# qwagrox/field-coverage-path-planning

Measured on AMD Instinct MI355X. Metric: validated path points/sec (Clothoid+speed+geofence) on 500x200m field batch, higher is better.
Workload: dtype f64; 1 GPU; cfg1 x 4096: 4096 fields of 500 x 200 m per GPU, ARC turns (the reference's own model, pinned to its outputs) at the reference's sampling, 1691 points per field; a step = one fresh plan call of the ba; turn_model=arc (reference, pinned), points_per_gpu_step=6926336, fields_per_gpu=4096, setup=device

## Files before the change

### field_coverage_path_planning_amd/_lib.py

```python
import ctypes as C
import os

_HERE = os.path.dirname(os.path.abspath(__file__))
LIB_PATH = os.environ.get('FCPP_LIBRARY') or os.path.join(_HERE, 'libfcpp.so')

OK, EINVAL, EHEADLAND, EUNSUPPORTED, EHIP, ENOMEM, ESIZE = 0, -1, -2, -3, -4, -5, -6
TURN_ARC, TURN_CLOTHOID = 0, 1
KIND_SWATH, KIND_UTURN, KIND_HEAD_START, KIND_HEAD_STRAIGHT, KIND_CORNER, KIND_REVERSE, KIND_DETOUR = range(7)
OBSTACLES_FLAG, OBSTACLES_AVOID = 0, 1
RING_AS_VERTICES, RING_REVERSED = 0, 1
KIND_MASK, FLAG_HEADLAND, FLAG_ALAT, FLAG_OUTSIDE, FLAG_OBSTACLE, INDEX_SHIFT = 7, 8, 16, 32, 64, 8
OUTPUT_PITCH = 24 << 30

c_double_p = C.POINTER(C.c_double)
c_i64_p = C.POINTER(C.c_int64)


class FcppError(RuntimeError):
    def __init__(self, code, msg):
        super().__init__(f'libfcpp error {code}: {msg}')
        self.code = code


class Vehicle(C.Structure):
    _fields_ = [(n, C.c_double) for n in (
        'working_width', 'min_turn_radius', 'max_work_speed_kmh', 'max_headland_speed_kmh',
        'headland_turn_speed_kmh', 'max_lateral_accel', 'max_longitudinal_accel', 'safety_factor')]


class Options(C.Structure):
    _fields_ = [('turn_model', C.c_int32), ('clothoid_fit', C.c_int32), ('sample_spacing', C.c_double),
                ('clothoid_frac', C.c_double), ('geofence_tol', C.c_double), ('obstacle_mode', C.c_int32), ('ring_order', C.c_int32)]


class Field(C.Structure):
    _fields_ = [('vx', C.c_double * 4), ('vy', C.c_double * 4), ('from_vertices', C.c_int32),
                ('has_start', C.c_int32), ('has_end', C.c_int32),
                ('start_x', C.c_double), ('start_y', C.c_double), ('end_x', C.c_double), ('end_y', C.c_double),
                ('n_obstacles', C.c_int32), ('_pad', C.c_int32), ('obstacle_first', C.c_int64)]


class Polys(C.Structure):
    _fields_ = [('n_polys', C.c_int64), ('offsets', c_i64_p), ('x', c_double_p), ('y', c_double_p)]


class FieldInfo(C.Structure):
    _fields_ = [('point_offset', C.c_int64), ('n_main', C.c_int64), ('n_head', C.c_int64),
                ('n_swaths', C.c_int32), ('n_loops', C.c_int32), ('start_corner', C.c_int32),
                ('reverse_order', C.c_int32), ('start_from_right', C.c_int32), ('rotated', C.c_int32),
                ('start_kept', C.c_int32), ('end_kept', C.c_int32), ('shape', C.c_int32),
                ('n_reverse', C.c_int32 * 4), ('status', C.c_int32),
                ('corner_angles', C.c_double * 4), ('field_length', C.c_double), ('field_width', C.c_double),
                ('headland_width', C.c_double), ('rotation_angle', C.c_double),
                ('approach_from', C.c_double * 2), ('approach_to', C.c_double * 2),
                ('departure_from', C.c_double * 2), ('departure_to', C.c_double * 2)]


class FieldStats(C.Structure):
    _fields_ = [('main_len_m', C.c_double), ('main_time_pre_s', C.c_double), ('main_time_s', C.c_double),
                ('head_len_m', C.c_double), ('head_time_pre_s', C.c_double), ('head_time_s', C.c_double),
                ('max_kappa', C.c_double), ('max_alat', C.c_double), ('max_jump', C.c_double),
                ('n_viol', C.c_int64), ('n_outside', C.c_int64), ('n_in_obstacle', C.c_int64),
                ('n_adjusted', C.c_int64)]


class SetupTimes(C.Structure):
    _fields_ = [('host_plan_ms', C.c_double), ('templates_ms', C.c_double), ('tiler_ms', C.c_double), ('image_ms', C.c_double),
                ('h2d_ms', C.c_double), ('total_ms', C.c_double), ('image_bytes', C.c_int64), ('threads', C.c_int32), ('device_setup', C.c_int32)]


class GaConfig(C.Structure):
    _fields_ = [('population_size', C.c_int32), ('max_generations', C.c_int32), ('crossover_rate', C.c_double),
                ('mutation_rate', C.c_double), ('elite_size', C.c_int32), ('tournament_size', C.c_int32),
                ('convergence_threshold', C.c_int32), ('_pad', C.c_int32), ('seed', C.c_uint64)]


class GaResult(C.Structure):
    _fields_ = [('generations', C.c_int32), ('convergence_gen', C.c_int32), ('best_distance', C.c_double),
                ('best_fitness', C.c_double)]


class CoverJob(C.Structure):
    _fields_ = [('ox', C.c_double), ('oy', C.c_double), ('res', C.c_double), ('shift', C.c_double), ('radius', C.c_double),
                ('nx', C.c_int32), ('ny', C.c_int32), ('n_a', C.c_int32), ('n_b', C.c_int32),
                ('pts_first', C.c_int64), ('grid_first', C.c_int64), ('strict', C.c_int32), ('region', C.c_int32),
                ('outer', C.c_double * 12), ('inner', C.c_double * 12)]


SETUP_AUTO, SETUP_HOST, SETUP_DEVICE = 0, 1, 2

STATS_DOUBLES = 9
STATS_WORDS = 13

_VP = C.c_void_p
PROTOTYPES = [
    ('fcpp_last_error', C.c_char_p, []),
    ('fcpp_abi_version', C.c_int, []),
    ('fcpp_vehicle_default', None, [C.POINTER(Vehicle)]),
    ('fcpp_options_default', None, [C.POINTER(Options)]),
    ('fcpp_ctx_create', C.c_int, [C.c_int, C.POINTER(_VP)]),
    ('fcpp_ctx_destroy', C.c_int, [_VP]),
    ('fcpp_ctx_set_stream', C.c_int, [_VP, _VP]),
    ('fcpp_ctx_synchronize', C.c_int, [_VP]),
    ('fcpp_ctx_set_setup', C.c_int, [_VP, C.c_int]),
    ('fcpp_malloc', C.c_int, [_VP, C.c_int64, C.POINTER(_VP)]),
    ('fcpp_free', C.c_int, [_VP, _VP]),
    ('fcpp_ctx_reserve_outputs', C.c_int, [_VP, C.c_int64, C.c_int64]),
    ('fcpp_ctx_outputs_info', C.c_int, [_VP, c_i64_p, c_i64_p, c_i64_p]),
    ('fcpp_outputs_alloc', C.c_int, [_VP, C.c_int64, C.c_int64] + [C.POINTER(_VP)] * 5),
    ('fcpp_outputs_free', C.c_int, [_VP, _VP]),
    ('fcpp_memcpy_h2d', C.c_int, [_VP, _VP, _VP, C.c_int64]),
    ('fcpp_memcpy_d2h', C.c_int, [_VP, _VP, _VP, C.c_int64]),
    ('fcpp_plan_count', C.c_int, [C.POINTER(Vehicle), C.POINTER(Options), C.c_int64, C.POINTER(Field), C.POINTER(Polys),
                                  C.POINTER(FieldInfo)]),
    ('fcpp_plan_points', C.c_int, [_VP, C.POINTER(Vehicle), C.POINTER(Options), C.c_int64, C.POINTER(Field), C.POINTER(Polys), c_i64_p]),
    ('fcpp_batch_create', C.c_int, [_VP, C.POINTER(Vehicle), C.POINTER(Options), C.c_int64, C.POINTER(Field),
                                    C.POINTER(Polys), C.POINTER(_VP)]),
    ('fcpp_batch_plan', C.c_int, [_VP, C.POINTER(Vehicle), C.POINTER(Options), C.c_int64, C.POINTER(Field), C.POINTER(Polys), _VP,
                                  C.POINTER(_VP)] + [C.POINTER(_VP)] * 5 + [c_i64_p]),
    ('fcpp_batch_own_stats', C.c_int, [_VP, C.POINTER(_VP)]),
    ('fcpp_batch_info', C.c_int, [_VP, C.POINTER(FieldInfo), c_i64_p]),
    ('fcpp_batch_setup_times', C.c_int, [_VP, C.POINTER(SetupTimes)]),
    ('fcpp_batch_run', C.c_int, [_VP, _VP, _VP, _VP, _VP, _VP, _VP, C.c_int]),
    ('fcpp_batch_connectors', C.c_int, [_VP, _VP, _VP]),
    ('fcpp_batch_trajectory', C.c_int, [_VP] * 9),
    ('fcpp_batch_destroy', C.c_int, [_VP]),
    ('fcpp_batch_set_profiling', C.c_int, [_VP, C.c_int]),
    ('fcpp_batch_stage_times', C.c_int, [_VP, C.c_int, c_double_p, C.POINTER(C.c_int), C.POINTER(C.c_int)]),
    ('fcpp_batch_stage_name', C.c_char_p, [C.c_int, C.c_int]),
    ('fcpp_batch_stage_points', C.c_int, [_VP, C.c_int, C.c_int, c_i64_p]),
    ('fcpp_batch_point_split', C.c_int, [_VP, c_i64_p, c_i64_p]),
    ('fcpp_batch_reduce_classes', C.c_int, [_VP, c_i64_p]),
    ('fcpp_curvature', C.c_int, [_VP, C.c_int64, _VP, C.c_int64, _VP, _VP, _VP, _VP]),
    ('fcpp_speed_plan', C.c_int, [_VP, C.POINTER(Vehicle), C.c_int, C.c_int64, _VP, C.c_int64, _VP, _VP, _VP, _VP,
                                  _VP, _VP, _VP]),
    ('fcpp_verify', C.c_int, [_VP, C.POINTER(Vehicle), C.c_int64, _VP, C.c_int64, _VP, _VP, _VP, _VP, _VP]),
    ('fcpp_validate', C.c_int, [_VP, C.POINTER(Vehicle), C.POINTER(Options), C.c_int64, _VP, C.c_int64, _VP, _VP, _VP, C.POINTER(Polys),
                               C.POINTER(Polys), _VP, _VP, _VP, _VP]),
    ('fcpp_trajectory', C.c_int, [_VP, C.c_int64, _VP, C.c_int64] + [_VP] * 9),
    ('fcpp_trajectory_counts', C.c_int, [_VP, C.c_int64, _VP, C.c_double, C.c_int, _VP, _VP]),
    ('fcpp_trajectory_sample', C.c_int, [_VP, C.c_int64, _VP, C.c_int64] + [_VP] * 7 + [C.c_double, C.c_int, _VP, C.c_int64] + [_VP] * 9),
    ('fcpp_straight_segments', C.c_int, [_VP, C.c_int64, _VP, C.c_int32, _VP]),
    ('fcpp_corner_turns', C.c_int, [_VP, C.POINTER(Vehicle), C.c_int64, _VP, _VP, _VP, C.c_double, C.c_double, C.c_int32, _VP, _VP]),
    ('fcpp_fresnel', C.c_int, [_VP, C.c_int64, _VP, _VP, _VP]),
    ('fcpp_ga_fitness', C.c_int, [_VP, C.c_int32, C.c_int64, _VP, _VP, _VP, _VP, C.c_int]),
    ('fcpp_distance_matrix', C.c_int, [_VP, C.c_int32, _VP, _VP, _VP]),
    ('fcpp_best_connections', C.c_int, [_VP, C.c_int64, _VP, _VP, _VP, _VP, _VP, _VP, _VP, _VP, _VP]),
    ('fcpp_dubins_solve', C.c_int, [_VP, C.c_int64] + [_VP] * 6 + [C.c_double, _VP, _VP, _VP]),
    ('fcpp_dubins_matrix', C.c_int, [_VP, C.c_int64, _VP, _VP, _VP, C.c_int64, _VP, _VP, _VP, C.c_double, _VP, _VP]),
    ('fcpp_dubins_counts', C.c_int, [_VP, C.c_int64, _VP, C.c_double, _VP, _VP]),
    ('fcpp_dubins_sample', C.c_int, [_VP, C.c_int64, _VP, _VP, _VP, C.c_double, _VP, _VP, C.c_double, _VP, C.c_int64] + [_VP] * 5),
    ('fcpp_rs_solve', C.c_int, [_VP, C.c_int64] + [_VP] * 6 + [C.c_double, _VP, _VP, _VP]),
    ('fcpp_rs_matrix', C.c_int, [_VP, C.c_int64, _VP, _VP, _VP, C.c_int64, _VP, _VP, _VP, C.c_double, _VP, _VP]),
    ('fcpp_rs_counts', C.c_int, [_VP, C.c_int64, _VP, _VP, C.c_double, _VP, _VP]),
    ('fcpp_rs_sample', C.c_int, [_VP, C.c_int64, _VP, _VP, _VP, C.c_double, _VP, _VP, C.c_double, _VP, C.c_int64] + [_VP] * 6),
    ('fcpp_swath_scores', C.c_int, [_VP, C.c_int64, _VP, C.c_int64, _VP, C.c_int64, _VP, _VP, C.c_int64, _VP, C.c_double, C.c_double, C.c_double]
     + [_VP] * 4),
    ('fcpp_swath_counts', C.c_int, [_VP, C.c_int64, _VP, C.c_int64, _VP, C.c_int64, _VP, _VP, _VP, C.c_double, C.c_double, C.c_double] + [_VP] * 4),
    ('fcpp_swath_fill', C.c_int, [_VP, C.c_int64, _VP, C.c_int64, _VP, C.c_int64, _VP, _VP, _VP, C.c_double, C.c_double, C.c_double, _VP, C.c_int64]
     + [_VP] * 6),
    ('fcpp_ga_evolve', C.c_int, [_VP, C.c_int32, C.POINTER(GaConfig), _VP, _VP, _VP, _VP, C.POINTER(GaResult)]),
    ('fcpp_cover_grid', C.c_int, [_VP, C.c_int64, C.POINTER(CoverJob), C.c_int64, _VP, _VP, _VP, _VP]),
    ('fcpp_gather', C.c_int, [_VP, _VP, C.c_int, C.c_int, C.c_int, C.c_int, _VP, _VP, c_i64_p, _VP, C.c_int]),
    ('fcpp_debug_math', C.c_int, [C.c_int, C.c_int64, _VP, _VP, _VP, _VP]),
    ('fcpp_debug_math_dev', C.c_int, [_VP, C.c_int, C.c_int64, _VP, _VP, _VP, _VP]),
    ('fcpp_debug_dubins', C.c_int, [C.c_int64] + [_VP] * 6 + [C.c_double, _VP, _VP, _VP]),
    ('fcpp_debug_rs', C.c_int, [C.c_int64] + [_VP] * 6 + [C.c_double, _VP, _VP, _VP]),
    ('fcpp_debug_swaths', C.c_int, [C.c_int64, _VP, C.c_int64, _VP, C.c_int64, _VP, _VP, C.c_int64, _VP, C.c_int, C.c_double, C.c_double, C.c_double]
     + [_VP] * 5 + [C.c_int64] + [_VP] * 6),
    ('fcpp_batch_debug_table', C.c_int, [_VP, C.c_int, _VP, C.c_int64, c_i64_p]),
]

_lib = None


def load():
    global _lib
    if _lib is None:
        if not os.path.exists(LIB_PATH):
            raise ImportError(
                f'{LIB_PATH} is missing: build it with `python -c "import __graft_entry__ as g; g.build()"` '
                f'or `make -C {os.path.join(_HERE, "csrc")}`; there is no CPU fallback')
        try:
            import torch
        except ImportError:
            pass
        lib = C.CDLL(LIB_PATH)
        for name, res, args in PROTOTYPES:
            fn = getattr(lib, name)
            fn.restype = res
            fn.argtypes = args
        if lib.fcpp_abi_version() != 5:
            raise ImportError('libfcpp.so ABI version mismatch')
        _lib = lib
    return _lib


def check(rc):
    if rc != OK:
        raise FcppError(rc, load().fcpp_last_error().decode('utf-8', 'replace'))


def default_vehicle():
    v = Vehicle()
    load().fcpp_vehicle_default(C.byref(v))
    return v


def default_options():
    o = Options()
    load().fcpp_options_default(C.byref(o))
    return o
```

### field_coverage_path_planning_amd/csrc/fcpp_api.cpp

```cpp
#include <dlfcn.h>
#include <hip/hip_runtime_api.h>
#include <math.h>
#include <stdio.h>
#include <stdlib.h>
#include <string.h>

#include <algorithm>
#include <atomic>
#include <chrono>
#include <memory>
#include <new>
#include <string>
#include <vector>

#include "fcpp_api_internal.h"
#include "fcpp_cover.h"
#include "fcpp_ga.h"
#include "fcpp_devplan.h"
#include "fcpp_dubinsfn.h"
#include "fcpp_rsfn.h"
#include "fcpp_parallel.h"

using namespace fcpp;

namespace fcpp { thread_local LaunchProf g_launch_prof; }

namespace { thread_local std::string g_err; }

int fcpp::fail(int code, const std::string &msg) { g_err = msg; return code; }

DevConst fcpp::make_const(const fcpp_vehicle &veh, const fcpp_options &opt)
{
    DevConst c;
    c.a_lat = veh.max_lateral_accel; c.a_lon = veh.max_longitudinal_accel; c.sf = veh.safety_factor;
    c.geofence_tol = opt.geofence_tol;
    c.v_work = veh.max_work_speed_kmh; c.v_turn = veh.headland_turn_speed_kmh; c.v_head = veh.max_headland_speed_kmh;
    const double vm = std::max(std::max(veh.max_work_speed_kmh, veh.max_headland_speed_kmh),
                               std::max(veh.headland_turn_speed_kmh, 2.5)) / 3.6;
    c.u_cap = vm * vm;
    c.inv_sf36 = 1.0 / (c.sf * 3.6);
    c.ms_work = c.v_work / 3.6; c.ms_turn = c.v_turn / 3.6; c.ms_head = c.v_head / 3.6; c.ms_rev = 2.5 / 3.6;
    c.shapes = nullptr; c.tmpl_u = nullptr; c.tmpl_c = nullptr; c.tmpl_u_dk = nullptr; c.field_junc = nullptr;
    c.tmpl_n = 0; c.tmpl_nc = 1;
    c.turn_kappa_last[0] = c.turn_kappa_last[1] = c.turn_len = c.turn_time = 0.0;
    c.turn_max_kappa[0] = c.turn_max_kappa[1] = c.turn_max_jump[0] = c.turn_max_jump[1] = 0.0;
    c.turn_jump[0] = c.turn_jump[1] = 0.0;
    return c;
}

namespace fcpp {
struct TemplateSet {
    TurnTemplates tt;
    double clothoid_frac = 0.0;
    DevBuf<CacShape> shapes;
    DevBuf<double2> tmpl_u, tmpl_c, tmpl_u_dk;
    DevBuf<double2> tmpl_c_dk;
    std::vector<double2> h_tu, h_tc, h_dk, h_dkc;
    double tc_lo[2] = { 0.0, 0.0 }, tc_hi[2] = { 0.0, 0.0 };
    bool box_done = false;
    void template_box()
    {
        if (box_done) return;
        for (int d = 0; d < 2; ++d) { tc_lo[d] = 0.0; tc_hi[d] = 0.0; }
        for (size_t k = 0; k < h_tc.size(); ++k) {
            tc_lo[0] = std::min(tc_lo[0], h_tc[k].x); tc_hi[0] = std::max(tc_hi[0], h_tc[k].x);
            tc_lo[1] = std::min(tc_lo[1], h_tc[k].y); tc_hi[1] = std::max(tc_hi[1], h_tc[k].y);
        }
        box_done = true;
    }
    bool same(const TurnTemplates &o, double frac) const { return memcmp(&tt, &o, sizeof tt) == 0 && clothoid_frac == frac; }
};
}

struct fcpp_batch {
    fcpp_ctx *ctx = nullptr;
    fcpp_vehicle veh;
    fcpp_options opt;
    int64_t n_fields = 0;
    HostPlan hp;
    DevConst cst;
    void *slab = nullptr; size_t slab_bytes = 0;
    ImageLayout lay;
    SlabTables t;
    DevTiling til0;
    bool til0_built = false;
    std::shared_ptr<TemplateSet> templates;
    int profiling = 0;
    int64_t run_counter = 0;
    std::vector<hipEvent_t> events;
    std::vector<unsigned char> ev_set;
    int prof_runs = 0;
    int last_mode = 0;
    fcpp_setup_times setup = {};
    const fcpp_field_info *info_dev = nullptr;
    std::vector<hipStream_t> used_streams;
    void note_stream(hipStream_t s) { if (std::find(used_streams.begin(), used_streams.end(), s) == used_streams.end()) used_streams.push_back(s); }
    hipStream_t setup_stream = nullptr;
    bool setup_pending = false;
    hipEvent_t ev_setup = nullptr;
    std::vector<hipStream_t> setup_seen;
    hipError_t wait_setup(hipStream_t s)
    {
        if (!setup_pending || s == setup_stream || std::find(setup_seen.begin(), setup_seen.end(), s) != setup_seen.end()) return hipSuccess;
        if (!ev_setup) {
            if (!ctx->ev_pool.empty()) { ev_setup = ctx->ev_pool.back(); ctx->ev_pool.pop_back(); }
            else { const hipError_t e = hipEventCreateWithFlags(&ev_setup, hipEventDisableTiming); if (e != hipSuccess) return e; }
        }
        hipError_t e = hipEventRecord(ev_setup, setup_stream);
        if (e != hipSuccess) {
            (void)hipGetLastError();
            e = hipDeviceSynchronize();
            if (e == hipSuccess) setup_pending = false;
            return e;
        }
        e = hipStreamWaitEvent(s, ev_setup, 0);
        if (e == hipSuccess) setup_seen.push_back(s);
        return e;
    }
    ~fcpp_batch() { for (hipEvent_t e : events) (void)hipEventDestroy(e); if (ev_setup) (void)hipEventDestroy(ev_setup); }
};

namespace {
constexpr int kStages = 7;
constexpr int kProfRuns = 256;
const char *const kStageNames[2][kStages] = {
    { "k_generate", "k_curv_clamp", "k_scan_tiles", "k_scan_spine", "k_scan_apply", "k_validate", "k_reduce_stats" },
    { "k_plan_quiet_spans", "k_plan_quiet", "k_plan_sparse", "k_plan_fused", "k_reduce_stats", "k_plan_sparse_fields", "" } };
const int kStageCount[2] = { 7, 6 };
}

static bool closed_form_turns(const fcpp_vehicle &veh, const TurnTemplates &tt, const std::vector<double2> &t,
                              const std::vector<double2> &dk, DevConst &c)
{
    const int nu = tt.nu;
    const double W = veh.working_width, R = veh.min_turn_radius;
    if (nu < 3 || fabs(t[0].x - (tt.turn_model == FCPP_TURN_ARC ? R : 0.0)) > 1e-9 || fabs(t[0].y) > 1e-9) return false;
    const double q_t = c.v_turn * c.inv_sf36, q_w = c.v_work * c.inv_sf36, lim = c.a_lat * 0.999;
    double len = 0.0, maxk = 0.0, maxj = 0.0;
    for (int k = 1; k < nu; ++k) len += dk[(size_t)k].x;
    for (int k = 1; k + 1 < nu; ++k) {
        maxk = std::max(maxk, dk[(size_t)k].y);
        maxj = std::max(maxj, fabs(dk[(size_t)k].y - dk[(size_t)k - 1].y));
    }
    if (maxk * q_t * q_t >= lim) return false;
    const bool arc = tt.turn_model == FCPP_TURN_ARC;
    const double sx = arc ? -1.0 : 1.0;
    const double c1x = sx * (t[(size_t)nu - 1].x - t[(size_t)nu - 2].x), c1y = t[(size_t)nu - 1].y - t[(size_t)nu - 2].y;
    const double d1 = sqrt(c1x * c1x + c1y * c1y);
    const double u_t = c.ms_turn * c.ms_turn, u_w = c.ms_work * c.ms_work;
    for (int v = 0; v < 2; ++v) {
        const double jx = arc ? (-R + t[(size_t)nu - 1].x) : -t[(size_t)nu - 1].x;
        const double jy = (v == 0 ? W : -W) - t[(size_t)nu - 1].y;
        const double dj = sqrt(jx * jx + jy * jy);
        if (!(dj >= 1e-3) || d1 < 1e-6) return false;
        if (u_t + 2 * c.a_lon * dj < u_w * (1.0 + 1e-9)) return false;
        const double k_last = fabs(2 * atan2_fd(c1x * jy - c1y * jx, c1x * jx + c1y * jy) / (d1 + dj));
        const double k_first_max = fabs(2 * atan2_fd(jx * 0.0 - jy * -1.0, jx * -1.0 + jy * 0.0) / dj);
        if (k_last * q_t * q_t >= lim || k_first_max * q_w * q_w >= lim) return false;
        c.turn_kappa_last[v] = k_last;
        c.turn_jump[v] = dj;
        c.turn_max_kappa[v] = std::max(maxk, k_last);
        c.turn_max_jump[v] = std::max(std::max(maxj, fabs(dk[(size_t)nu - 2].y - (nu >= 3 ? dk[(size_t)nu - 3].y : 0.0))), fabs(k_last - dk[(size_t)nu - 2].y));
    }
    c.turn_len = len;
    c.turn_time = len / std::max(c.ms_turn, 0.1);
    return true;
}
static CutConsts make_cut_consts(TemplateSet &ts, bool device, const BatchTileConsts &k, const DevConst &cst)
{
    CutConsts cc;
    memset(&cc, 0, sizeof cc);
    ts.template_box();
    if (device) {
        cc.tu = reinterpret_cast<const Pt2 *>(ts.tmpl_u.p); cc.tc = reinterpret_cast<const Pt2 *>(ts.tmpl_c.p);
        cc.dk_u = reinterpret_cast<const Pt2 *>(ts.tmpl_u_dk.p); cc.dk_c = reinterpret_cast<const Pt2 *>(ts.tmpl_c_dk.p);
    } else {
        cc.tu = reinterpret_cast<const Pt2 *>(ts.h_tu.data()); cc.tc = reinterpret_cast<const Pt2 *>(ts.h_tc.data());
        cc.dk_u = reinterpret_cast<const Pt2 *>(ts.h_dk.data()); cc.dk_c = reinterpret_cast<const Pt2 *>(ts.h_dkc.data());
    }
    cc.nu = k.nu; cc.nc = k.nc; cc.turn_quiet = k.turn_quiet ? 1 : 0; cc.wave_factor = k.wave_factor;
    cc.two_a = k.two_a; cc.u_cap = k.u_cap; cc.c_line = k.c_line; cc.fence_margin = k.fence_margin;
    cc.jump[0] = cst.turn_jump[0]; cc.jump[1] = cst.turn_jump[1];
    for (int d = 0; d < 2; ++d) { cc.tc_lo[d] = ts.tc_lo[d]; cc.tc_hi[d] = ts.tc_hi[d]; }
    cc.u_step_min = cc.c_step_min = HUGE_VAL;
    for (size_t k = 1; k < ts.h_dk.size(); ++k) cc.u_step_min = std::min(cc.u_step_min, ts.h_dk[k].x);
    for (size_t k = 1; k < ts.h_dkc.size(); ++k) cc.c_step_min = std::min(cc.c_step_min, ts.h_dkc[k].x);
    if (ts.h_dk.size() < 2) cc.u_step_min = 0.0;
    if (ts.h_dkc.size() < 2) cc.c_step_min = 0.0;
    return cc;
}

extern "C" {

const char *fcpp_last_error(void) { return g_err.c_str(); }
int fcpp_abi_version(void) { return FCPP_ABI_VERSION; }

void fcpp_vehicle_default(fcpp_vehicle *v)
{
    v->working_width = 3.2; v->min_turn_radius = 8.0; v->max_work_speed_kmh = 9.0;
    v->max_headland_speed_kmh = 15.0; v->headland_turn_speed_kmh = 4.0; v->max_lateral_accel = 2.0;
    v->max_longitudinal_accel = 1.5; v->safety_factor = 0.85;
}

void fcpp_options_default(fcpp_options *o)
{
    o->turn_model = FCPP_TURN_ARC; o->clothoid_fit = 1; o->sample_spacing = 0.0; o->clothoid_frac = 0.5;
    o->geofence_tol = 1e-6; o->obstacle_mode = FCPP_OBSTACLES_FLAG; o->ring_order = FCPP_RING_AS_VERTICES;
}

int fcpp_ctx_create(int device_id, fcpp_ctx **out)
{
    if (!out) return fail(FCPP_EINVAL, "ctx out pointer is NULL");
    *out = nullptr;
    int n = 0;
    hipError_t e = hipGetDeviceCount(&n);
    if (e != hipSuccess || n <= 0)
        return fail(FCPP_EHIP, "no HIP device available: libfcpp has no CPU fallback");
    if (device_id < 0 || device_id >= n) return fail(FCPP_EINVAL, "device_id out of range");
    HIPCHK(hipSetDevice(device_id));
    fcpp_ctx *c = new (std::nothrow) fcpp_ctx();
    if (!c) return fail(FCPP_ENOMEM, "out of host memory");
    c->device = device_id;
    e = hipStreamCreateWithFlags(&c->own, hipStreamNonBlocking);
    if (e == hipSuccess) e = hipStreamCreateWithFlags(&c->side, hipStreamNonBlocking);
    if (e == hipSuccess) e = hipEventCreateWithFlags(&c->ev_fork, hipEventDisableTiming);
    if (e == hipSuccess) e = hipEventCreateWithFlags(&c->ev_join, hipEventDisableTiming);
    if (e != hipSuccess) {
        if (c->own) (void)hipStreamDestroy(c->own);
        if (c->side) (void)hipStreamDestroy(c->side);
        if (c->ev_fork) (void)hipEventDestroy(c->ev_fork);
        delete c;
        return fail(FCPP_EHIP, std::string("hipStreamCreate: ") + hipGetErrorString(e));
    }
    c->stream = c->own;
    if (const char *e = getenv("FCPP_SETUP")) c->setup_mode = !strcmp(e, "host") ? FCPP_SETUP_HOST : (!strcmp(e, "device") ? FCPP_SETUP_DEVICE : FCPP_SETUP_AUTO);
    *out = c;
    return FCPP_OK;
}

int fcpp_ctx_set_setup(fcpp_ctx *c, int mode)
{
    if (!c || mode < FCPP_SETUP_AUTO || mode > FCPP_SETUP_DEVICE) return fail(FCPP_EINVAL, "bad arguments");
    c->setup_mode = mode;
    return FCPP_OK;
}

int fcpp_ctx_destroy(fcpp_ctx *c)
{
    if (!c) return FCPP_OK;
    (void)hipSetDevice(c->device);
    if (c->own) { (void)hipStreamSynchronize(c->own); (void)hipStreamDestroy(c->own); }
    if (c->side) { (void)hipStreamSynchronize(c->side); (void)hipStreamDestroy(c->side); }
    if (c->ev_fork) (void)hipEventDestroy(c->ev_fork);
    if (c->ev_join) (void)hipEventDestroy(c->ev_join);
    free_paths_cache(c);
    (void)c->stage_wait();
    if (c->stage) (void)hipHostFree(c->stage);
    if (c->spare) (void)hipFree(c->spare);
    for (auto &sl : c->plan_slots) if (sl.p) { (void)hipDeviceSynchronize(); (void)hipFree(sl.p); sl.p = nullptr; }
    if (c->arena) { (void)hipDeviceSynchronize(); (void)hipFree(c->arena); }
    if (c->ev_plan) (void)hipEventDestroy(c->ev_plan);
    for (hipEvent_t e : c->ev_pool) (void)hipEventDestroy(e);
    if (c->plan_totals_host) (void)hipHostFree(c->plan_totals_host);
    if (c->ga_mirror) (void)hipHostFree(c->ga_mirror);
    if (c->verify_scratch) (void)hipFree(c->verify_scratch);
    c->templates.reset();
    delete c;
    return FCPP_OK;
}

int fcpp_ctx_set_stream(fcpp_ctx *c, void *s)
{
    if (!c) return fail(FCPP_EINVAL, "ctx is NULL");
    c->stream = (hipStream_t)s;
    return FCPP_OK;
}

int fcpp_ctx_synchronize(fcpp_ctx *c)
{
    if (!c) return fail(FCPP_EINVAL, "ctx is NULL");
    HIPCHK(hipSetDevice(c->device));
    HIPCHK(hipStreamSynchronize(c->stream));
    return FCPP_OK;
}

int fcpp_malloc(fcpp_ctx *c, int64_t bytes, void **p)
{
    if (!c || !p || bytes < 0) return fail(FCPP_EINVAL, "bad arguments");
    HIPCHK(hipSetDevice(c->device));
    *p = nullptr;
    if (bytes == 0) return FCPP_OK;
    HIPCHK(hipMalloc(p, (size_t)bytes));
    return FCPP_OK;
}

int fcpp_free(fcpp_ctx *c, void *p)
{
    if (!c) return fail(FCPP_EINVAL, "ctx is NULL");
    HIPCHK(hipSetDevice(c->device));
    if (p) HIPCHK(hipFree(p));
    return FCPP_OK;
}

int fcpp_ctx_reserve_outputs(fcpp_ctx *c, int64_t lane_bytes, int64_t pitch_bytes)
{
    if (!c || lane_bytes < 0 || pitch_bytes < 0) return fail(FCPP_EINVAL, "bad arguments");
    HIPCHK(hipSetDevice(c->device));
    if (c->arena) {
        if (!c->arena_live.empty()) return fail(FCPP_EINVAL, "the output arena has live allocations");
        HIPCHK(hipDeviceSynchronize());
        HIPCHK(hipFree(c->arena));
        c->arena = nullptr; c->arena_pitch = c->arena_lane = 0;
    }
    size_t pitch = pitch_bytes > 0 ? (size_t)pitch_bytes : (size_t)FCPP_OUTPUT_PITCH;
    size_t lane = lane_bytes > 0 ? (size_t)lane_bytes : pitch;
    pitch = (pitch + 4095) / 4096 * 4096; lane = (lane + 4095) / 4096 * 4096;
    if (lane > pitch) pitch = lane;
    size_t free_b = 0, total_b = 0;
    HIPCHK(hipMemGetInfo(&free_b, &total_b));
    const size_t reserve = (size_t)8 << 30;
    if (free_b < 4 * pitch + lane + reserve) return fail(FCPP_ENOMEM, "not enough free device memory for the output arena (4 x pitch + lane + 8 GiB)");
    void *p = nullptr;
    hipError_t e = hipMalloc(&p, 4 * pitch + lane);
    if (e != hipSuccess) return fail(FCPP_ENOMEM, std::string("output arena: ") + hipGetErrorString(e));
    c->arena = p; c->arena_pitch = pitch; c->arena_lane = lane;
    c->arena_live.clear();
    return FCPP_OK;
}

int fcpp_ctx_outputs_info(const fcpp_ctx *c, int64_t *lane_bytes, int64_t *pitch_bytes, int64_t *live_bytes)
{
    if (!c) return fail(FCPP_EINVAL, "ctx is NULL");
    if (lane_bytes) *lane_bytes = (int64_t)c->arena_lane;
    if (pitch_bytes) *pitch_bytes = (int64_t)c->arena_pitch;
    if (live_bytes) { size_t s = 0; for (const auto &blk : c->arena_live) s += blk.len; *live_bytes = (int64_t)s; }
    return FCPP_OK;
}

int fcpp_outputs_alloc(fcpp_ctx *c, int64_t n_points, int64_t pitch_bytes, double **x, double **y, double **kappa, double **v, uint32_t **flagseg)
{
    if (!c || n_points < 0 || !x || !y || !kappa || !v || !flagseg) return fail(FCPP_EINVAL, "bad arguments");
    HIPCHK(hipSetDevice(c->device));
    const size_t S = (((size_t)n_points * 8 + 4095) / 4096) * 4096;
    char *b = nullptr;
    size_t P = 0;
    if (pitch_bytes == 0 && c->arena && S <= c->arena_lane) {
        const size_t need = std::max<size_t>(S, 4096);
        size_t off = 0;
        size_t at = 0;
        for (; at < c->arena_live.size(); ++at) {
            if (c->arena_live[at].off - off >= need) break;
            off = c->arena_live[at].off + c->arena_live[at].len;
        }
        if (off + need <= c->arena_lane) {
            c->arena_live.insert(c->arena_live.begin() + (long)at, fcpp_ctx::ArenaBlock{ off, need, nullptr, false });
            b = static_cast<char *>(c->arena) + off;
            P = c->arena_pitch;
        }
    }
    if (!b) {
        P = pitch_bytes > 0 ? (size_t)pitch_bytes : S;
        if (P < S) P = S;
        P = (P + 4095) / 4096 * 4096;
        void *slab = nullptr;
        hipError_t e = hipMalloc(&slab, std::max<size_t>(4 * P + S, 4096));
        if (e != hipSuccess) return fail(FCPP_ENOMEM, std::string("output arrays: ") + hipGetErrorString(e));
        b = static_cast<char *>(slab);
    }
    *x = reinterpret_cast<double *>(b); *y = reinterpret_cast<double *>(b + P); *kappa = reinterpret_cast<double *>(b + 2 * P);
    *v = reinterpret_cast<double *>(b + 3 * P); *flagseg = reinterpret_cast<uint32_t *>(b + 4 * P);
    return FCPP_OK;
}

int fcpp_outputs_free(fcpp_ctx *c, double *x)
{
    if (!c) return fail(FCPP_EINVAL, "ctx is NULL");
    HIPCHK(hipSetDevice(c->device));
    if (!x) return FCPP_OK;
    char *p = reinterpret_cast<char *>(x);
    if (c->arena && p >= static_cast<char *>(c->arena) && p < static_cast<char *>(c->arena) + c->arena_lane) {
        const size_t off = (size_t)(p - static_cast<char *>(c->arena));
        for (size_t k = 0; k < c->arena_live.size(); ++k)
            if (c->arena_live[k].off == off) {
                const fcpp_ctx::ArenaBlock blk = c->arena_live[k];
                if (blk.used && hipStreamQuery(blk.last) != hipSuccess) { (void)hipGetLastError(); HIPCHK(hipStreamSynchronize(blk.last)); }
                c->arena_live.erase(c->arena_live.begin() + (long)k);
                return FCPP_OK;
            }
        return fail(FCPP_EINVAL, "not an allocation of the output arena");
    }
    HIPCHK(hipStreamSynchronize(c->stream));
    HIPCHK(hipFree(x));
    return FCPP_OK;
}

int fcpp_memcpy_h2d(fcpp_ctx *c, void *dst, const void *src, int64_t bytes)
{
    if (!c || bytes < 0) return fail(FCPP_EINVAL, "bad arguments");
    if (bytes == 0) return FCPP_OK;
    HIPCHK(hipMemcpyAsync(dst, src, (size_t)bytes, hipMemcpyHostToDevice, c->stream));
    HIPCHK(hipStreamSynchronize(c->stream));
    return FCPP_OK;
}

int fcpp_memcpy_d2h(fcpp_ctx *c, void *dst, const void *src, int64_t bytes)
{
    if (!c || bytes < 0) return fail(FCPP_EINVAL, "bad arguments");
// ... 36 lines not shown
}

namespace {
int plan_scratch(fcpp_ctx *c, int64_t n_fields, int max_prims, hipStream_t st, DevPlanScratch &s, std::string &err);
int device_fields(const fcpp_field *fields, int64_t n_fields, hipStream_t st, const DevPlanScratch &s, const fcpp_field *&dev, std::string &err);
}

int fcpp_plan_points(fcpp_ctx *c, const fcpp_vehicle *veh, const fcpp_options *opt, int64_t n_fields, const fcpp_field *fields,
                     const fcpp_polys *obstacles, int64_t *points_out)
{
    if (!c || !veh || !opt || n_fields < 0 || (n_fields > 0 && (!fields || !points_out))) return fail(FCPP_EINVAL, "bad arguments");
    if (n_fields == 0) return FCPP_OK;
    std::string err;
    PlanConsts pc;
    TurnTemplates tt;
    int rc = plan_prepare(*veh, *opt, pc, tt, err);
    if (rc != FCPP_OK) return fail(rc, err);
    const bool on_device = c->setup_mode != FCPP_SETUP_HOST && opt->sample_spacing == 0.0 && opt->obstacle_mode == FCPP_OBSTACLES_FLAG &&
                           pc.max_prims <= DEVPLAN_PRIMS_CAP;
    if (!on_device) {
        HostPlan hp;
        std::vector<fcpp_field> fcopy;
        if ((rc = host_fields(fields, n_fields, fcopy, fields)) != FCPP_OK) return rc;
        rc = build_host_plan(*veh, *opt, n_fields, fields, obstacles, false, hp, err);
        if (rc != FCPP_OK) return fail(rc, err);
        for (int64_t i = 0; i < n_fields; ++i) points_out[i] = hp.info[(size_t)i].n_main + hp.info[(size_t)i].n_head;
        return FCPP_OK;
    }
    HIPCHK(hipSetDevice(c->device));
    hipStream_t st = c->stream;
    DevPlanScratch s;
    if ((rc = plan_scratch(c, n_fields, pc.max_prims, st, s, err)) != FCPP_OK) return fail(rc, err);
    const fcpp_field *dev_fields = nullptr;
    if ((rc = device_fields(fields, n_fields, st, s, dev_fields, err)) != FCPP_OK) return fail(rc, err);
    {
        const int lrc = launch_devplan_points(st, n_fields, pc, s, dev_fields);
        if (lrc) { (void)hipStreamSynchronize(st); return fail(FCPP_EHIP, std::string("launch_devplan_points: ") + hipGetErrorString((hipError_t)lrc)); }
    }
    HIPCHK(hipMemcpyAsync(points_out, s.counts + (int64_t)PC_POINTS * n_fields, (size_t)n_fields * sizeof(int64_t), hipMemcpyDeviceToHost, st));
    HIPCHK(hipStreamSynchronize(st));
    return FCPP_OK;
}

static int get_templates(fcpp_ctx *c, const TurnTemplates &tt, const fcpp_options &opt, hipStream_t st, std::shared_ptr<TemplateSet> &out, bool &fresh)
{
    fresh = false;
    if (c->templates && c->templates->same(tt, opt.clothoid_frac)) { out = c->templates; return FCPP_OK; }
    std::shared_ptr<TemplateSet> ts(new (std::nothrow) TemplateSet());
    if (!ts) return fail(FCPP_ENOMEM, "out of host memory");
    ts->tt = tt; ts->clothoid_frac = opt.clothoid_frac;
    const int nu = tt.nu, nc = tt.nc;
    std::vector<CacShape> shp = { make_cac_shape(kPi, opt.clothoid_frac), make_cac_shape(kHalfPi, opt.clothoid_frac) };
    HIPCHK(ts->shapes.upload(shp, st));
    HIPCHK(hipStreamSynchronize(st));
    HIPCHK(ts->tmpl_u.alloc((size_t)nu));
    HIPCHK(ts->tmpl_c.alloc((size_t)nc));
    HIPCHK(ts->tmpl_u_dk.alloc((size_t)nu));
    HIPCHK(ts->tmpl_c_dk.alloc((size_t)nc));
    LAUNCHCHK(launch_build_templates(st, tt, ts->shapes.p, ts->tmpl_u.p, ts->tmpl_c.p));
    LAUNCHCHK(launch_build_template_metrics(st, nu, ts->tmpl_u.p, ts->tmpl_u_dk.p));
    LAUNCHCHK(launch_build_template_metrics(st, nc, ts->tmpl_c.p, ts->tmpl_c_dk.p));
    ts->h_tu.resize((size_t)nu); ts->h_tc.resize((size_t)nc); ts->h_dk.resize((size_t)nu); ts->h_dkc.resize((size_t)nc);
    if (nu > 0) {
        HIPCHK(hipMemcpyAsync(ts->h_tu.data(), ts->tmpl_u.p, (size_t)nu * sizeof(double2), hipMemcpyDeviceToHost, st));
        HIPCHK(hipMemcpyAsync(ts->h_dk.data(), ts->tmpl_u_dk.p, (size_t)nu * sizeof(double2), hipMemcpyDeviceToHost, st));
    }
    if (nc > 0) {
        HIPCHK(hipMemcpyAsync(ts->h_tc.data(), ts->tmpl_c.p, (size_t)nc * sizeof(double2), hipMemcpyDeviceToHost, st));
        HIPCHK(hipMemcpyAsync(ts->h_dkc.data(), ts->tmpl_c_dk.p, (size_t)nc * sizeof(double2), hipMemcpyDeviceToHost, st));
    }
    out = ts;
    fresh = true;
    return FCPP_OK;
}

namespace {
constexpr size_t kStageMax = (size_t)2 << 30;
constexpr size_t kSpareMax = (size_t)1 << 30;
double ms_since(std::chrono::steady_clock::time_point t0)
{
    return std::chrono::duration<double, std::milli>(std::chrono::steady_clock::now() - t0).count();
}
}

namespace {
thread_local double g_trace_totals_ms = 0.0;
constexpr int kNotOnDevice = 1;

int take_slab(fcpp_ctx *c, fcpp_batch *b, std::string &err)
{
    const ImageLayout &lay = b->lay;
    if (c->spare && c->spare_cap >= lay.total_bytes) { b->slab = c->spare; b->slab_bytes = c->spare_cap; c->spare = nullptr; c->spare_cap = 0; return FCPP_OK; }
    hipError_t e = hipMalloc(&b->slab, std::max<size_t>(lay.total_bytes, 256));
    if (e != hipSuccess) { b->slab = nullptr; err = std::string("batch tables: ") + hipGetErrorString(e); return FCPP_ENOMEM; }
    b->slab_bytes = std::max<size_t>(lay.total_bytes, 256);
    return FCPP_OK;
}

#define DEVCHK(expr)                                                                                     \
    do {                                                                                                 \
        hipError_t e_ = (expr);                                                                          \
        if (e_ != hipSuccess) { err = std::string(#expr) + ": " + hipGetErrorString(e_); return FCPP_EHIP; } \
    } while (0)

int upload_buffer(fcpp_ctx *c, size_t nb, size_t want, std::vector<unsigned char> &pageable, unsigned char *&img, std::string &err)
{
    img = nullptr;
    if (nb <= kStageMax) {
        DEVCHK(c->stage_wait());
        if (c->stage_cap < nb) {
            if (c->stage) { (void)hipHostFree(c->stage); c->stage = nullptr; c->stage_cap = 0; }
            if (hipHostMalloc(&c->stage, want, hipHostMallocDefault) == hipSuccess) c->stage_cap = want;
            else { c->stage = nullptr; (void)hipGetLastError(); }
        }
        if (c->stage_cap >= nb) img = static_cast<unsigned char *>(c->stage);
    }
    if (!img) {
        try { pageable.resize(nb); } catch (const std::bad_alloc &) { err = "out of host memory"; return FCPP_ENOMEM; }
        img = pageable.data();
    }
    return FCPP_OK;
}

bool set_batch_consts(fcpp_batch *b, const TemplateSet &ts)
{
    b->cst = make_const(b->veh, b->opt);
    b->cst.shapes = ts.shapes.p;
    b->cst.tmpl_u = ts.tmpl_u.p; b->cst.tmpl_c = ts.tmpl_c.p; b->cst.tmpl_u_dk = ts.tmpl_u_dk.p;
    b->cst.tmpl_n = (int)ts.tt.nu; b->cst.tmpl_nc = std::max(1, (int)ts.tt.nc);
    return ts.tt.nu >= 3 && closed_form_turns(b->veh, ts.tt, ts.h_tu, ts.h_dk, b->cst);
}

int plan_scratch(fcpp_ctx *c, int64_t n_fields, int max_prims, hipStream_t st, DevPlanScratch &s, std::string &err)
{
    int k = -1;
    for (int i = 0; i < fcpp_ctx::kPlanSlots; ++i) if (c->plan_slots[i].p && c->plan_slots[i].stream == st) k = i;
    if (k < 0) for (int i = 0; i < fcpp_ctx::kPlanSlots; ++i) if (!c->plan_slots[i].p) { k = i; break; }
    if (k < 0) { k = 0; for (int i = 1; i < fcpp_ctx::kPlanSlots; ++i) if (c->plan_slots[i].tick < c->plan_slots[k].tick) k = i; }
    fcpp_ctx::PlanSlot &sl = c->plan_slots[k];
    if (sl.pending && sl.stream != st) {
        if (!c->ev_plan) DEVCHK(hipEventCreateWithFlags(&c->ev_plan, hipEventDisableTiming));
        if (hipEventRecord(c->ev_plan, sl.stream) == hipSuccess) DEVCHK(hipStreamWaitEvent(st, c->ev_plan, 0));
        else { (void)hipGetLastError(); DEVCHK(hipDeviceSynchronize()); }
        sl.pending = false;
    }
    sl.stream = st; sl.tick = ++c->plan_tick;
    c->plan_cur = k;
    const size_t need = devplan_scratch_layout(n_fields, max_prims, nullptr, s);
    if (sl.cap < need) {
        if (sl.p) { DEVCHK(hipDeviceSynchronize()); (void)hipFree(sl.p); sl.p = nullptr; sl.cap = 0; }
        const size_t want = need + need / 4;
        if (hipMalloc(&sl.p, want) != hipSuccess) { (void)hipGetLastError(); sl.p = nullptr; err = "out of device memory for the planner's scratch"; return FCPP_ENOMEM; }
        sl.cap = want;
        DEVCHK(hipMemsetAsync(sl.p, 0, PLAN_TOTALS * sizeof(int64_t), st));
    }
    if (!c->plan_totals_host)
        { DEVCHK(hipHostMalloc((void **)&c->plan_totals_host, PLAN_TOTALS * sizeof(int64_t), hipHostMallocMapped | hipHostMallocCoherent)); memset(c->plan_totals_host, 0, PLAN_TOTALS * sizeof(int64_t)); }
    devplan_scratch_layout(n_fields, max_prims, sl.p, s);
    return FCPP_OK;
}

int device_fields(const fcpp_field *fields, int64_t n_fields, hipStream_t st, const DevPlanScratch &s, const fcpp_field *&dev, std::string &err)
{
    hipPointerAttribute_t at;
    memset(&at, 0, sizeof at);
    void *dp = nullptr;
    if (hipPointerGetAttributes(&at, fields) == hipSuccess && at.type == hipMemoryTypeHost &&
        hipHostGetDevicePointer(&dp, const_cast<fcpp_field *>(fields), 0) == hipSuccess && dp) {
        dev = static_cast<const fcpp_field *>(dp);
        return FCPP_OK;
    }
    int cur = -1;
    if (at.type == hipMemoryTypeDevice && hipGetDevice(&cur) == hipSuccess && at.device == cur) { dev = fields; return FCPP_OK; }
    (void)hipGetLastError();
    DEVCHK(hipMemcpyAsync(s.fields_in, fields, (size_t)n_fields * sizeof(fcpp_field), at.type == hipMemoryTypeDevice ? hipMemcpyDefault : hipMemcpyHostToDevice, st));
    dev = s.fields_in;
    return FCPP_OK;
}

void batch_tile_consts(const fcpp_batch &b, bool turn_quiet, bool field_work, int64_t span_line_max, BatchTileConsts &k)
{
    k.nu = b.templates->tt.nu; k.nc = b.templates->tt.nc;
    k.turn_quiet = turn_quiet;
    k.two_a = 2 * b.cst.a_lon; k.u_cap = b.cst.u_cap; k.c_line = b.cst.ms_work * b.cst.ms_work;
    k.fence_margin = 1e-7 - b.opt.geofence_tol;
    k.fuse_spans = field_work && k.nu <= TMPL_LDS_SAMPLES;
    k.span_line_max = span_line_max;
}

DevTileConsts dev_tile_consts(const BatchTileConsts &k, const fcpp_batch &b, int max_prims, bool dense, int64_t n_fields, int64_t gen)
{
    DevTileConsts tc;
    tc.tu = reinterpret_cast<const Pt2 *>(b.templates->tmpl_u.p); tc.tc = reinterpret_cast<const Pt2 *>(b.templates->tmpl_c.p);
    tc.nu = k.nu; tc.nc = k.nc; tc.turn_quiet = k.turn_quiet; tc.fuse_spans = k.fuse_spans; tc.span_line_max = k.span_line_max;
    tc.two_a = k.two_a; tc.u_cap = k.u_cap; tc.c_line = k.c_line; tc.fence_margin = k.fence_margin;
    tc.wave_factor = k.wave_factor; tc.field_work_tiles = FIELD_WORK_TILES; tc.reduce_wg_max = TileConsts::reduce_wg_max; tc.max_prims = max_prims;
    tc.no_bases = 0; tc.speculative = 0; tc.closed_cut = dense ? 0 : 1; tc.dense = dense ? 1 : 0;
    tc.gen = gen;
    tc.cut = make_cut_consts(*b.templates, true, k, b.cst);
    return tc;
}

void device_layout(ImageLayout &l, int64_t n_fields, const fcpp_polys *obstacles)
{
    l = ImageLayout();
    l.n_fields = n_fields; l.info_on_device = true;
    l.n_polys = obstacles ? obstacles->n_polys : 0; l.n_poly_verts = l.n_polys > 0 ? obstacles->offsets[l.n_polys] : 0;
}

void capacity_layout(ImageLayout &l, int64_t n_fields, const fcpp_polys *obstacles, int max_prims)
{
    device_layout(l, n_fields, obstacles);
    const int64_t K = DEVPLAN_KEEP_TILES;
    l.n_prims = n_fields * max_prims;
    l.n_tiles = l.n_stat = n_fields * (1 + K); l.n_wave = l.n_general = l.n_open_wave = n_fields * K;
    l.n_span_chunks = n_fields * SPEC_SPAN_CHUNKS; l.n_runs = n_fields;
    l.n_red[0] = n_fields; l.n_work[0] = l.n_field_work = n_fields;
    layout_image(l);
}

void counts_from_totals(ImageLayout &l, const int64_t *tot, bool fuse)
{
    l.n_prims = tot[PC_PRIMS];
    l.n_tiles = tot[PC_TILES]; l.n_wave = tot[PC_WAVE]; l.n_general = tot[PC_GENERAL]; l.n_stat = tot[PC_STAT];
    l.n_span_chunks = fuse ? tot[PC_SPAN_F] : tot[PC_SPAN]; l.n_runs = tot[PC_RUNS];
    for (int k = 0; k < 4; ++k) l.n_red[k] = tot[PC_CLS0 + k];
    l.n_work[0] = tot[PC_WORK]; l.n_field_work = tot[PC_WORK]; l.n_open_wave = tot[PC_OPEN];
    l.quiet_points = tot[PC_SPAN_PTS] + tot[PC_CHUNK_PTS]; l.span_points = tot[PC_SPAN_PTS] - (fuse ? tot[PC_WORK_SPAN_PTS] : 0); l.work_span_points = fuse ? tot[PC_WORK_SPAN_PTS] : 0;
    l.n_chunks = tot[PC_CHUNKS]; l.chunk_points = tot[PC_CHUNK_PTS]; l.wave_points = tot[PC_WAVE_PTS];
    l.work_wave_points = tot[PC_WORK_WAVE_PTS]; l.wave_inside = tot[PC_WAVE_INSIDE];
}

int bind_and_upload_obstacles(fcpp_ctx *c, fcpp_batch *b, const fcpp_polys *obstacles, hipStream_t st, std::string &err)
{
    const ImageLayout &lay = b->lay;
    b->t = bind_tables(lay, b->slab);
    if (lay.n_polys <= 0) return FCPP_OK;
    const size_t o0 = lay.obs_off, o1 = lay.seg, nb = o1 - o0;
    std::vector<unsigned char> tmp;
    unsigned char *img = nullptr;
    if (const int urc = upload_buffer(c, nb, nb + nb / 4, tmp, img, err); urc != FCPP_OK) return urc;
    fill_obstacles(obstacles, lay, img, o0);
    DEVCHK(hipMemcpyAsync(static_cast<unsigned char *>(b->slab) + o0, img, nb, hipMemcpyHostToDevice, st));
    if (!tmp.empty()) DEVCHK(hipStreamSynchronize(st));
    else { c->stage_stream = st; c->stage_busy = true; }
    return FCPP_OK;
}

int enqueue_fill(fcpp_batch *b, hipStream_t st, const DevTileConsts &tc, const DevPlanScratch &s, std::string &err)
{
    b->cst.field_junc = b->t.field_junc;
    const int frc = launch_devplan_fill(st, b->n_fields, tc, b->cst, s, b->t);
    if (frc) { err = std::string("launch_devplan_fill: ") + hipGetErrorString((hipError_t)frc); return FCPP_EHIP; }
    return FCPP_OK;
}

int await_totals(const int64_t *tot, int64_t gen, hipStream_t st, std::chrono::steady_clock::time_point t_call, std::string &err)
{
    const volatile int64_t *done = tot + PX_DONE;
    const auto t_poll = std::chrono::steady_clock::now();
    bool seen = false;
    for (int spin = 0; !seen; ++spin) {
        seen = *done == gen;
        if (!seen && (spin & 1023) == 1023 && ms_since(t_poll) > 2.0) break;
    }
    if (!seen) DEVCHK(hipStreamSynchronize(st));
    std::atomic_thread_fence(std::memory_order_acquire);
    g_trace_totals_ms = ms_since(t_call);
    if (tot[PC_COLS + PF_BAD_OBSTACLES] == gen) { err = "field obstacle range outside the polygon table"; return FCPP_ESIZE; }
    if (tot[PC_COLS + PF_FALLBACK] == gen) { err = "a field beyond the device planner's limits (general stretch, primitives)"; return kNotOnDevice; }
    if (tot[PC_POINTS] > kCountCap) { err = "batch too large"; return FCPP_ESIZE; }
    if (tot[PC_PRIMS] > ((int64_t)1 << 26)) { err = "too many path primitives in one batch: split the batch"; return FCPP_ESIZE; }
    if (tot[PC_TILES] > INT32_MAX) { err = "too many tiles in one batch: split the batch"; return FCPP_ESIZE; }
    return FCPP_OK;
}

int try_device_setup(fcpp_ctx *c, fcpp_batch *b, int64_t n_fields, const fcpp_field *fields, const fcpp_polys *obstacles, bool &fresh_templates,
                     bool field_work, int64_t span_line_max, std::string &err)
{
    const fcpp_options &opt = b->opt;
    fcpp_setup_times &tm = b->setup;
    if (c->setup_mode == FCPP_SETUP_HOST) { err = "host setup requested"; return kNotOnDevice; }
    if (n_fields <= 0) { err = "empty batch"; return kNotOnDevice; }
    const char *e_small = getenv("FCPP_SMALL_BATCH");
    if (c->setup_mode == FCPP_SETUP_AUTO && n_fields < (e_small ? atoll(e_small) : 16)) { err = "a handful of fields: set up by the host"; return kNotOnDevice; }
    const bool dense = opt.sample_spacing != 0.0;
    if (opt.obstacle_mode != FCPP_OBSTACLES_FLAG) { err = "obstacle-aware swaths are planned on the host"; return kNotOnDevice; }
    if (!field_work) { err = "FCPP_FIELD_WORK=0: the host tiler's reference path"; return kNotOnDevice; }
    PlanConsts pc;
    TurnTemplates tt;
    int rc = plan_prepare(b->veh, opt, pc, tt, err);
    if (rc != FCPP_OK) return rc;
    if ((rc = validate_polys(obstacles, err)) != FCPP_OK) return rc;
    if (pc.max_prims > DEVPLAN_PRIMS_CAP) { err = "too many headland loops for the device planner"; return kNotOnDevice; }
    hipStream_t st = c->stream;
    auto t0 = std::chrono::steady_clock::now();
    const auto t_call = t0;

    if (fresh_templates) { DEVCHK(hipStreamSynchronize(st)); fresh_templates = false; }
    c->templates = b->templates;
    const bool turn_quiet = set_batch_consts(b, *b->templates);
    tm.templates_ms += ms_since(t0);

    t0 = std::chrono::steady_clock::now();
    DevPlanScratch s;
    if ((rc = plan_scratch(c, n_fields, pc.max_prims, st, s, err)) != FCPP_OK) return rc;
    const fcpp_field *dev_fields = nullptr;
    if ((rc = device_fields(fields, n_fields, st, s, dev_fields, err)) != FCPP_OK) return rc;
    BatchTileConsts k;
    batch_tile_consts(*b, turn_quiet, field_work, span_line_max, k);
    DevTileConsts tc = dev_tile_consts(k, *b, pc.max_prims, dense, n_fields, ++c->plan_gen);
    const int64_t *tot = c->plan_totals_host;

    ImageLayout &lay = b->lay;
    const bool exact_only = getenv("FCPP_SETUP_EXACT") != nullptr;
    bool spec = (n_fields + 1023) / 1024 <= devplan_small_blocks() && !exact_only && !dense;
    if (spec) {
        capacity_layout(lay, n_fields, obstacles, pc.max_prims);
        if (lay.total_bytes > ((size_t)1 << 30)) spec = false;
    }
    tc.speculative = spec ? 1 : 0;
    if (spec) {
        if ((rc = take_slab(c, b, err)) != FCPP_OK) return rc;
        if ((rc = bind_and_upload_obstacles(c, b, obstacles, st, err)) != FCPP_OK) return rc;
    }
    const int lrc = launch_devplan_count(st, n_fields, pc, tc, s, dev_fields, obstacles ? obstacles->n_polys : 0, obstacles != nullptr, c->plan_totals_host);
    if (lrc) { (void)hipStreamSynchronize(st); err = std::string("launch_devplan_count: ") + hipGetErrorString((hipError_t)lrc); return FCPP_EHIP; }
    if (spec && (rc = enqueue_fill(b, st, tc, s, err)) != FCPP_OK) { (void)hipStreamSynchronize(st); return rc; }
    rc = await_totals(tot, tc.gen, st, t_call, err);
    tm.host_plan_ms = ms_since(t0);
    if (rc != FCPP_OK) return rc;

    t0 = std::chrono::steady_clock::now();
    const bool fuse = tc.fuse_spans && tot[PC_UNFUSABLE] == 0 && tot[PC_WORK_SPAN_PTS] > 0;
    if (spec && tot[PC_COLS + PF_OVER_CAPACITY] != tc.gen) {
        counts_from_totals(lay, tot, fuse);
        tm.image_ms = ms_since(t0);
    } else {
        ImageLayout ex;
        device_layout(ex, n_fields, obstacles);
        counts_from_totals(ex, tot, fuse);
        layout_image(ex);
        if (b->slab && b->slab_bytes < ex.total_bytes) {
            DEVCHK(hipStreamSynchronize(st));
            (void)hipFree(b->slab); b->slab = nullptr; b->slab_bytes = 0;
        }
        lay = ex;
        if (!b->slab && (rc = take_slab(c, b, err)) != FCPP_OK) return rc;
        if ((rc = bind_and_upload_obstacles(c, b, obstacles, st, err)) != FCPP_OK) return rc;
        tm.image_ms = ms_since(t0);
        t0 = std::chrono::steady_clock::now();
        tc.speculative = 0;
        tc.fuse_spans = fuse;
        if ((rc = enqueue_fill(b, st, tc, s, err)) != FCPP_OK) return rc;
    }
    tm.image_bytes = (int64_t)((size_t)n_fields * sizeof(fcpp_field) + (lay.n_polys > 0 ? lay.seg - lay.obs_off : 0));
    c->plan_slots[c->plan_cur].pending = true;
    b->setup_stream = st; b->setup_pending = true;
    b->info_dev = b->t.info;
    b->hp.info.clear();
    b->hp.tt = tt;
    b->hp.total_points = tot[PC_POINTS]; b->hp.total_prims = tot[PC_PRIMS];
    b->hp.fields.clear(); b->hp.blocks.clear(); b->hp.same_as.clear();
    tm.tiler_ms = ms_since(t0);
    tm.h2d_ms = 0.0;
    tm.device_setup = 1;
    return FCPP_OK;
}
#undef DEVCHK
}

int fcpp_batch_create(fcpp_ctx *c, const fcpp_vehicle *veh, const fcpp_options *opt, int64_t n_fields,
                      const fcpp_field *fields, const fcpp_polys *obstacles, fcpp_batch **out)
{
    if (!c || !veh || !opt || !out || n_fields < 0 || (n_fields > 0 && !fields))
        return fail(FCPP_EINVAL, "bad arguments");
    if (n_fields > INT32_MAX) return fail(FCPP_ESIZE, "too many fields");
    *out = nullptr;
    const auto t_begin = std::chrono::steady_clock::now();
    HIPCHK(hipSetDevice(c->device));
    std::unique_ptr<fcpp_batch> b(new (std::nothrow) fcpp_batch());
    if (!b) return fail(FCPP_ENOMEM, "out of host memory");
    b->ctx = c; b->veh = *veh; b->opt = *opt; b->n_fields = n_fields;
    const char *e_fw = getenv("FCPP_FIELD_WORK"), *e_span = getenv("FCPP_DENSE_SPAN");
    const bool field_work = !(e_fw && atoi(e_fw) == 0);
    const int64_t span_line_max = e_span && atoll(e_span) <= 0 ? 64 : INT64_MAX;
    fcpp_setup_times &tm = b->setup;
    tm.threads = WorkerPool::width();
    std::string err;
    hipStream_t st = c->stream;
    b->note_stream(st);

    auto t0 = std::chrono::steady_clock::now();
    bool fresh = false;
    {
        TurnTemplates tt;
        int rc = plan_templates(*veh, *opt, tt, err);
        if (rc != FCPP_OK) return fail(rc, err);
        rc = get_templates(c, tt, *opt, st, b->templates, fresh);
        if (rc != FCPP_OK) return rc;
    }
    tm.templates_ms = ms_since(t0);

    {
        int rc = try_device_setup(c, b.get(), n_fields, fields, obstacles, fresh, field_work, span_line_max, err);
        if (rc == FCPP_OK) {
            tm.total_ms = ms_since(t_begin);
            c->last_setup = tm;
            *out = b.release();
            return FCPP_OK;
        }
        if (b->slab) { (void)hipStreamSynchronize(c->stream); (void)hipFree(b->slab); b->slab = nullptr; }
        if (rc != kNotOnDevice) return fail(rc, err);
        if (c->setup_mode == FCPP_SETUP_DEVICE) return fail(FCPP_EUNSUPPORTED, "FCPP_SETUP_DEVICE: " + err);
        err.clear();
    }

    t0 = std::chrono::steady_clock::now();
    std::vector<fcpp_field> fcopy;
    int rc = host_fields(fields, n_fields, fcopy, fields);
    if (rc != FCPP_OK) { if (fresh) (void)hipStreamSynchronize(st); return rc; }
    rc = build_host_plan(*veh, *opt, n_fields, fields, obstacles, true, b->hp, err);
    if (rc != FCPP_OK) { if (fresh) (void)hipStreamSynchronize(st); return fail(rc, err); }
    tm.host_plan_ms = ms_since(t0);

    t0 = std::chrono::steady_clock::now();
    if (fresh) HIPCHK(hipStreamSynchronize(st));
    c->templates = b->templates;
    const TemplateSet &ts = *b->templates;
    const bool turn_quiet = set_batch_consts(b.get(), ts);
    tm.templates_ms += ms_since(t0);

    t0 = std::chrono::steady_clock::now();
    TileConsts tc;
    batch_tile_consts(*b, turn_quiet, field_work, span_line_max, tc);
    tc.tu = reinterpret_cast<const Pt2 *>(ts.h_tu.data()); tc.tc = reinterpret_cast<const Pt2 *>(ts.h_tc.data());
    tc.templates_ok = true;
    tc.field_work = field_work;
    tc.device_chunks = !(getenv("FCPP_HOST_CHUNKS") && atoi(getenv("FCPP_HOST_CHUNKS")) != 0);
    tc.closed_cut = opt->sample_spacing == 0.0 && opt->obstacle_mode == FCPP_OBSTACLES_FLAG;
    tc.cut = make_cut_consts(*b->templates, false, tc, b->cst);
    BatchTiler tiler;
    ImageLayout &lay = b->lay;
    rc = tiler.plan(b->hp, tc, obstacles, lay, err);
    if (rc != FCPP_OK) return fail(rc, err);
    if (tc.fuse_spans && lay.unfusable_work > 0) {
        tc.fuse_spans = false;
        rc = tiler.plan(b->hp, tc, obstacles, lay, err);
        if (rc != FCPP_OK) return fail(rc, err);
    }
    tm.tiler_ms = ms_since(t0);

    t0 = std::chrono::steady_clock::now();
    if ((rc = take_slab(c, b.get(), err)) != FCPP_OK) return fail(rc, err);
    struct SlabGuard {
        fcpp_batch *b; bool armed = true;
        ~SlabGuard() { if (armed && b->slab) { (void)hipFree(b->slab); b->slab = nullptr; } }
    } guard{ b.get() };
    unsigned char *img = nullptr;
    std::vector<unsigned char> pageable;
    rc = upload_buffer(c, lay.upload_bytes, std::min(kStageMax, std::max<size_t>(lay.upload_bytes + lay.upload_bytes / 4, (size_t)1 << 20)), pageable, img, err);
    if (rc != FCPP_OK) return fail(rc, err);
    tiler.fill(b->hp, obstacles, lay, img);
    b->t = bind_tables(lay, b->slab);
    for (PlanBlock &blk : b->hp.blocks) std::vector<DevPrim>().swap(blk.prims);
    std::vector<int32_t>().swap(b->hp.same_as);
    tm.image_ms = ms_since(t0);
    tm.image_bytes = (int64_t)lay.upload_bytes;

    t0 = std::chrono::steady_clock::now();
    if (lay.upload_bytes > 0) HIPCHK(hipMemcpyAsync(b->slab, img, lay.upload_bytes, hipMemcpyHostToDevice, st));
    if (n_fields > 0) {
        b->cst.field_junc = b->t.field_junc;
        LAUNCHCHK(launch_field_junctions(st, n_fields, b->t.fields, b->cst, b->t.field_junc));
        LAUNCHCHK(launch_expand_chunks(st, lay.n_chunk_groups, b->t.chunk_groups,
                                       b->t.tiles, b->t.fields, b->t.chunks, b->t.span_chunks));
        LAUNCHCHK(launch_run_consts(st, lay.n_stat, b->t.stat_ids, b->t.stat_run, b->t.tiles, b->t.fields, b->t.prims, b->cst, b->t.partial));
        LAUNCHCHK(launch_work_totals(st, lay.n_field_work, b->t.field_work, b->t.stat_run, b->t.partial, b->t.work_totals));
    }
    if (!pageable.empty() || lay.upload_bytes == 0) HIPCHK(hipStreamSynchronize(st));
    else { c->stage_stream = st; c->stage_busy = true; b->setup_stream = st; b->setup_pending = true; }
    tm.h2d_ms = ms_since(t0);
    tm.total_ms = ms_since(t_begin);
    c->last_setup = tm;
    guard.armed = false;
    *out = b.release();
    return FCPP_OK;
}

static int ensure_info(fcpp_batch *b)
{
    if (!b->info_dev || !b->hp.info.empty() || b->n_fields == 0) return FCPP_OK;
    HIPCHK(hipSetDevice(b->ctx->device));
    try { b->hp.info.resize((size_t)b->n_fields); } catch (const std::bad_alloc &) { return fail(FCPP_ENOMEM, "out of host memory"); }
    for (hipStream_t s : b->used_streams) HIPCHK(hipStreamSynchronize(s));
    HIPCHK(hipMemcpy(b->hp.info.data(), b->info_dev, (size_t)b->n_fields * sizeof(fcpp_field_info), hipMemcpyDeviceToHost));
    return FCPP_OK;
}

int fcpp_batch_setup_times(const fcpp_batch *b, fcpp_setup_times *out)
{
    if (!b || !out) return fail(FCPP_EINVAL, "bad arguments");
    *out = b->setup;
    return FCPP_OK;
}

int fcpp_batch_info(const fcpp_batch *b, fcpp_field_info *info_out, int64_t *total_points)
{
    if (!b) return fail(FCPP_EINVAL, "batch is NULL");
    if (info_out && b->n_fields) { const int rc = ensure_info(const_cast<fcpp_batch *>(b)); if (rc) return rc; }
    if (info_out && b->n_fields) memcpy(info_out, b->hp.info.data(), (size_t)b->n_fields * sizeof(fcpp_field_info));
    if (total_points) *total_points = b->hp.total_points;
    return FCPP_OK;
}

int fcpp_batch_run(fcpp_batch *b, double *x, double *y, double *kappa, double *v, uint32_t *fs,
                   fcpp_field_stats *stats, int mode)
{
    if (!b) return fail(FCPP_EINVAL, "batch is NULL");
    if (mode != 0 && mode != 1) return fail(FCPP_EINVAL, "unknown pipeline mode");
    if (mode != b->last_mode) { b->prof_runs = 0; b->last_mode = mode; }
    if (b->n_fields == 0) return FCPP_OK;
    if (b->hp.total_points > 0 && (!x || !y || !kappa || !v || !fs)) return fail(FCPP_EINVAL, "output pointer is NULL");
    if (!stats) return fail(FCPP_EINVAL, "stats pointer is NULL");
    HIPCHK(hipSetDevice(b->ctx->device));
    hipStream_t st = b->ctx->stream;
    b->note_stream(st);
    HIPCHK(b->wait_setup(st));
    if (fcpp_ctx *c = b->ctx; c->arena && x) {
        const char *p = reinterpret_cast<const char *>(x), *a0 = static_cast<const char *>(c->arena);
        if (p >= a0 && p < a0 + c->arena_lane) {
            const size_t off = (size_t)(p - a0);
            for (auto &blk : c->arena_live) if (off >= blk.off && off < blk.off + blk.len) { blk.last = st; blk.used = true; break; }
        }
    }
    if (mode == 0 && !b->til0_built) {
        { const int rc = ensure_info(b); if (rc) return rc; }
        Tiling t0;
        std::vector<int64_t> offs((size_t)b->n_fields + 1, 0);
        for (int64_t i = 0; i < b->n_fields; ++i) offs[(size_t)i + 1] = offs[(size_t)i] + b->hp.info[(size_t)i].n_main + b->hp.info[(size_t)i].n_head;
        t0.build(b->n_fields, offs.data());
        HIPCHK(b->til0.upload(t0, st));
        b->til0_built = true;
    }
    DevObstacles obs = { b->t.obs_off, b->t.obs_x, b->t.obs_y, b->t.obs_bbox };
    hipEvent_t *ev = nullptr;
    unsigned char *evs = nullptr;
    if (b->profiling > 0 && b->prof_runs < kProfRuns && (b->run_counter++ % b->profiling) == 0) {
        ev = &b->events[(size_t)b->prof_runs * kStages * 2];
        evs = &b->ev_set[(size_t)b->prof_runs * kStages];
    }
#define STAGE(k, call)                                                                  \
    do {                                                                                \
        if (ev) { g_launch_prof.start = ev[2 * (k)]; g_launch_prof.stop = ev[2 * (k) + 1]; } \
        const int e_ = (call);                                                          \
        if (ev) { evs[k] = g_launch_prof.start == nullptr; g_launch_prof = LaunchProf(); }   \
        if (e_ != 0) return fail(FCPP_EHIP, std::string(#call) + ": " + hipGetErrorString((hipError_t)e_)); \
    } while (0)
    if (mode == 1) {
        const SlabTables &t = b->t;
        const ImageLayout &lay = b->lay;
        hipStream_t sd = st;
        const bool two = lay.span_points + lay.chunk_points > 0 && lay.n_general > 0 && lay.n_general <= 512 && lay.n_wave == 0;
        if (two) {
            sd = b->ctx->side;
            HIPCHK(hipEventRecord(b->ctx->ev_fork, st));
            HIPCHK(hipStreamWaitEvent(sd, b->ctx->ev_fork, 0));
        }
        const bool fw = lay.n_field_work > 0;
        if (!fw) STAGE(2, launch_plan_sparse(sd, lay.n_wave, t.wtiles, t.fields, t.prims, b->cst, obs, x, y, kappa, v, fs, t.partial));
        else STAGE(2, launch_plan_sparse(sd, lay.n_open_wave, t.wtiles, t.fields, t.prims, b->cst, obs, x, y, kappa, v, fs, t.partial, t.open_wave_ids));
        STAGE(3, launch_plan_fused(sd, lay.n_general, t.general_ids, t.tiles, t.fields, t.prims, b->cst, obs, x,
                                   y, kappa, v, fs, t.partial));
        if (two) HIPCHK(hipEventRecord(b->ctx->ev_join, sd));
        STAGE(0, launch_plan_quiet(st, lay.n_span_chunks, t.span_chunks, 16, t.fields, t.prims, b->cst, obs, x, y, kappa, v, fs, t.partial));
        STAGE(1, launch_plan_quiet(st, lay.n_chunks, t.chunks, 14, t.fields, t.prims, b->cst, obs, x, y, kappa, v, fs, t.partial));
        if (fw) {
            int64_t off = 0;
            bool first = true;
            for (int c = 0; c < 4; ++c) {
                if (lay.n_work[c] == 0) continue;
                if (first) STAGE(5, launch_plan_sparse_fields(st, lay.n_work[c], t.field_packs + off, b->cst, obs, x, y, kappa, v, fs, t.partial,
                                                              FIELD_WORK_WAVES[c], t.work_totals + off, stats, lay.work_span_points > 0));
                else LAUNCHCHK(launch_plan_sparse_fields(st, lay.n_work[c], t.field_packs + off, b->cst, obs, x, y, kappa, v, fs, t.partial,
                                                         FIELD_WORK_WAVES[c], t.work_totals + off, stats, lay.work_span_points > 0));
                first = false;
                off += lay.n_work[c];
            }
        }
        if (two) HIPCHK(hipStreamWaitEvent(st, b->ctx->ev_join, 0));
        {
            const int groups[4] = { 8, 64, 256, 256 };
            const int32_t *pl = t.red_paths;
            bool first = true;
            for (int c = 0; c < 4; ++c) {
                if (lay.n_red[c] == 0) continue;
                const int32_t *list = lay.n_red[c] == lay.n_fields ? nullptr : pl;
                if (first)
                    STAGE(4, launch_reduce_stats(st, lay.n_red[c], t.partial, t.stat_first, nullptr, stats, nullptr, nullptr, nullptr,
                                                 nullptr, nullptr, &b->cst, list, groups[c], c == 3 ? t.red_scratch : nullptr, 1));
                else
                    LAUNCHCHK(launch_reduce_stats(st, lay.n_red[c], t.partial, t.stat_first, nullptr, stats, nullptr, nullptr, nullptr,
                                                  nullptr, nullptr, &b->cst, list, groups[c], c == 3 ? t.red_scratch : nullptr, 1));
                first = false;
                pl += lay.n_red[c];
            }
        }
        if (ev) ++b->prof_runs;
        return FCPP_OK;
    }
    DevTiling &t = b->til0;
    HIPCHK(hipMemsetAsync(t.n_adj.p, 0, (size_t)t.n_paths * sizeof(unsigned long long), st));
    STAGE(0, launch_generate(st, t.n_tiles, t.tiles.p, b->t.fields, b->t.prims, b->cst, x, y, v, fs));
    STAGE(1, launch_curv_clamp(st, t.n_tiles, t.tiles.p, t.paths.p, b->cst, 1, x, y, v, v, kappa, t.n_adj.p));
    STAGE(2, launch_scan_tiles(st, t.n_tiles, t.tiles.p, t.paths.p, b->cst, x, y, v, t.agg_f.p, t.agg_b.p));
    STAGE(3, launch_scan_spine(st, t.n_tiles, t.agg_f.p, t.agg_b.p, t.carry_f.p, t.carry_b.p, t.spine.p));
    STAGE(4, launch_scan_apply(st, t.n_tiles, t.tiles.p, t.paths.p, b->cst, 3, x, y, v, v, t.carry_f.p, t.carry_b.p));
    STAGE(5, launch_validate(st, t.n_tiles, t.tiles.p, t.paths.p, b->t.fields, b->cst, obs, x, y, kappa, v, fs, t.partial.p));
    STAGE(6, launch_reduce_stats(st, t.n_paths, t.partial.p, t.tile_first.p, t.n_adj.p, stats));
#undef STAGE
    if (ev) ++b->prof_runs;
    return FCPP_OK;
}

int fcpp_batch_plan(fcpp_ctx *c, const fcpp_vehicle *veh, const fcpp_options *opt, int64_t n_fields, const fcpp_field *fields,
                    const fcpp_polys *obstacles, fcpp_field_stats *stats, fcpp_batch **batch, double **x, double **y, double **kappa, double **v,
                    uint32_t **fs, int64_t *total_points)
{
    if (!batch || !x || !y || !kappa || !v || !fs) return fail(FCPP_EINVAL, "bad arguments");
    *batch = nullptr; *x = *y = *kappa = *v = nullptr; *fs = nullptr;
    fcpp_batch *b = nullptr;
    static const bool trace = getenv("FCPP_TRACE_PLAN") != nullptr;
    const auto t_begin = std::chrono::steady_clock::now();
    int rc = fcpp_batch_create(c, veh, opt, n_fields, fields, obstacles, &b);
    if (rc != FCPP_OK) return rc;
    const double t_create = trace ? ms_since(t_begin) : 0.0;
    const int64_t total = b->hp.total_points;
    rc = fcpp_outputs_alloc(c, total, 0, x, y, kappa, v, fs);
    const double t_alloc = trace ? ms_since(t_begin) : 0.0;
    if (rc == FCPP_OK) {
        if (!stats) stats = b->t.own_stats;
        rc = fcpp_batch_run(b, *x, *y, *kappa, *v, *fs, stats, 1);
        if (trace) fprintf(stderr, "[fcpp] plan call: entered at %.1f us (CLOCK_MONOTONIC mod 1 s), totals seen %.1f us, create returns %.1f, arrays %.1f, step enqueued %.1f\n",
                           (double)(std::chrono::duration_cast<std::chrono::nanoseconds>(t_begin.time_since_epoch()).count() % 1000000000ll) / 1e3,
                           g_trace_totals_ms * 1e3, t_create * 1e3, t_alloc * 1e3, ms_since(t_begin) * 1e3);
        if (rc != FCPP_OK) { const std::string keep = g_err; (void)hipStreamSynchronize(c->stream); (void)fcpp_outputs_free(c, *x); g_err = keep; }
    }
    if (rc != FCPP_OK) {
        const std::string keep = g_err;
        (void)fcpp_batch_destroy(b);
        *x = *y = *kappa = *v = nullptr; *fs = nullptr;
        g_err = keep;
        return rc;
    }
    *batch = b;
    if (total_points) *total_points = total;
    return FCPP_OK;
}

int fcpp_batch_own_stats(const fcpp_batch *b, fcpp_field_stats **stats)
{
    if (!b || !stats) return fail(FCPP_EINVAL, "bad arguments");
    *stats = b->t.own_stats;
    return FCPP_OK;
}

int fcpp_batch_set_profiling(fcpp_batch *b, int enable)
{
    if (!b) return fail(FCPP_EINVAL, "batch is NULL");
    HIPCHK(hipSetDevice(b->ctx->device));
    if (enable && b->events.empty()) {
        b->events.resize((size_t)kProfRuns * kStages * 2);
        b->ev_set.assign((size_t)kProfRuns * kStages, 0);
        for (hipEvent_t &e : b->events) HIPCHK(hipEventCreate(&e));
    }
    b->profiling = enable > 0 ? enable : 0;
    b->prof_runs = 0; b->run_counter = 0;
    return FCPP_OK;
}

int fcpp_batch_stage_times(fcpp_batch *b, int max_stages, double *ms_sum, int *n_stages, int *n_runs)
{
    if (!b || !ms_sum || max_stages < kStages) return fail(FCPP_EINVAL, "bad arguments");
    HIPCHK(hipSetDevice(b->ctx->device));
    HIPCHK(hipStreamSynchronize(b->ctx->stream));
    const int ns = kStageCount[b->last_mode];
    for (int k = 0; k < kStages; ++k) ms_sum[k] = 0.0;
    for (int r = 0; r < b->prof_runs; ++r) {
        hipEvent_t *ev = &b->events[(size_t)r * kStages * 2];
        for (int k = 0; k < ns; ++k) {
            if (!b->ev_set[(size_t)r * kStages + k]) continue;
            float ms = 0.f;
            HIPCHK(hipEventElapsedTime(&ms, ev[2 * k], ev[2 * k + 1]));
            ms_sum[k] += ms;
        }
    }
    if (n_stages) *n_stages = ns;
    if (n_runs) *n_runs = b->prof_runs;
    b->prof_runs = 0;
    return FCPP_OK;
}

int fcpp_batch_stage_points(const fcpp_batch *b, int mode, int stage, int64_t *points)
{
    if (!b || !points || mode < 0 || mode > 1 || stage < 0 || stage >= kStageCount[mode]) return fail(FCPP_EINVAL, "bad arguments");
    const ImageLayout &t = b->lay;
    const int64_t all = b->hp.total_points;
    if (mode == 0) { *points = all; return FCPP_OK; }
    const int64_t per_stage[6] = { t.span_points, t.chunk_points, t.wave_points - t.work_wave_points, all - t.quiet_points - t.wave_points, all,
                                   t.work_wave_points + t.work_span_points };
    *points = per_stage[stage];
    return FCPP_OK;
}

int fcpp_batch_point_split(const fcpp_batch *b, int64_t *quiet_points, int64_t *general_points)
{
    if (!b) return fail(FCPP_EINVAL, "batch is NULL");
    const int64_t q = b->lay.quiet_points;
    if (quiet_points) *quiet_points = q;
    if (general_points) *general_points = b->hp.total_points - q;
    return FCPP_OK;
}

int fcpp_batch_reduce_classes(const fcpp_batch *b, int64_t *classes_out)
{
    if (!b || !classes_out) return fail(FCPP_EINVAL, "bad arguments");
    for (int c = 0; c < 4; ++c) classes_out[c] = b->lay.n_red[c];
    return FCPP_OK;
}

const char *fcpp_batch_stage_name(int mode, int stage)
{
    return (mode >= 0 && mode < 2 && stage >= 0 && stage < kStages) ? kStageNames[mode][stage] : "";
}

int fcpp_batch_connectors(fcpp_batch *b, double *approach_xy, double *departure_xy)
{
    if (!b) return fail(FCPP_EINVAL, "batch is NULL");
    if (b->n_fields == 0) return FCPP_OK;
    HIPCHK(hipSetDevice(b->ctx->device));
    hipStream_t st = b->ctx->stream;
    b->note_stream(st);
    HIPCHK(b->wait_setup(st));
    if (approach_xy) LAUNCHCHK(launch_straight(st, b->n_fields, b->t.seg, 50, b->t.seg_mask, approach_xy));
    if (departure_xy)
        LAUNCHCHK(launch_straight(st, b->n_fields, b->t.seg + 4 * b->n_fields, 50, b->t.seg_mask + b->n_fields, departure_xy));
    return FCPP_OK;
}

int fcpp_batch_destroy(fcpp_batch *b)
{
    if (!b) return FCPP_OK;
    fcpp_ctx *c = b->ctx;
    (void)hipSetDevice(c->device);
    for (hipStream_t s : b->used_streams) (void)hipStreamSynchronize(s);
    if (c->side) (void)hipStreamSynchronize(c->side);
    if (b->slab) {
        if (b->slab_bytes <= kSpareMax && b->slab_bytes > c->spare_cap) {
            if (c->spare) (void)hipFree(c->spare);
            c->spare = b->slab; c->spare_cap = b->slab_bytes;
        } else (void)hipFree(b->slab);
        b->slab = nullptr;
    }
    if (b->ev_setup && c->ev_pool.size() < 64) { c->ev_pool.push_back(b->ev_setup); b->ev_setup = nullptr; }
    delete b;
    return FCPP_OK;
}

int fcpp_batch_trajectory(fcpp_batch *b, const double *x, const double *y, const double *v, const uint32_t *flagseg, double *s, double *t,
                          double *heading, double *totals)
{
    if (!b) return fail(FCPP_EINVAL, "batch is NULL");
    if (b->n_fields == 0) return FCPP_OK;
    if (b->hp.total_points > 0 && (!x || !y || !v)) return fail(FCPP_EINVAL, "bad arguments");
    HIPCHK(hipSetDevice(b->ctx->device));
    { const int rc = ensure_info(b); if (rc) return rc; }
    std::vector<int64_t> offs;
    try { offs.assign(2 * (size_t)b->n_fields + 1, 0); } catch (const std::bad_alloc &) { return fail(FCPP_ENOMEM, "out of host memory"); }
    for (int64_t i = 0; i < b->n_fields; ++i) {
        const fcpp_field_info &fi = b->hp.info[(size_t)i];
        offs[2 * (size_t)i + 1] = offs[2 * (size_t)i] + fi.n_main;
        offs[2 * (size_t)i + 2] = offs[2 * (size_t)i + 1] + fi.n_head;
    }
    hipStream_t st = b->ctx->stream;
    b->note_stream(st);
    HIPCHK(b->wait_setup(st));
    return trajectory_paths(b->ctx, 2 * b->n_fields, nullptr, offs.data(), b->hp.total_points, x, y, v, flagseg, s, t, heading, totals);
}

int fcpp_ga_evolve(fcpp_ctx *c, int32_t n, const fcpp_ga_config *cfg, const double *D, int32_t *routes, int32_t *best_route,
                   double *hist, fcpp_ga_result *result)
{
    if (!c || !cfg || !D || !routes || !best_route || !result) return fail(FCPP_EINVAL, "bad arguments");
    const int pop = cfg->population_size;
    if (n < 2 || n > GA_MAX_NODES) return fail(FCPP_EUNSUPPORTED, "n_nodes must be in [2, 2048]");
    if (pop < 2 || (pop & 1) || cfg->elite_size < 0 || cfg->elite_size >= pop || cfg->tournament_size < 1 ||
        cfg->tournament_size > 64 || cfg->tournament_size > pop || cfg->max_generations < 0)
        return fail(FCPP_EINVAL, "population_size must be even and > elite_size; 1 <= tournament_size <= min(64, population_size)");
    HIPCHK(hipSetDevice(c->device));
// ... 299 lines not shown
```

### field_coverage_path_planning_amd/csrc/fcpp_api_internal.h

```cpp
#pragma once
#include <hip/hip_runtime_api.h>
#include <stdint.h>

#include <memory>
#include <string>
#include <vector>

#include "fcpp_device.h"
#include "fcpp_internal.h"
#include "fcpp_tiler.h"

namespace fcpp {

int fail(int code, const std::string &msg);

#define HIPCHK(expr)                                                                                     \
    do {                                                                                                 \
        hipError_t e_ = (expr);                                                                          \
        if (e_ != hipSuccess)                                                                            \
            return fail(FCPP_EHIP, std::string(#expr) + ": " + hipGetErrorString(e_));                   \
    } while (0)
#define LAUNCHCHK(expr) HIPCHK((hipError_t)(expr))

template <class T>
struct DevBuf {
    T *p = nullptr;
    size_t n = 0;
    ~DevBuf() { release(); }
    void release() { if (p) (void)hipFree(p); p = nullptr; n = 0; }
    hipError_t alloc(size_t count)
    {
        release();
        n = count;
        if (count == 0) return hipSuccess;
        return hipMalloc((void **)&p, count * sizeof(T));
    }
    hipError_t upload(const std::vector<T> &h, hipStream_t st)
    {
        hipError_t e = alloc(h.size());
        if (e != hipSuccess || h.empty()) return e;
        return hipMemcpyAsync(p, h.data(), h.size() * sizeof(T), hipMemcpyHostToDevice, st);
    }
};

DevConst make_const(const fcpp_vehicle &veh, const fcpp_options &opt);

struct Tiling {
    std::vector<DevPath> paths;
    std::vector<DevTile> tiles;
    std::vector<int64_t> tile_first;
    void build(int64_t n_paths, const int64_t *offsets)
    {
        paths.resize((size_t)n_paths);
        tile_first.assign((size_t)n_paths + 1, 0);
        tiles.clear();
        for (int64_t p = 0; p < n_paths; ++p) {
            const int64_t n = offsets[p + 1] - offsets[p];
            paths[(size_t)p] = { offsets[p], n };
            tile_first[(size_t)p] = (int64_t)tiles.size();
            if (n <= 0) continue;
            const int64_t k = (n + TILE_POINTS - 1) / TILE_POINTS;
            const TilerSplit<int64_t> sp(n, k);
            for (int64_t i = 0; i < k; ++i) {
                DevTile t;
                t.field = (int32_t)p; t.start = sp.start(i); t.count = (int32_t)sp.count(i); t.quiet = 0; t.stat_tile = 0; t.idx0 = 0; t.off0 = 0;
                tiles.push_back(t);
            }
        }
        tile_first[(size_t)n_paths] = (int64_t)tiles.size();
    }
};

struct DevTiling {
    DevBuf<DevPath> paths;
    DevBuf<DevTile> tiles;
    DevBuf<int64_t> tile_first;
    DevBuf<char> agg_f, agg_b;
    DevBuf<double> carry_f, carry_b;
    DevBuf<char> spine;
    DevBuf<TilePartial> partial;
    DevBuf<unsigned long long> n_adj;
    int64_t n_tiles = 0, n_paths = 0;
    hipError_t upload(const Tiling &t, hipStream_t st)
    {
        n_tiles = (int64_t)t.tiles.size(); n_paths = (int64_t)t.paths.size();
        hipError_t e;
        if ((e = paths.upload(t.paths, st)) != hipSuccess) return e;
        if ((e = tiles.upload(t.tiles, st)) != hipSuccess) return e;
        if ((e = tile_first.upload(t.tile_first, st)) != hipSuccess) return e;
        if ((e = agg_f.alloc((size_t)n_tiles * 16)) != hipSuccess) return e;
        if ((e = agg_b.alloc((size_t)n_tiles * 16)) != hipSuccess) return e;
        if ((e = carry_f.alloc((size_t)n_tiles)) != hipSuccess) return e;
        if ((e = carry_b.alloc((size_t)n_tiles)) != hipSuccess) return e;
        if ((e = spine.alloc((size_t)spine_scratch_bytes(n_tiles))) != hipSuccess) return e;
        if ((e = partial.alloc((size_t)n_tiles)) != hipSuccess) return e;
        if ((e = n_adj.alloc((size_t)n_paths)) != hipSuccess) return e;
        return hipStreamSynchronize(st);
    }
};

struct TemplateSet;
struct PathTiling;
void free_paths_cache(fcpp_ctx *c);

int trajectory_paths(fcpp_ctx *c, int64_t n_paths, const int64_t *offsets, const int64_t *offsets_host, int64_t total, const double *x,
                     const double *y, const double *v, const uint32_t *fs, double *s, double *t, double *heading, double *totals);

}

struct fcpp_ctx {
    int device = 0;
    fcpp::PathTiling *paths_cache = nullptr;
    hipStream_t own = nullptr, stream = nullptr;
    hipStream_t side = nullptr;
    hipEvent_t ev_fork = nullptr, ev_join = nullptr;
    void *stage = nullptr; size_t stage_cap = 0;
    hipStream_t stage_stream = nullptr; bool stage_busy = false;
    hipError_t stage_wait()
    {
        if (!stage_busy) return hipSuccess;
        stage_busy = false;
        hipError_t e = hipStreamSynchronize(stage_stream);
        if (e != hipSuccess) { (void)hipGetLastError(); e = hipDeviceSynchronize(); }
        return e;
    }
    void *spare = nullptr; size_t spare_cap = 0;
    std::shared_ptr<fcpp::TemplateSet> templates;
    fcpp_setup_times last_setup = {};
    int setup_mode = FCPP_SETUP_AUTO;
    struct PlanSlot { void *p = nullptr; size_t cap = 0; hipStream_t stream = nullptr; bool pending = false; uint64_t tick = 0; };
    static constexpr int kPlanSlots = 4;
    PlanSlot plan_slots[kPlanSlots];
    uint64_t plan_tick = 0;
    int plan_cur = 0;
    void *verify_scratch = nullptr;
    size_t verify_scratch_cap = 0;
    int64_t *plan_totals_host = nullptr;
    unsigned long long *ga_mirror = nullptr;
    int64_t plan_gen = 0;
    hipEvent_t ev_plan = nullptr;
    void *arena = nullptr; size_t arena_pitch = 0, arena_lane = 0;
    struct ArenaBlock { size_t off, len; hipStream_t last = nullptr; bool used = false; };
    std::vector<ArenaBlock> arena_live;
    std::vector<hipEvent_t> ev_pool;
};
```

### field_coverage_path_planning_amd/csrc/fcpp_device.h

```cpp
#pragma once
#include <stdlib.h>
#include <hip/hip_runtime_api.h>
#include <hip/hip_vector_types.h>
#include <stdint.h>

#include "fcpp_geom.h"
#include "fcpp_internal.h"

namespace fcpp {

struct DevPath { int64_t off, n; };

struct DevObstacles {
    const int64_t *offsets;
    const double *x, *y;
    const double *bbox;
};

struct DevConst {
    double a_lat, a_lon, sf, geofence_tol;
    double v_work, v_turn, v_head;
    double u_cap;
    double ms_work, ms_turn, ms_head, ms_rev;
    double inv_sf36;
    const CacShape *shapes;
    const double2 *tmpl_u, *tmpl_c;
    int tmpl_n, tmpl_nc;
    double turn_kappa_last[2];
    double turn_len, turn_time;
    double turn_max_kappa[2], turn_max_jump[2];
    double turn_jump[2];
    const double2 *field_junc;
    const double2 *tmpl_u_dk;
};

struct LaunchProf { hipEvent_t start = nullptr, stop = nullptr; };
extern thread_local LaunchProf g_launch_prof;

int launch_generate(hipStream_t st, int64_t n_tiles, const DevTile *tiles, const DevField *fields,
                    const DevPrim *prims, const DevConst &cst, double *x, double *y, double *v, uint32_t *fs);
int launch_curv_clamp(hipStream_t st, int64_t n_tiles, const DevTile *tiles, const DevPath *paths,
                      const DevConst &cst, int do_clamp, const double *x, const double *y, const double *v_in,
                      double *v_out, double *kappa, unsigned long long *n_adjusted);
int launch_scan_tiles(hipStream_t st, int64_t n_tiles, const DevTile *tiles, const DevPath *paths, const DevConst &cst,
                      const double *x, const double *y, const double *v_in, void *agg_f, void *agg_b);
int64_t spine_scratch_bytes(int64_t n_tiles);
int launch_scan_spine(hipStream_t st, int64_t n_tiles, const void *agg_f, const void *agg_b, double *carry_f,
                      double *carry_b, void *scratch = nullptr);
int launch_scan_apply(hipStream_t st, int64_t n_tiles, const DevTile *tiles, const DevPath *paths, const DevConst &cst,
                      int min_n, const double *x, const double *y, const double *v_in, double *v_out,
                      const double *carry_f, const double *carry_b);
int launch_validate(hipStream_t st, int64_t n_tiles, const DevTile *tiles, const DevPath *paths,
                    const DevField *fields, const DevConst &cst, const DevObstacles &obs, const double *x,
                    const double *y, const double *kappa, const double *v, uint32_t *fs, TilePartial *partial);
int launch_validate_polys(hipStream_t st, int64_t n_tiles, const DevTile *tiles, const DevPath *paths, const int64_t *field_off, const double *field_x,
                          const double *field_y, int64_t n_field, const int64_t *obst_off, const double *obst_x, const double *obst_y, int64_t n_obst,
                          const int64_t *obst_range, double tol, double a_lat, const double *x, const double *y, const double *kappa, const double *v,
                          uint32_t *flags, fcpp_field_stats *stats);
int launch_reduce_stats(hipStream_t st, int64_t n_list, TilePartial *partial, const int64_t *tile_first,
                        const unsigned long long *n_adjusted, fcpp_field_stats *stats, const int32_t *ids = nullptr,
                        const int64_t *run_count = nullptr, const DevTile *tiles = nullptr, const DevField *fields = nullptr,
                        const DevPrim *prims = nullptr, const DevConst *cst = nullptr, const int32_t *path_list = nullptr, int group = 64,
                        void *scratch = nullptr,
                        int clear_counts = 0);
int launch_expand_chunks(hipStream_t st, int64_t n_segments, const DevChunkGroup *groups, const DevTile *tiles, const DevField *fields,
                         DevTile *chunks, DevTile *span_chunks);
int launch_run_consts(hipStream_t st, int64_t n_entries, const int32_t *ids, const int64_t *run_count, const DevTile *tiles, const DevField *fields,
                      const DevPrim *prims, const DevConst &cst, TilePartial *partial);
int launch_build_templates(hipStream_t st, const TurnTemplates &tt, const CacShape *shapes, void *tu, void *tc);
int launch_plan_fused(hipStream_t st, int64_t n_tiles, const int32_t *ids, const DevTile *tiles,
                      const DevField *fields, const DevPrim *prims, const DevConst &cst, const DevObstacles &obs, double *x,
                      double *y, double *kappa, double *v, uint32_t *fs, TilePartial *partial);
int launch_plan_sparse(hipStream_t st, int64_t n_wtiles, const DevWaveTile *wtiles, const DevField *fields, const DevPrim *prims,
                       const DevConst &cst, const DevObstacles &obs, double *x, double *y, double *kappa, double *v, uint32_t *fs,
                       TilePartial *partial, const int32_t *ids = nullptr);
int launch_plan_sparse_fields(hipStream_t st, int64_t n_work, const DevFieldPack *packs, const DevConst &cst, const DevObstacles &obs, double *x,
                              double *y, double *kappa, double *v, uint32_t *fs, TilePartial *partial, int waves, const TilePartial *totals,
                              fcpp_field_stats *stats, bool spans);
int launch_work_totals(hipStream_t st, int64_t n_work, const DevFieldWork *work, const int64_t *stat_run, const TilePartial *partial, TilePartial *totals);
int launch_distance_matrix(hipStream_t st, int n, const double *x, const double *y, double *D);
int launch_best_connections(hipStream_t st, int64_t n_pairs, const int64_t *fo, const int64_t *to, const double *fx, const double *fy,
                            const double *tx, const double *ty, int32_t *bf, int32_t *bt, double *bd);
int launch_build_template_metrics(hipStream_t st, int n, const void *tmpl, void *dk);
int launch_field_junctions(hipStream_t st, int64_t n_fields, const DevField *fields, const DevConst &cst, void *junc);
int launch_plan_quiet(hipStream_t st, int64_t n_chunks, const DevTile *chunks, int kinds, const DevField *fields, const DevPrim *prims,
                      const DevConst &cst, const DevObstacles &obs, double *x, double *y, double *kappa, double *v, uint32_t *fs,
                      TilePartial *partial);
int launch_straight(hipStream_t st, int64_t n_seg, const double *seg, int n_pts, const int32_t *mask, double *out);
int launch_corner_turns(hipStream_t st, int64_t n, const double *corners, const int32_t *ci, const int32_t *rev, double R, double L,
                        double H, int stride, double *out, int32_t *counts);
int launch_fresnel(hipStream_t st, int64_t n, const double *t, double *c, double *s);
int launch_ga_fitness(hipStream_t st, int n, int64_t pop, const double *D, const int32_t *routes, double *dist,
                      double *fit, int order_mode);

}
```

### field_coverage_path_planning_amd/csrc/fcpp_devplan.h

```cpp
#pragma once
#include <hip/hip_runtime_api.h>
#include <stdint.h>

#include "fcpp_device.h"
#include "fcpp_internal.h"
#include "fcpp_slab.h"
#include "fcpp_planfn.h"
#include "fcpp_tilefn.h"
#include "fcpp_cutfn.h"

namespace fcpp {

enum PlanCol : int {
    PC_POINTS = 0, PC_PRIMS, PC_TILES, PC_WAVE, PC_GENERAL, PC_STAT, PC_SPAN, PC_WORK, PC_OPEN, PC_CLS0, PC_CLS1, PC_CLS2, PC_CLS3,
    PC_RUNS, PC_SPAN_PTS, PC_WAVE_PTS, PC_WORK_WAVE_PTS, PC_WAVE_INSIDE, PC_WORK_SPAN_PTS, PC_SPAN_F, PC_UNFUSABLE,
    PC_CHUNKS, PC_CHUNK_PTS,
    PC_COLS
};
enum PlanFlag : int { PF_FALLBACK = 0, PF_BAD_OBSTACLES = 1, PF_OVER_CAPACITY = 2, PF_COUNT = 3 };
constexpr int PX_ARRIVED = PC_COLS + PF_COUNT, PX_DONE = PC_COLS + PF_COUNT + 1, PLAN_TOTALS = PC_COLS + PF_COUNT + 2;
constexpr int SPEC_SPAN_CHUNKS = 16;

struct DevTileConsts {
    const Pt2 *tu, *tc;
    int32_t nu, nc;
    int32_t turn_quiet, wave_factor, field_work_tiles, max_prims, fuse_spans;
    int32_t no_bases;
    int32_t speculative;
    int32_t closed_cut;
    int32_t dense;
    int64_t span_line_max;
    double two_a, u_cap, c_line, fence_margin;
    int64_t reduce_wg_max;
    int64_t gen;
    CutConsts cut;
};

struct DevPlanScratch {
    fcpp_field *fields_in;
    fcpp_field_info *info;
    DevField *fields_tmp;
    DevPrim *prims_tmp;
    int64_t *counts, *bases;
    int64_t *blk_sums;
    int64_t *totals;
    DevTile *keep_tiles;
    DevWaveTile *keep_wtiles;
};
int64_t devplan_small_blocks();
size_t devplan_scratch_layout(int64_t n, int max_prims, void *base, DevPlanScratch &s);

constexpr int DEVPLAN_WINDOW = 576;
constexpr int DEVPLAN_PRIMS_CAP = 255;
constexpr int DEVPLAN_KEEP_TILES = 8;
constexpr int DEVPLAN_KEEP_ROWS = CUT_TILES_MAX;
static_assert(DEVPLAN_KEEP_ROWS >= DEVPLAN_KEEP_TILES, "the window cut keeps its first DEVPLAN_KEEP_TILES tiles in the same rows");
constexpr int DEVPLAN_KEEP_WROWS = DEVPLAN_KEEP_ROWS + 1;
static_assert(sizeof(DevWaveTile) == 64, "a row of the kept wave tiles holds the 64 stretches' bytes");

int launch_devplan_count(hipStream_t st, int64_t n, const PlanConsts &pc, const DevTileConsts &tc, const DevPlanScratch &s, const fcpp_field *fields,
                         int64_t n_polys, int check_obstacles, int64_t *totals_host);
int launch_devplan_points(hipStream_t st, int64_t n, const PlanConsts &pc, const DevPlanScratch &s, const fcpp_field *fields);
int launch_devplan_fill(hipStream_t st, int64_t n, const DevTileConsts &tc, const DevConst &cst, const DevPlanScratch &s, const SlabTables &t);
int launch_debug_math(hipStream_t st, int fn, int64_t n, const double *a, const double *b, double *out0, double *out1);

}
```

### field_coverage_path_planning_amd/csrc/fcpp_devplan.hip

```cpp
#include <hip/hip_runtime.h>
#include <stddef.h>
#include <stdlib.h>
#include <string.h>

#include "fcpp_devplan.h"
#include "fcpp_quiet_fn.h"

namespace fcpp {

size_t devplan_scratch_layout(int64_t n, int max_prims, void *base, DevPlanScratch &s)
{
    size_t off = 0;
    auto take = [&](auto *&p, size_t count) { p = base ? reinterpret_cast<decltype(p + 0)>(static_cast<unsigned char *>(base) + off) : nullptr; off = (off + count * sizeof(*p) + 255) & ~(size_t)255; };
    const size_t nn = (size_t)(n > 0 ? n : 1), nblk = (nn + 1023) / 1024;
    take(s.totals, PLAN_TOTALS);
    take(s.fields_in, nn); take(s.info, nn); take(s.fields_tmp, nn); take(s.prims_tmp, nn * (size_t)max_prims);
    take(s.counts, nn * PC_COLS); take(s.bases, nn * PC_COLS); take(s.blk_sums, nblk * PC_COLS);
    take(s.keep_tiles, nn * DEVPLAN_KEEP_ROWS); take(s.keep_wtiles, nn * DEVPLAN_KEEP_WROWS);
    return off;
}

#define FCPP_FILL_TABLES(X)                                                                                                          \
    X(fields) X(prims) X(tiles) X(wtiles) X(general_ids) X(span_chunks) X(chunks) X(stat_ids) X(stat_first) X(stat_run) X(red_paths) \
    X(field_work) X(field_packs) X(open_wave_ids) X(seg) X(seg_mask) X(partial) X(field_junc) X(work_totals) X(info)
#define X(name) decltype(SlabTables::name) name;
struct DevPlanTables { FCPP_FILL_TABLES(X) };
#undef X

int64_t devplan_small_blocks()
{
    return 8;
}

namespace {

struct DevSink {
    DevPrim *base;
    int cap;
    int64_t n;
    __device__ int64_t size() const { return n; }
    __device__ void push(const DevPrim &p) { if (n < cap) base[n] = p; ++n; }
    __device__ void truncate(int64_t m) { n = m; }
    __device__ int clipped_layer1(const PlanConsts &, const fcpp_field &, const Layer1Frame &, int64_t &) { return FCPP_EUNSUPPORTED; }
    __device__ int headland_straight(const PlanConsts &, const Quad &, const DevPrim &, int64_t &) { return FCPP_EUNSUPPORTED; }
    __device__ bool box_meets_square(double, double, double) const { return false; }
    __device__ bool box_meets_segment(double, double, double, double) const { return false; }
};

__global__ __launch_bounds__(64) void k_plan_fields(int64_t n, PlanConsts pc, const fcpp_field *__restrict__ fin, fcpp_field_info *__restrict__ info,
                                                    DevField *__restrict__ ftmp, DevPrim *__restrict__ ptmp, int64_t *__restrict__ counts,
                                                    int64_t *__restrict__ totals, int64_t n_polys, int check_obstacles, int count_only, int64_t gen)
{
    const int64_t i = (int64_t)blockIdx.x * 64 + threadIdx.x;
    if (i >= n) return;
    const fcpp_field f = fin[i];
    if (check_obstacles && (f.n_obstacles < 0 || f.obstacle_first < 0 || (f.n_obstacles > 0 && f.obstacle_first + f.n_obstacles > n_polys)))
        atomicMax(reinterpret_cast<unsigned long long *>(totals + PC_COLS + PF_BAD_OBSTACLES), (unsigned long long)gen);
    DevSink sink{ count_only ? nullptr : ptmp + i * pc.max_prims, count_only ? 0 : pc.max_prims, 0 };
    const int64_t npts = plan_field_t(pc, f, info[i], ftmp[i], sink);
    counts[(int64_t)PC_POINTS * n + i] = npts;
    if (count_only) return;
    counts[(int64_t)PC_PRIMS * n + i] = ftmp[i].prim_count;
    if (sink.n > pc.max_prims) atomicMax(reinterpret_cast<unsigned long long *>(totals + PC_COLS + PF_FALLBACK), (unsigned long long)gen);
}

#ifdef FCPP_DIAG_TILE
__device__ unsigned long long g_plan_stamps[16];
#define PSTAMP(k) do { if (field == 1000 && (threadIdx.x & 15) == 0) g_plan_stamps[k] = wall_clock64(); } while (0)
#else
#define PSTAMP(k) do { } while (0)
#endif
namespace p16 {
__device__ __forceinline__ double qget(double v, int k) { return __shfl(v, (int)((threadIdx.x & ~3u) | (unsigned)k)); }
__device__ __forceinline__ int qgeti(int v, int k) { return __shfl(v, (int)((threadIdx.x & ~3u) | (unsigned)k)); }
__device__ __forceinline__ double rget(double v, int k) { return __shfl(v, (int)((threadIdx.x & ~15u) | (unsigned)k)); }
__device__ __forceinline__ int rgeti(int v, int k) { return __shfl(v, (int)((threadIdx.x & ~15u) | (unsigned)k)); }
__device__ __forceinline__ unsigned qballot(bool p) { return (unsigned)((__ballot(p) >> (threadIdx.x & 60u)) & 0xFull); }
__device__ __forceinline__ unsigned rballot(bool p) { return (unsigned)((__ballot(p) >> (threadIdx.x & 48u)) & 0xFFFFull); }
__device__ __forceinline__ double qsum_seq(double v) { double s = 0.0; s += qget(v, 0); s += qget(v, 1); s += qget(v, 2); s += qget(v, 3); return s; }
__device__ __forceinline__ double qmin_seq(double v) { double m = qget(v, 0); for (int k = 1; k < 4; ++k) m = hmin(m, qget(v, k)); return m; }
__device__ __forceinline__ double qmax_seq(double v) { double m = qget(v, 0); for (int k = 1; k < 4; ++k) m = hmax(m, qget(v, k)); return m; }
__device__ __forceinline__ double area_centroid_q(double px, double py, int i, double &cx, double &cy)
{
    const double nx = qget(px, (i + 1) & 3), ny = qget(py, (i + 1) & 3);
    const double cr = px * ny - nx * py;
    double a = qsum_seq(cr);
    const double sx = qsum_seq((px + nx) * cr), sy = qsum_seq((py + ny) * cr);
    a *= 0.5;
    if (fabs(a) < 1e-300) { cx = qget(px, 0); cy = qget(py, 0); return 0.0; }
    cx = sx / (6.0 * a); cy = sy / (6.0 * a);
    return a;
}
}

__global__ __launch_bounds__(64) void k_plan_fields16(int64_t n, PlanConsts pc, const fcpp_field *__restrict__ fin, fcpp_field_info *__restrict__ info,
                                                      DevField *__restrict__ ftmp, DevPrim *__restrict__ ptmp, int64_t *__restrict__ counts,
                                                      int64_t *__restrict__ totals, int64_t n_polys, int check_obstacles, int64_t gen)
{
    using namespace p16;
    const int lane = threadIdx.x, l16 = lane & 15, i = lane & 3, lp = l16 >> 2;
    const int64_t field = (int64_t)blockIdx.x * 4 + (lane >> 4);
    if (field >= n) return;
    PSTAMP(0);
    const fcpp_field f = fin[field];
    if (check_obstacles && l16 == 0 && (f.n_obstacles < 0 || f.obstacle_first < 0 || (f.n_obstacles > 0 && f.obstacle_first + f.n_obstacles > n_polys)))
        atomicMax(reinterpret_cast<unsigned long long *>(totals + PC_COLS + PF_BAD_OBSTACLES), (unsigned long long)gen);
    const fcpp_vehicle &veh = pc.veh;
    const fcpp_options &opt = pc.opt;
    const double W = pc.W, R = pc.R, ds = pc.ds;
    const bool cloth = pc.cloth != 0;
    fcpp_field_info &in = info[field];
    DevField &df = ftmp[field];
    {
        static_assert(sizeof(fcpp_field_info) % 8 == 0 && sizeof(DevField) % 8 == 0, "zeroed as 8-byte words");
        unsigned long long *zi = reinterpret_cast<unsigned long long *>(&in), *zd = reinterpret_cast<unsigned long long *>(&df);
        for (int w = l16; w < (int)(sizeof(fcpp_field_info) / 8); w += 16) zi[w] = 0ull;
        for (int w = l16; w < (int)(sizeof(DevField) / 8); w += 16) zd[w] = 0ull;
    }
    const bool w0 = l16 == 0;
    DevPrim *const pbase = ptmp + field * pc.max_prims;
    auto finish = [&](int64_t npts, int32_t prim_count, int32_t n_pushed) {
        if (w0) {
            counts[(int64_t)PC_POINTS * n + field] = npts;
            counts[(int64_t)PC_PRIMS * n + field] = prim_count;
            if (n_pushed > pc.max_prims) atomicMax(reinterpret_cast<unsigned long long *>(totals + PC_COLS + PF_FALLBACK), (unsigned long long)gen);
        }
    };
#define P16_FAIL(code) do { if (w0) { in.status = (code); in.n_main = in.n_head = 0; in.n_reverse[0] = in.n_reverse[1] = in.n_reverse[2] = in.n_reverse[3] = 0; \
                                      df.n_main = df.n_total = 0; df.gen_main = 0; df.prim_first = 0; df.prim_count = 0; } finish(0, 0, 0); return; } while (0)
    const double qx = i == 0 ? f.vx[0] : (i == 1 ? f.vx[1] : (i == 2 ? f.vx[2] : f.vx[3]));
    const double qy = i == 0 ? f.vy[0] : (i == 1 ? f.vy[1] : (i == 2 ? f.vy[2] : f.vy[3]));
    const int in1 = (i + 1) & 3, ip1 = (i + 3) & 3, io = (i + 2) & 3;
    const double xn = qget(qx, in1), yn = qget(qy, in1), xp = qget(qx, ip1), yp = qget(qy, ip1), xo = qget(qx, io), yo = qget(qy, io);
    {
        const bool fin_i = isfinite(qx) && isfinite(qy);
        const double cr = (xn - qx) * (yo - yn) - (yn - qy) * (xo - xn);
        const int pos = __popc(qballot(cr > 0)), neg = __popc(qballot(cr < 0));
        const bool convex = (pos == 0 || neg == 0) && (pos + neg) > 0;
        if (qballot(fin_i) != 0xFu || !convex) P16_FAIL(FCPP_EUNSUPPORTED);
    }
    PSTAMP(1);
    const double bminx = qmin_seq(qx), bmaxx = qmax_seq(qx), bminy = qmin_seq(qy), bmaxy = qmax_seq(qy);
    const double L = f.from_vertices ? (bmaxx - bminx) : f.vx[1];
    const double H = f.from_vertices ? (bmaxy - bminy) : f.vy[2];
    if (w0) { in.field_length = L; in.field_width = H; }
    double cang;
    {
        const double v1x = xp - qx, v1y = yp - qy, v2x = xn - qx, v2y = yn - qy;
        double c = (v1x * v2x + v1y * v2y) / (sqrt(v1x * v1x + v1y * v1y) * sqrt(v2x * v2x + v2y * v2y));
        c = hmin(1.0, hmax(-1.0, c));
        cang = fc_acos(c) * (180.0 / kPi);
    }
    const double cang0 = qget(cang, 0), cang1 = qget(cang, 1), cang2 = qget(cang, 2), cang3 = qget(cang, 3);
    if (w0) { in.corner_angles[0] = cang0; in.corner_angles[1] = cang1; in.corner_angles[2] = cang2; in.corner_angles[3] = cang3; }
    const bool all90 = qballot(fabs(cang - 90) < 1.0) == 0xFu;
    bool is_par;
    {
        const double ex = xn - qx, ey = yn - qy, ox = xp - xo, oy = yp - yo;
        const double cross = fabs(ex * oy - ey * ox);
        const double na = sqrt(ex * ex + ey * ey), nb = sqrt(ox * ox + oy * oy);
        const bool ok = cross < 0.01 * (na * nb);
        is_par = (qballot(ok) & 3u) == 3u;
    }
    if (w0) { in.shape = all90 ? 0 : (is_par ? 1 : 2); }
    const double hw = R;
    if (w0) { in.headland_width = hw; }
    const bool has_start = f.has_start && (0 <= f.start_x && f.start_x <= L && 0 <= f.start_y && f.start_y <= H);
    const bool has_end = f.has_end && (0 <= f.end_x && f.end_x <= L && 0 <= f.end_y && f.end_y <= H);
    if (w0) { in.start_kept = has_start; in.end_kept = has_end; }
    int sci = 0;
    if (has_start) {
        const double cxs = (i == 0 || i == 3) ? hw / 2 : L - hw / 2, cys = i < 2 ? hw / 2 : H - hw / 2;
// ... 281 lines not shown
    const unsigned long long arrived = atomicAdd(reinterpret_cast<unsigned long long *>(totals + PX_ARRIVED), 1ull);
    if (arrived == (unsigned long long)(n_cols - 1)) {
        totals[PX_ARRIVED] = 0;
        __threadfence_system();
        reinterpret_cast<volatile int64_t *>(mirror)[PX_DONE] = done_gen;
    }
}

__device__ __forceinline__ int64_t wg_incl_scan(int64_t v, int64_t *lds , int64_t &total)
{
    const int lane = threadIdx.x & 63, wave = threadIdx.x >> 6;
#pragma unroll
    for (int o = 1; o < 64; o <<= 1) {
        const int64_t u = __shfl_up(v, o);
        if (lane >= o) v += u;
    }
    if (lane == 63) lds[wave] = v;
    __syncthreads();
    int64_t pre = 0, tot = 0;
#pragma unroll
    for (int q = 0; q < 4; ++q) { const int64_t s = lds[q]; if (q < wave) pre += s; tot += s; }
    __syncthreads();
    total = tot;
    return v + pre;
}

__device__ __forceinline__ void span_counts(int64_t pt_off, int64_t S, bool is_work, bool fuse_possible, int64_t &c_span, int64_t &c_span_f,
                                            int64_t &c_work_span_pts, int64_t &c_unfusable)
{
    c_span = c_span_f = c_work_span_pts = c_unfusable = 0;
    if (S <= 0) return;
    const int64_t n_chunks = ((pt_off % TILE_POINTS) + S + TILE_POINTS - 1) / TILE_POINTS;
    const bool fusable = is_work && n_chunks <= FUSED_SPAN_CHUNKS;
    const int64_t fused = (fusable && fuse_possible) ? S : 0;
    c_span = n_chunks; c_span_f = fused > 0 ? 0 : n_chunks; c_work_span_pts = fused; c_unfusable = (is_work && !fusable) ? 1 : 0;
}

__global__ __launch_bounds__(256) void k_scan_block_sums(int64_t n, int c0, const int64_t *__restrict__ counts, int64_t *__restrict__ blk_sums, int64_t nblk)
{
    __shared__ int64_t lds[4];
    const int col = c0 + blockIdx.y;
    const int64_t base = (int64_t)blockIdx.x * 1024;
    int64_t v = 0;
#pragma unroll
    for (int k = 0; k < 4; ++k) { const int64_t i = base + k * 256 + threadIdx.x; if (i < n) v += counts[(int64_t)col * n + i]; }
    int64_t tot;
    wg_incl_scan(v, lds, tot);
    if (threadIdx.x == 0) blk_sums[(int64_t)col * nblk + blockIdx.x] = tot;
}
__global__ __launch_bounds__(256) void k_scan_block_bases(int c0, int64_t *__restrict__ blk_sums, int64_t nblk, int64_t *__restrict__ totals,
                                                          int64_t *__restrict__ mirror, int with_flags, int64_t done_gen)
{
    __shared__ int64_t lds[4];
    const int col = c0 + blockIdx.x;
    int64_t carry = 0;
    for (int64_t b0 = 0; b0 < nblk; b0 += 256) {
        const int64_t i = b0 + threadIdx.x;
        const int64_t v = i < nblk ? blk_sums[(int64_t)col * nblk + i] : 0;
        int64_t tot;
        const int64_t inc = wg_incl_scan(v, lds, tot);
        if (i < nblk) blk_sums[(int64_t)col * nblk + i] = carry + inc - v;
        carry += tot;
    }
    if (threadIdx.x == 0) { totals[col] = carry; publish_total(totals, mirror, col, carry, with_flags && blockIdx.x == 0); if (with_flags) publish_done(totals, mirror, (int)gridDim.x, done_gen); }
}
__global__ __launch_bounds__(256) void k_scan_apply(int64_t n, int c0, int64_t *__restrict__ counts, const int64_t *__restrict__ blk_sums,
                                                    int64_t nblk, int64_t *__restrict__ bases, int derive, int fuse_possible)
{
    __shared__ int64_t lds[4];
    const int col = c0 + blockIdx.y;
    const int64_t base = (int64_t)blockIdx.x * 1024 + (int64_t)threadIdx.x * 4;
    int64_t v[4], s = 0;
#pragma unroll
    for (int k = 0; k < 4; ++k) { v[k] = base + k < n ? counts[(int64_t)col * n + base + k] : 0; s += v[k]; }
    int64_t tot;
    int64_t run = wg_incl_scan(s, lds, tot) - s + blk_sums[(int64_t)col * nblk + blockIdx.x];
#pragma unroll
    for (int k = 0; k < 4; ++k) {
        if (base + k < n) {
            bases[(int64_t)col * n + base + k] = run;
            if (derive && col == PC_POINTS) {
                const int64_t f = base + k;
                int64_t c_span, c_span_f, c_wsp, c_unf;
                span_counts(run, counts[(int64_t)PC_SPAN_PTS * n + f], counts[(int64_t)PC_WORK * n + f] != 0, fuse_possible != 0, c_span, c_span_f, c_wsp, c_unf);
                counts[(int64_t)PC_SPAN * n + f] = c_span; counts[(int64_t)PC_SPAN_F * n + f] = c_span_f;
                counts[(int64_t)PC_WORK_SPAN_PTS * n + f] = c_wsp; counts[(int64_t)PC_UNFUSABLE * n + f] = c_unf;
            }
        }
        run += v[k];
    }
}

__global__ __launch_bounds__(1024) void k_scan_small(int64_t n, int c0, int64_t *__restrict__ counts, int64_t *__restrict__ bases, int64_t *__restrict__ totals,
                                                     int64_t *__restrict__ mirror, int with_flags, int derive, int fuse_possible, int64_t spec_gen, int64_t done_gen)
{
    __shared__ int64_t lds[16];
    int over = 0;
    const int col = c0 + blockIdx.x;
    const int lane = threadIdx.x & 63, wave = threadIdx.x >> 6;
    auto scan4 = [&](const int64_t (&v)[4], int64_t &tot) -> int64_t {
        const int64_t s = v[0] + v[1] + v[2] + v[3];
        int64_t inc = s;
#pragma unroll
        for (int o = 1; o < 64; o <<= 1) {
            const int64_t u = __shfl_up(inc, o);
            if (lane >= o) inc += u;
        }
        if (lane == 63) lds[wave] = inc;
        __syncthreads();
        int64_t pre = 0, t = 0;
#pragma unroll
        for (int q = 0; q < 16; ++q) { const int64_t x = lds[q]; if (q < wave) pre += x; t += x; }
        __syncthreads();
        tot = t;
        return inc + pre - s;
    };
    const bool derived = derive && (col == PC_SPAN || col == PC_SPAN_F || col == PC_WORK_SPAN_PTS || col == PC_UNFUSABLE);
    int64_t carry = 0, carry_pts = 0;
    for (int64_t b0 = 0; b0 < n; b0 += 4096) {
        const int64_t base = b0 + (int64_t)threadIdx.x * 4;
        int64_t v[4];
        if (derived) {
            int64_t pts[4], S[4], work[4];
#pragma unroll
            for (int k = 0; k < 4; ++k) {
                const bool in = base + k < n;
                pts[k] = in ? counts[(int64_t)PC_POINTS * n + base + k] : 0;
                S[k] = in ? counts[(int64_t)PC_SPAN_PTS * n + base + k] : 0;
                work[k] = in ? counts[(int64_t)PC_WORK * n + base + k] : 0;
            }
            int64_t tot_pts;
            int64_t off = scan4(pts, tot_pts) + carry_pts;
            carry_pts += tot_pts;
#pragma unroll
            for (int k = 0; k < 4; ++k) {
                int64_t c_span, c_span_f, c_wsp, c_unf;
                span_counts(off, S[k], work[k] != 0, fuse_possible != 0, c_span, c_span_f, c_wsp, c_unf);
                v[k] = col == PC_SPAN ? c_span : (col == PC_SPAN_F ? c_span_f : (col == PC_WORK_SPAN_PTS ? c_wsp : c_unf));
                if (col == PC_SPAN && c_span > SPEC_SPAN_CHUNKS) over = 1;
                if (base + k < n) counts[(int64_t)col * n + base + k] = v[k];
                off += pts[k];
            }
        } else {
#pragma unroll
            for (int k = 0; k < 4; ++k) v[k] = base + k < n ? counts[(int64_t)col * n + base + k] : 0;
        }
        int64_t tot;
        int64_t run = scan4(v, tot) + carry;
#pragma unroll
        for (int k = 0; k < 4; ++k) { if (base + k < n) bases[(int64_t)col * n + base + k] = run; run += v[k]; }
        carry += tot;
    }
    const bool spec_span = derive && spec_gen > 0 && col == PC_SPAN;
    if (spec_span) over = __syncthreads_or(over);
    if (threadIdx.x == 0) {
        totals[col] = carry;
        publish_total(totals, mirror, col, carry, with_flags && blockIdx.x == 0, derive && spec_gen > 0);
        if (spec_span) {
            unsigned long long *flag = reinterpret_cast<unsigned long long *>(totals + PC_COLS + PF_OVER_CAPACITY);
            if (over) atomicMax(flag, (unsigned long long)spec_gen);
            const int64_t v = over ? spec_gen : totals[PC_COLS + PF_OVER_CAPACITY];
            if (mirror) mirror[PC_COLS + PF_OVER_CAPACITY] = v;
        }
        if (with_flags) publish_done(totals, mirror, (int)gridDim.x, done_gen);
    }
}

int launch_scan(hipStream_t st, int64_t n, int c0, int c1, const DevPlanScratch &s, int64_t *mirror, int with_flags, int derive = 0, int fuse_possible = 0,
                int64_t spec_gen = 0, int64_t done_gen = 0)
{
    const int64_t nblk = (n + 1023) / 1024;
    const int nc = c1 - c0;
    if (nblk <= devplan_small_blocks()) {
        hipLaunchKernelGGL(k_scan_small, dim3((unsigned)nc), dim3(1024), 0, st, n, c0, s.counts, s.bases, s.totals, mirror, with_flags, derive, fuse_possible, spec_gen, done_gen);
        const hipError_t e0 = hipGetLastError();
        return e0 == hipSuccess ? 0 : (int)e0;
    }
    hipLaunchKernelGGL(k_scan_block_sums, dim3((unsigned)nblk, (unsigned)nc), dim3(256), 0, st, n, c0, s.counts, s.blk_sums, nblk);
    hipLaunchKernelGGL(k_scan_block_bases, dim3((unsigned)nc), dim3(256), 0, st, c0, s.blk_sums, nblk, s.totals, mirror, with_flags, done_gen);
    hipLaunchKernelGGL(k_scan_apply, dim3((unsigned)nblk, (unsigned)nc), dim3(256), 0, st, n, c0, s.counts, s.blk_sums, nblk, s.bases, derive, fuse_possible);
    const hipError_t e = hipGetLastError();
    return e == hipSuccess ? 0 : (int)e;
}

#ifdef FCPP_DIAG_TILE
__device__ unsigned long long g_tile_stamps[40], g_fill_stamps[40];
#define TSTAMP(k) do { if (!FILL && field == 1000 && lane == 0 && (k) < 40) g_tile_stamps[k] = wall_clock64(); } while (0)
#define FSTAMP(k) do { if (FILL && field == 1000 && lane == 0 && (k) < 40) g_fill_stamps[k] = wall_clock64(); } while (0)
#define WSTAMP(k) do { if (w_base == 128) TSTAMP(k); } while (0)
#else
#define TSTAMP(k) do { } while (0)
#define FSTAMP(k) do { } while (0)
#define WSTAMP(k) do { } while (0)
#endif
constexpr int TW_WAVES = 2;
constexpr int TW_NW = DEVPLAN_WINDOW;
constexpr int TW_LDS_PRIMS = 32;
constexpr int TW_LDS_TMPL = 36;
template <bool STAGE>
struct TileWaveLds {
    double d[TW_NW];
    static_assert(sizeof(double) * TW_NW >= sizeof(CutPrim) * CUT_PRIMS_MAX + sizeof(Pt2) * TW_LDS_TMPL, "the closed-form cut's LDS fits the window's");
    __device__ CutPrim *cut_rows() { return reinterpret_cast<CutPrim *>(d); }
    __device__ Pt2 *cut_tmpl() { return reinterpret_cast<Pt2 *>(reinterpret_cast<unsigned char *>(d) + sizeof(CutPrim) * CUT_PRIMS_MAX); }
    unsigned long long prim_words[STAGE ? TW_LDS_PRIMS * (sizeof(DevPrim) / 8) : 1];
    Pt2 tmpl[STAGE ? TW_LDS_TMPL : 1];
    int32_t pstart[DEVPLAN_PRIMS_CAP + 1];
    uint8_t pidx[TW_NW];
    uint8_t ins[TW_NW];
};

static_assert(sizeof(TilePartial) == 13 * 8, "thirteen 8-byte components");
__device__ __forceinline__ void init_entry(const DevPlanTables &T, int64_t e)
{
    T.stat_ids[e] = (int32_t)e; T.stat_run[e] = 0;
    unsigned long long *slot = reinterpret_cast<unsigned long long *>(T.partial + e);
    for (int w = 0; w < 13; ++w) slot[w] = 0ull;
}

__device__ __forceinline__ TilePartial run_consts(const DevField &F, double2 junc, int64_t e, int64_t count, const DevTile &tl,
                                                  const DevPrim *__restrict__ prims, const DevConst &cst)
{
    FieldStatView fv;
    fv.set(F, junc);
    const DevRun run = { (int32_t)e, 0, count };
    TilePartial tp = quiet_run_partial(run, tl, fv, prims, cst);
    tp.n_viol = tp.n_outside = tp.n_in_obstacle = tp.n_adjusted = 0;
    return tp;
}
__device__ __forceinline__ double2 field_junction(const DevField &F, const DevConst &cst)
{
    double2 junc = make_double2(0.0, 0.0);
    if (F.P >= 2 && F.n_line >= 2 && F.n_turn >= 1) junc.x = line_start_curvature(F, cst, 1, junc.y);
    return junc;
}

template <bool FILL, bool STAGE, bool DENSE>
struct TilePass {
    const int64_t n;
    const DevTileConsts &tc;
    const DevConst &cst;
    const DevField &F;
    const DevPrim *const prims;
    int64_t *const counts;
    const int64_t *const bases;
    int64_t *const totals;
    DevTile *const keep_tiles;
    DevWaveTile *const keep_wtiles;
    const DevPlanTables &T;
    TileWaveLds<STAGE> &L;
    const int64_t field;
    const int lane;
    const int64_t n_total = F.n_total;
    const int prim_count = F.prim_count;

    int64_t c_tiles = 0, c_wave = 0, c_general = 0, c_stat = 0, c_span = 0, c_work = 0, c_open = 0, c_runs = 0, c_span_pts = 0, c_wave_pts = 0,
            c_work_wave_pts = 0, c_wave_inside = 0, c_work_span_pts = 0, c_span_f = 0, c_unfusable = 0, c_chunks = 0, c_chunk_pts = 0;
    int cls = 0;
    bool fuse_spans = false, no_bases = false;
    int64_t pt_off = 0, wave_base = 0, general_base = 0, stat_base = 0, span_base = 0;
    int64_t prim_index0 = 0;
    int64_t S = 0, span_k = 0, fused_span = 0;
    int64_t n_wave = 0, n_general = 0, n_quiet = 0;
    bool fallback = false, is_work = false;
    bool dense_entries = false;
    DevWaveTile my_wt;
    int my_p0_rel = 0, my_np = 0;
    static constexpr int NFW = (int)(sizeof(DevField) / 8), NIW = (int)(sizeof(fcpp_field_info) / 8), PWD = (int)(sizeof(DevPrim) / 8), PF_ROUNDS = 7;
    static_assert(sizeof(DevField) % 8 == 0 && sizeof(DevPrim) % 8 == 0 && sizeof(fcpp_field_info) % 8 == 0 && NFW <= 64 && NIW <= 64, "copied as 8-byte words, a lane each");
    unsigned long long fw = 0, iw = 0, pw[PF_ROUNDS];
    int nwords_p = 0;
    int64_t per = 0, P = 0, gen_main = 0, n_main = 0, need1 = 0, pos = 0;
    double line_step_len = 0.0, cap = 0.0;
    bool turn_quiet = false, wave_ok = false;
    bool win_staged = false;
    const DevPrim *wprims = prims;
    const Pt2 *wtu = tc.tu, *wtc = tc.tc;
    int32_t my_pstart = INT32_MAX;

    __device__ __forceinline__ int64_t base_of(int col) const { return bases[(int64_t)col * n + field]; }
    __device__ __forceinline__ int64_t first_entry() const { return span_k > 0 ? 1 : 0; }

    __device__ __forceinline__ bool header(const fcpp_field_info *__restrict__ info)
    {
        if (FILL && tc.speculative) {
            bool up = false;
            for (int k = 0; k < PF_COUNT; ++k) up = up || totals[PC_COLS + k] == tc.gen;
            if (up) return false;
        }
        fuse_spans = (FILL && tc.speculative) ? (tc.fuse_spans != 0 && totals[PC_UNFUSABLE] == 0 && totals[PC_WORK_SPAN_PTS] > 0) : tc.fuse_spans != 0;
        no_bases = !FILL && tc.no_bases != 0;
        pt_off = no_bases ? 0 : base_of(PC_POINTS);
        if (FILL) {
            wave_base = base_of(PC_WAVE); general_base = base_of(PC_GENERAL); stat_base = base_of(PC_STAT);
            span_base = base_of(fuse_spans ? PC_SPAN_F : PC_SPAN); prim_index0 = base_of(PC_PRIMS);
        }
        nwords_p = prim_count * PWD;
        if (FILL) {
            if (lane < NFW) fw = reinterpret_cast<const unsigned long long *>(&F)[lane];
            if (lane < NIW) iw = reinterpret_cast<const unsigned long long *>(&info[field])[lane];
#pragma unroll
            for (int j = 0; j < PF_ROUNDS; ++j) { const int k = lane + 64 * j; pw[j] = k < nwords_p ? reinterpret_cast<const unsigned long long *>(prims)[k] : 0ull; }
            constexpr int W_PT = (int)(offsetof(DevField, pt_off) / 8), W_PF = (int)(offsetof(DevField, prim_first) / 8);
            constexpr bool PF_HI = (offsetof(DevField, prim_first) % 8) != 0;
            if (lane == W_PT) fw = (unsigned long long)pt_off;
            if (lane == (int)(offsetof(fcpp_field_info, point_offset) / 8)) iw = (unsigned long long)pt_off;
            if (lane == W_PF) fw = PF_HI ? ((fw & 0xffffffffull) | ((unsigned long long)(uint32_t)prim_index0 << 32)) : ((fw & 0xffffffff00000000ull) | (unsigned long long)(uint32_t)prim_index0);
// ... 851 lines not shown
```

### field_coverage_path_planning_amd/csrc/fcpp_sparse.hip

```cpp
#include "fcpp_sparse2_fn.h"
#include "fcpp_quiet_fn.h"

namespace fcpp {

template <int SP_WAVES, int PTS>
__global__ __launch_bounds__(64 * SP_WAVES) void k_plan_sparse(const DevWaveTile *__restrict__ wtiles, const int32_t *__restrict__ ids, int64_t n_wtiles,
                                                               const DevField *__restrict__ fields, const DevPrim *__restrict__ prims,
                                                               DevConst cst, DevObstacles obs, double *__restrict__ xo, double *__restrict__ yo,
                                                               double *__restrict__ ko, double *__restrict__ vo, uint32_t *__restrict__ fso,
                                                               TilePartial *__restrict__ partial, int xcd_map)
{
    __shared__ double obs_lds[SP_WAVES][2 * OBS_LDS_VERTS];
    __shared__ double atab[ATAN_TAB_DOUBLES];
    __shared__ double plds[SP_WAVES][TILE_PRIMS_LDS];
    const int wave = __builtin_amdgcn_readfirstlane((int)(threadIdx.x >> 6)), lane = threadIdx.x & 63;
    const unsigned bid = xcd_map ? (blockIdx.x & 7u) * (gridDim.x >> 3) + (blockIdx.x >> 3) : blockIdx.x;
    const int64_t slot = (int64_t)bid * SP_WAVES + wave;
    if (slot >= n_wtiles) return;
    atan_tab_stage(atab);
    const DevWaveTile wt = wtiles[ids ? (int64_t)ids[slot] : slot];
    SparseAcc acc;
    acc.clear();
    sparse_tile2<false>(wt, fields[wt.field], prims, cst, obs, obs_lds[wave], atab, plds[wave], xo, yo, ko, vo, fso, acc);

    double g[3] = { 0.0, 0.0, 0.0 };
    const int out0 = wt.hb, out1 = wt.hb + wt.count;
    if (out0 < wt.rel_seam) g[0] = wave4_to_hi<0>(acc.s_len[0], acc.s_tpre[0], acc.s_t[0], 0.0);
    if (out1 > wt.rel_seam + 1) g[1] = wave4_to_hi<0>(acc.s_len[1], acc.s_tpre[1], acc.s_t[1], 0.0);
    if (__ballot(acc.mk != 0.0 || acc.mj != 0.0) != 0ull) g[2] = wave4_to_hi<1>(acc.mk, acc.ma, acc.mj, 0.0);
    const int vs = WAVE4_SLOT(lane);
    if (lane >= 60 && vs < 3) {
        double *tp = reinterpret_cast<double *>(&partial[wt.tile]);
        tp[vs] = g[0]; tp[3 + vs] = g[1]; tp[6 + vs] = g[2];
    }
    if (lane == 63) {
        TilePartial &tp = partial[wt.tile];
        tp.n_viol = acc.c_viol; tp.n_outside = acc.c_out; tp.n_in_obstacle = acc.c_obs; tp.n_adjusted = acc.c_adj;
    }
}

template <int W, bool OBS>
__device__ __forceinline__ void field_span_chunk(const DevFieldPack &pk, int wave, const DevConst &cst, const DevObstacles &obs, double *obs_lds,
                                                 double *tlds, double *__restrict__ xo, double *__restrict__ yo, double *__restrict__ ko,
                                                 double *__restrict__ vo, uint32_t *__restrict__ fso, unsigned long long *cnt)
{
    static_assert(W == FUSED_SPAN_CHUNKS, "one chunk per wavefront");
    const int64_t S = pk.span_points;
    const DevField &f = pk.field;
    const unsigned per = (unsigned)(f.n_line + f.n_turn);
    const int r0 = (int)(f.pt_off & (TILE_POINTS - 1));
    const int c_first = (int)(S < TILE_POINTS - r0 ? S : TILE_POINTS - r0);
    const int n_chunks = (int)((r0 + S + TILE_POINTS - 1) / TILE_POINTS);
    if (wave >= n_chunks) return;
    wave_sync();
    stage_turn_template(cst, tlds);
    DevTile tl;
    const unsigned start = wave == 0 ? 0u : (unsigned)(c_first + (wave - 1) * TILE_POINTS);
    tl.field = pk.work.field; tl.start = start; tl.quiet = 4; tl.stat_tile = 0;
    tl.count = wave == 0 ? c_first : (int)((S - start < TILE_POINTS) ? S - start : TILE_POINTS);
    tl.idx0 = __builtin_amdgcn_readfirstlane((int)(start / per)); tl.off0 = __builtin_amdgcn_readfirstlane((int)(start - (unsigned)tl.idx0 * per));
    tl.count = __builtin_amdgcn_readfirstlane(tl.count);
    quiet_tile<16, true, OBS>(tl, &f, nullptr, cst, obs, obs_lds, tlds, xo, yo, ko, vo, fso, cnt, cnt + 1);
}

template <int W, bool OBS, bool SPANS>
__device__ __forceinline__ void plan_sparse_fields_body(const DevFieldPack *__restrict__ packs,
                                                              DevConst cst, double *__restrict__ xo, double *__restrict__ yo,
                                                              double *__restrict__ ko, double *__restrict__ vo, uint32_t *__restrict__ fso,
                                                              DevObstacles obs, TilePartial *__restrict__ partial,
                                                              const TilePartial *__restrict__ totals, fcpp_field_stats *__restrict__ stats)
{
    __shared__ double obs_lds[W][OBS ? 2 * OBS_LDS_VERTS : 1];
    __shared__ TilePartial red[FIELD_WORK_TILES];
    __shared__ double atab[ATAN_TAB_DOUBLES];
    static_assert(3 * TMPL_LDS >= TILE_PRIMS_LDS, "one area serves both phases");
    __shared__ double wlds[W][3 * TMPL_LDS];
    __shared__ unsigned long long span_cnt[W][2];
    const int wave = __builtin_amdgcn_readfirstlane((int)(threadIdx.x >> 6)), lane = threadIdx.x & 63;
    atan_tab_stage(atab);
    const DevFieldPack &pk = packs[blockIdx.x];
    const DevFieldWork w = pk.work;
#ifdef FCPP_DIAG_SPARSE
    if (g_sparse_stop == -2) return;
#endif
    auto plan_tile = [&](const int t) {
        const DevWaveTile wt = pk.tile[t];
        SparseAcc acc;
        acc.clear();
        sparse_tile2<true>(wt, pk.field, pk.prims[t], cst, obs, obs_lds[wave], atab, wlds[wave], xo, yo, ko, vo, fso, acc);
        double g[3] = { 0.0, 0.0, 0.0 };
        const int out0 = wt.hb, out1 = wt.hb + wt.count;
        if (out0 < wt.rel_seam) g[0] = wave4_to_hi<0>(acc.s_len[0], acc.s_tpre[0], acc.s_t[0], 0.0);
        if (out1 > wt.rel_seam + 1) g[1] = wave4_to_hi<0>(acc.s_len[1], acc.s_tpre[1], acc.s_t[1], 0.0);
        if (__ballot(acc.mk != 0.0 || acc.mj != 0.0) != 0ull) g[2] = wave4_to_hi<1>(acc.mk, acc.ma, acc.mj, 0.0);
        const int vs = WAVE4_SLOT(lane);
        if (lane >= 60 && vs < 3) {
            double *tp = reinterpret_cast<double *>(&red[t]);
            tp[vs] = g[0]; tp[3 + vs] = g[1]; tp[6 + vs] = g[2];
        }
        if (lane == 63) { red[t].n_viol = acc.c_viol; red[t].n_outside = acc.c_out; red[t].n_in_obstacle = acc.c_obs; red[t].n_adjusted = acc.c_adj; }
    };
    if (lane < 2) span_cnt[wave][lane] = 0;
    auto span_phase = [&]() {
        const DevFieldPack *pk2 = &pk;
        asm volatile("" : "+s"(pk2) : : "memory");
        if (pk2->span_points > 0) field_span_chunk<W, OBS>(*pk2, wave, cst, obs, obs_lds[wave], wlds[wave], xo, yo, ko, vo, fso, &span_cnt[wave][0]);
    };
    if (wave < w.n_tiles) plan_tile(wave);
    if (SPANS) span_phase();
    static_assert(sizeof(TilePartial) == 13 * 8 && sizeof(fcpp_field_stats) == 13 * 8, "statistics records are thirteen 8-byte components");
    unsigned long long run_v = 0, c_out = 0, c_obs = 0;
    if (wave == 0) {
        if (lane < 13) run_v = reinterpret_cast<const unsigned long long *>(&totals[blockIdx.x])[lane];
        if (lane < w.n_entries) { const TilePartial &slot = partial[w.e_first + lane]; c_out = (unsigned long long)slot.n_outside; c_obs = (unsigned long long)slot.n_in_obstacle; }
    }
    asm volatile("s_waitcnt lgkmcnt(0)\n\ts_barrier" ::: "memory");
    if (wave != 0) return;
    if ((c_out | c_obs) != 0ull) { partial[w.e_first + lane].n_outside = 0; partial[w.e_first + lane].n_in_obstacle = 0; }
    if (lane < W) { c_out += span_cnt[lane][0]; c_obs += span_cnt[lane][1]; }
    if (__ballot((c_out | c_obs) != 0ull) != 0ull) {
#pragma unroll
        for (int o = FIELD_WORK_ENTRIES / 2; o > 0; o >>= 1) { c_out += __shfl_xor(c_out, o); c_obs += __shfl_xor(c_obs, o); }
    }
    if (lane >= 13) return;
    const unsigned long long *rv = reinterpret_cast<const unsigned long long *>(red) + lane;
    unsigned long long bits;
    if (lane < 9) {
        double a = __longlong_as_double((long long)run_v);
        for (int t = 0; t < w.n_tiles; ++t) {
            const double x = __longlong_as_double((long long)rv[13 * t]);
            a = lane < 6 ? a + x : max_raw(a, x);
        }
        bits = (unsigned long long)__double_as_longlong(a);
    } else {
        bits = run_v;
        for (int t = 0; t < w.n_tiles; ++t) bits += rv[13 * t];
        if (lane == 10) bits += c_out;
        if (lane == 11) bits += c_obs;
    }
    reinterpret_cast<unsigned long long *>(&stats[w.field])[lane] = bits;
}

template <int W, bool OBS, bool SPANS>
__global__ __launch_bounds__(64 * W) void k_plan_sparse_fields(const DevFieldPack *__restrict__ packs, DevConst cst, double *__restrict__ xo, double *__restrict__ yo,
                                                              double *__restrict__ ko, double *__restrict__ vo, uint32_t *__restrict__ fso,
                                                              DevObstacles obs, TilePartial *__restrict__ partial,
                                                              const TilePartial *__restrict__ totals, fcpp_field_stats *__restrict__ stats)
{
    plan_sparse_fields_body<W, OBS, SPANS>(packs, cst, xo, yo, ko, vo, fso, obs, partial, totals, stats);
}

__global__ void k_work_totals(int64_t n_work, const DevFieldWork *__restrict__ work, const int64_t *__restrict__ stat_run,
                              const TilePartial *__restrict__ partial, TilePartial *__restrict__ totals)
{
    const int64_t i = (int64_t)blockIdx.x * blockDim.x + threadIdx.x;
    if (i >= n_work) return;
    const DevFieldWork w = work[i];
    TilePartial t;
    memset(&t, 0, sizeof t);
    for (int e = 0; e < w.n_entries; ++e) {
        if (stat_run[w.e_first + e] == 0) continue;
        const TilePartial p = partial[w.e_first + e];
        t.main_len += p.main_len; t.main_time_pre += p.main_time_pre; t.main_time += p.main_time;
        t.head_len += p.head_len; t.head_time_pre += p.head_time_pre; t.head_time += p.head_time;
        t.max_kappa = fmax(t.max_kappa, p.max_kappa); t.max_alat = fmax(t.max_alat, p.max_alat); t.max_jump = fmax(t.max_jump, p.max_jump);
        t.n_viol += p.n_viol; t.n_adjusted += p.n_adjusted;
    }
    totals[i] = t;
}

int launch_work_totals(hipStream_t st, int64_t n_work, const DevFieldWork *work, const int64_t *stat_run, const TilePartial *partial, TilePartial *totals)
{
    if (n_work <= 0) return 0;
    hipLaunchKernelGGL(k_work_totals, dim3((unsigned)((n_work + 255) / 256)), dim3(256), 0, st, n_work, work, stat_run, partial, totals);
    hipError_t e = hipGetLastError();
    return e == hipSuccess ? 0 : (int)e;
}

int launch_plan_sparse_fields(hipStream_t st, int64_t n_work, const DevFieldPack *packs, const DevConst &cst, const DevObstacles &obs, double *x,
                              double *y, double *kappa, double *v, uint32_t *fs, TilePartial *partial, int waves, const TilePartial *totals,
                              fcpp_field_stats *stats, bool spans)
{
    if (n_work <= 0) return 0;
#define FCPP_FW(K, W, OB, SP) FCPP_LAUNCH((K<W, OB, SP>), dim3((unsigned)n_work), dim3(64 * W), 0, st, packs, cst, x, y, kappa, v, fs, obs, partial, totals, stats)
    if (waves != 4) return (int)hipErrorInvalidValue;
    const bool has_obs = obs.offsets != nullptr;
    if (has_obs && spans) FCPP_FW(k_plan_sparse_fields, 4, true, true);
    else if (has_obs) FCPP_FW(k_plan_sparse_fields, 4, true, false);
    else if (spans) FCPP_FW(k_plan_sparse_fields, 4, false, true);
    else FCPP_FW(k_plan_sparse_fields, 4, false, false);
#undef FCPP_FW
    hipError_t e = hipGetLastError();
    return e == hipSuccess ? 0 : (int)e;
}

int launch_plan_sparse(hipStream_t st, int64_t n_wtiles, const DevWaveTile *wtiles, const DevField *fields, const DevPrim *prims,
                       const DevConst &cst, const DevObstacles &obs, double *x, double *y, double *kappa, double *v, uint32_t *fs,
                       TilePartial *partial, const int32_t *ids)
{
    if (n_wtiles <= 0) return 0;
    auto grid8 = [&](int64_t per) { const int64_t g = (n_wtiles + per - 1) / per; return dim3((unsigned)((g + 7) / 8 * 8)); };
    if (n_wtiles >= 65536) FCPP_LAUNCH((k_plan_sparse<2, 2>), grid8(2), dim3(128), 0, st, wtiles, ids, n_wtiles, fields, prims, cst, obs, x, y, kappa, v, fs, partial, 1);
    else FCPP_LAUNCH((k_plan_sparse<4, 2>), grid8(4), dim3(256), 0, st, wtiles, ids, n_wtiles, fields, prims, cst, obs, x, y, kappa, v, fs, partial, 1);
    hipError_t e = hipGetLastError();
    return e == hipSuccess ? 0 : (int)e;
}

}

#ifdef FCPP_DIAG_SPARSE
extern "C" long long fcpp_diag_sparse(unsigned *rows, long long cap)
{
    unsigned n = 0, zero = 0;
    if (hipDeviceSynchronize() != hipSuccess) return -1;
    if (hipMemcpyFromSymbol(&n, HIP_SYMBOL(fcpp::g_sparse_diag_next), sizeof n) != hipSuccess) return -1;
    const long long m = n < (unsigned)fcpp::SP_DIAG_SLOTS ? n : fcpp::SP_DIAG_SLOTS;
    const long long c = m < cap ? m : cap;
    if (c > 0 && hipMemcpyFromSymbol(rows, HIP_SYMBOL(fcpp::g_sparse_diag), (size_t)c * 16 * sizeof(unsigned)) != hipSuccess) return -1;
    if (hipMemcpyToSymbol(HIP_SYMBOL(fcpp::g_sparse_diag_next), &zero, sizeof zero) != hipSuccess) return -1;
    return n;
}
extern "C" int fcpp_diag_sparse_stop(int section)
{
    return hipMemcpyToSymbol(HIP_SYMBOL(fcpp::g_sparse_stop), &section, sizeof section) == hipSuccess ? 0 : -1;
}
#endif
```

### field_coverage_path_planning_amd/engine.py

```python
import ctypes as C
from dataclasses import dataclass

import numpy as np

from . import _lib as L

_contexts = {}


def _torch():
    import torch
    return torch


class Context:

    def __init__(self, device=0):
        torch = _torch()
        if not torch.cuda.is_available():
            raise RuntimeError('no GPU visible: the fcpp operators have no CPU fallback')
        self.device = int(device)
        self.lib = L.load()
        h = C.c_void_p()
        L.check(self.lib.fcpp_ctx_create(self.device, C.byref(h)))
# ... 359 lines not shown
        return slice(info.point_offset, info.point_offset + info.n_main + info.n_head)

    def path_offsets(self):
        a = self.batch.info.array
        off = np.zeros(2 * len(a) + 1, dtype=np.int64)
        off[1::2], off[2::2] = a['n_main'], a['n_head']
        return np.cumsum(off)

    def trajectory(self):
        torch = _torch()
        b = self.batch
        s, t, h = torch.empty_like(self.x), torch.empty_like(self.x), torch.empty_like(self.x)
        totals = torch.zeros((b.n_fields, 4), dtype=torch.float64, device=self.x.device)
        b.ctx.bind_stream()
        L.check(b.lib.fcpp_batch_trajectory(b.handle, _ptr(self.x), _ptr(self.y), _ptr(self.v), _ptr(self.flagseg), _ptr(s), _ptr(t), _ptr(h),
                                            _ptr(totals)))
        return s, t, h, totals

    def sample(self, dt, include_end=True):
        s, t, h, totals = self.trajectory()
        return _sample(self.batch.ctx, self.x, self.y, self.v, self.flagseg, self.path_offsets(), None, (s, t, h, totals.view(-1, 2)), dt, include_end)


    def drivable_connectors(self, radius=None, spacing=0.5, start_headings=None, end_headings=None, reversing=False):
        torch = _torch()
        b = self.batch
        a = b.info.array
        dev = self.x.device
        R = float(b.vehicle.min_turn_radius if radius is None else radius)
        ok = a['status'] == 0
        first_head = a['point_offset'] + a['n_main']
        has = (ok & (a['start_kept'] != 0) & (a['n_head'] > 0), ok & (a['n_main'] > 0) & (a['n_head'] > 0), ok & (a['end_kept'] != 0) & (a['n_head'] > 0))
        field = np.concatenate([np.flatnonzero(h) for h in has]).astype(np.int64)
        kind = np.concatenate([np.full(int(h.sum()), k, dtype=np.int32) for k, h in enumerate(has)])
        order = np.lexsort((kind, field))
        field, kind = field[order], kind[order]
        m = len(field)
        fi = np.where(kind == 1, first_head[field] - 1, np.where(kind == 2, first_head[field] + a['n_head'][field] - 1, 0))
        ti = np.where(kind == 2, 0, first_head[field])
        park = np.where((kind == 0)[:, None], a['approach_from'][field], a['departure_to'][field]).reshape(m, 2)
        heads = np.full(m, np.nan)
        for k, given in ((0, start_headings), (2, end_headings)):
            if given is not None:
                g = np.broadcast_to(np.asarray(given, dtype=np.float64), (b.n_fields,))
                heads[kind == k] = g[field[kind == k]]
        h = self.trajectory()[2]
        fi_d, ti_d = torch.as_tensor(fi, device=dev), torch.as_tensor(ti, device=dev)
        kind_d = torch.as_tensor(kind, device=dev)
        park_d, heads_d = torch.as_tensor(park, device=dev), torch.as_tensor(heads, device=dev)
        if self.x.numel() == 0:
            fi_d, ti_d = fi_d[:0], ti_d[:0]
        frm = torch.stack((self.x[fi_d], self.y[fi_d], h[fi_d]), dim=1)
        to = torch.stack((self.x[ti_d], self.y[ti_d], h[ti_d]), dim=1)
        is_ap, is_dp = (kind_d == 0)[:, None], (kind_d == 2)[:, None]
        ap_dir = torch.atan2(to[:, 1] - park_d[:, 1], to[:, 0] - park_d[:, 0])
        dp_dir = torch.atan2(park_d[:, 1] - frm[:, 1], park_d[:, 0] - frm[:, 0])
        given = ~torch.isnan(heads_d)
        ap_pose = torch.cat((park_d, torch.where(given, heads_d, ap_dir)[:, None]), dim=1)
        dp_pose = torch.cat((park_d, torch.where(given, heads_d, dp_dir)[:, None]), dim=1)
        frm = torch.where(is_ap, ap_pose, frm)
        to = torch.where(is_dp, dp_pose, to)
        out = _rs_paths(b.ctx, frm, to, R, spacing) if reversing else _dubins_paths(b.ctx, frm, to, R, spacing)
        out.update(field=field, kind=kind, from_poses=frm, to_poses=to, radius=R)
        return out


class Batch:

    def __init__(self, specs, vehicle, options=None, device=None):
        self.ctx = get_context(device)
        self.lib = self.ctx.lib
        self.vehicle = vehicle
        self.options = options or make_options()
        self.n_fields = len(specs)
        import time
        t0 = time.perf_counter()
        arr, polys, _keep = pack_fields(specs)
        self.pack_ms = (time.perf_counter() - t0) * 1e3
        self.ctx.bind_stream()
        h = C.c_void_p()
        L.check(self.lib.fcpp_batch_create(self.ctx.handle, C.byref(self.vehicle), C.byref(self.options),
                                           self.n_fields, arr, C.byref(polys), C.byref(h)))
        self.handle = h
        self._info = None
        self._token = object()
        tot = C.c_int64()
        L.check(self.lib.fcpp_batch_info(self.handle, None, C.byref(tot)))
        self.total_points = tot.value
        self._last_mode = 1

    @classmethod
    def plan(cls, specs, vehicle, options=None, device=None):
        torch = _torch()
        self = cls.__new__(cls)
        self.ctx = get_context(device)
        self.lib = self.ctx.lib
        self.vehicle = vehicle
        self.options = options or make_options()
        self.n_fields = len(specs)
        arr, polys, _keep = pack_fields(specs)
        self.pack_ms = 0.0
        self._info = None
        self._token = object()
        self._last_mode = 1
        self.ctx.bind_stream()
        h = C.c_void_p()
        ptrs = [C.c_void_p() for _ in range(5)]
        tot = C.c_int64()
        L.check(self.lib.fcpp_batch_plan(self.ctx.handle, C.byref(self.vehicle), C.byref(self.options), self.n_fields, arr, C.byref(polys),
                                         None, C.byref(h), *[C.byref(q) for q in ptrs], C.byref(tot)))
        dev = torch.device('cuda', self.ctx.device)
        self.handle = h
        self.total_points = n = tot.value
        sp = C.c_void_p()
        L.check(self.lib.fcpp_batch_own_stats(h, C.byref(sp)))
        if self.n_fields > 0 and sp.value:
            sv = _StatsView(self, sp.value, self.n_fields * L.STATS_WORDS)
            stats = torch.as_tensor(sv, device=dev).view(self.n_fields, L.STATS_WORDS)
            stats._fcpp_owner = sv
            self._stats_views = 1
        else:
            stats = torch.empty((self.n_fields, L.STATS_WORDS), dtype=torch.int64, device=dev)
        owner = _ArenaArrays(self.ctx, n, [q.value or 0 for q in ptrs])
        if n > 0:
            x, y, kappa, v, fs = owner.tensors(n)
        else:
            x, y, kappa, v = (torch.empty(0, dtype=torch.float64, device=dev) for _ in range(4))
            fs = torch.empty(0, dtype=torch.int32, device=dev)
            x._fcpp_owner = owner
        lane, pitch = self.ctx.arena()
        self.layout = {'layout': 'arena' if (n > 0 and pitch and owner.ptrs[1] - owner.ptrs[0] == pitch) else 'plain', 'one_call': True}
        bufs = self._trusted((x, y, kappa, v, fs, stats))
        return self, BatchResult(self, *bufs)

    @property
    def info(self):
        if self._info is None:
            t = InfoTable(self.n_fields)
            L.check(self.lib.fcpp_batch_info(self.handle, t._c, None))
            self._info = t
        return self._info

    def setup_times(self):
        t = L.SetupTimes()
        L.check(self.lib.fcpp_batch_setup_times(self.handle, C.byref(t)))
        return {'pack': self.pack_ms, 'host_plan': t.host_plan_ms, 'templates': t.templates_ms, 'tiler': t.tiler_ms, 'image': t.image_ms,
                'h2d': t.h2d_ms, 'create': t.total_ms, 'threads': int(t.threads), 'image_bytes': int(t.image_bytes),
                'device_setup': int(t.device_setup)}

    def setup_path(self):
        t = L.SetupTimes()
        L.check(self.lib.fcpp_batch_setup_times(self.handle, C.byref(t)))
        return 'device' if t.device_setup else 'host'

    def debug_table(self, table):
        nb = C.c_int64()
        L.check(self.lib.fcpp_batch_debug_table(self.handle, int(table), None, 0, C.byref(nb)))
        buf = np.zeros(max(nb.value, 1), dtype=np.uint8)
        L.check(self.lib.fcpp_batch_debug_table(self.handle, int(table), C.c_void_p(buf.ctypes.data), nb.value, C.byref(nb)))
        return buf[:nb.value]

    SPREAD_MIN_BYTES = 512 << 20

    def alloc(self, layout='auto', best_of=1, include=()):
        if best_of > 1 and self.total_points > 0:
            torch = _torch()
            import time
            dev = torch.device('cuda', self.ctx.device)
            sets, ms = list(include), []
            for _ in range(int(best_of)):
                try:
                    sets.append(self._alloc_once())
                except RuntimeError:
                    break
            if not sets:
                raise RuntimeError(f'out of device memory: no candidate set of output arrays ({36 * self.total_points / 2**30:.1f} GiB each) could be allocated')
            for s in sets:
                self.run(s)
                torch.cuda.synchronize(dev)
                t0 = time.perf_counter()
                for _ in range(3):
                    self.run(s)
                torch.cuda.synchronize(dev)
                ms.append((time.perf_counter() - t0) / 3 * 1e3)
            k = min(range(len(sets)), key=lambda i: ms[i])
            self.placement = {'probe': 'step', 'step_ms': [round(v, 4) for v in ms], 'chosen': k}
            keep = sets[k]
            del sets
            torch.cuda.empty_cache()
            return keep
        if layout not in ('auto', 'plain', 'spread', 'arena'):
            raise ValueError("layout: 'auto', 'plain', 'spread' or 'arena'")
        n = self.total_points
        lane, pitch = self.ctx.arena()
        if layout == 'arena' or (layout == 'auto' and lane >= 8 * n and 36 * n >= self.SPREAD_MIN_BYTES):
            if lane < 8 * n:
                raise RuntimeError('the context has no output arena of that size: Context.reserve_outputs()')
            torch = _torch()
            arr = _ArenaArrays(self.ctx, n)
            if arr.ptrs[1] - arr.ptrs[0] != pitch:
                self.layout = {'layout': 'plain', 'note': 'the output arena is full'}
            else:
                self.layout = {'layout': 'arena', 'pitch_GiB': round(pitch / 2**30, 3), 'lane_GiB': round(lane / 2**30, 3)}
            x, y, kappa, v, fs = arr.tensors(n)
            stats = torch.empty((self.n_fields, L.STATS_WORDS), dtype=torch.int64, device=torch.device('cuda', self.ctx.device))
            return self._trusted((x, y, kappa, v, fs, stats))
        if layout in ('plain', 'auto'):
            self.layout = {'layout': 'plain'}
            return self._trusted(self._alloc_once())
        return self._trusted(self._alloc_spread(strict=True))

    def _trusted(self, buffers):
        tok = self._token
        for t in buffers:
            t._fcpp_ok = tok
        return buffers

    def _alloc_spread(self, strict=False):
        torch = _torch()
        dev = torch.device('cuda', self.ctx.device)
        n = self.total_points
        S = (8 * n + 4095) // 4096 * 4096
        free, _total = torch.cuda.mem_get_info(dev)
        free += torch.cuda.memory_reserved(dev) - torch.cuda.memory_allocated(dev)
        reserve = 8 << 30
        P = max(L.OUTPUT_PITCH, S + (1 << 30))
        if free < 4 * P + S + reserve:
            P = (free - reserve - S) // 4 if free > 5 * S + reserve else 0
        P = P // 4096 * 4096
        if P < S + (1 << 30) and not strict:
            self.layout = {'layout': 'plain', 'note': 'no room for the spread layout'}
            return self._alloc_once()
        P = max(P, S)
        try:
            slab = torch.empty(4 * P + S, dtype=torch.uint8, device=dev)
        except RuntimeError:
            if strict:
                raise
            self.layout = {'layout': 'plain', 'note': 'the spread allocation failed'}
            return self._alloc_once()
        x, y, kappa, v = (slab[k * P: k * P + 8 * n].view(torch.float64) for k in range(4))
        fs = slab[4 * P: 4 * P + 4 * n].view(torch.int32)
        stats = torch.empty((self.n_fields, L.STATS_WORDS), dtype=torch.int64, device=dev)
        self.layout = {'layout': 'spread', 'pitch_GiB': round(P / 2**30, 3), 'allocation_GiB': round((4 * P + S) / 2**30, 3)}
        return x, y, kappa, v, fs, stats

    def _alloc_once(self):
        torch = _torch()
        dev = torch.device('cuda', self.ctx.device)
        n = self.total_points
        npad = (n + 63) // 64 * 64
        x, y, kappa, v = torch.empty((4, npad), dtype=torch.float64, device=dev)[:, :n].unbind(0)
        fs = torch.empty(n, dtype=torch.int32, device=dev)
        stats = torch.empty((self.n_fields, L.STATS_WORDS), dtype=torch.int64, device=dev)
        return x, y, kappa, v, fs, stats

    def _check_buffers(self, buffers):
        torch = _torch()
        x, y, kappa, v, fs, stats = buffers
        want = [('x', x, torch.float64, self.total_points), ('y', y, torch.float64, self.total_points),
                ('kappa', kappa, torch.float64, self.total_points), ('v', v, torch.float64, self.total_points),
                ('flagseg', fs, None, self.total_points), ('stats', stats, torch.int64, self.n_fields * L.STATS_WORDS)]
        for name, t, dtype, numel in want:
            if not isinstance(t, torch.Tensor) or not t.is_cuda or t.device.index != self.ctx.device:
                raise ValueError(f'{name}: expected a tensor on cuda:{self.ctx.device}')
            if dtype is None:
                if t.dtype not in (torch.int32, torch.uint32):
                    raise ValueError(f'{name}: expected int32 / uint32, got {t.dtype}')
            elif t.dtype != dtype:
                raise ValueError(f'{name}: expected {dtype}, got {t.dtype}')
            if t.numel() < numel or not t.is_contiguous():
                raise ValueError(f'{name}: needs {numel} contiguous elements, got {t.numel()}')

    def run(self, buffers=None, mode=1):
        if buffers is None:
            buffers = self.alloc()
        tok = self._token
        for t in buffers:
            if getattr(t, '_fcpp_ok', None) is not tok:
                self._check_buffers(buffers)
                break
        x, y, kappa, v, fs, stats = buffers
        self._last_mode = 1 if int(mode) >= 1 else 0
        self.ctx.bind_stream()
        L.check(self.lib.fcpp_batch_run(self.handle, _ptr(x), _ptr(y), _ptr(kappa), _ptr(v), _ptr(fs), _ptr(stats),
                                        int(mode)))
        return BatchResult(self, x, y, kappa, v, fs, stats)

    def connectors(self):
        torch = _torch()
        dev = torch.device('cuda', self.ctx.device)
        ap = torch.full((self.n_fields, 50, 2), float('nan'), dtype=torch.float64, device=dev)
        dp = torch.full((self.n_fields, 50, 2), float('nan'), dtype=torch.float64, device=dev)
        self.ctx.bind_stream()
        L.check(self.lib.fcpp_batch_connectors(self.handle, _ptr(ap), _ptr(dp)))
        return ap, dp

    def set_profiling(self, on=True, every=1):
        L.check(self.lib.fcpp_batch_set_profiling(self.handle, int(every) if on else 0))

    def stage_times(self):
        ms = (C.c_double * 16)()
        ns, nr = C.c_int(), C.c_int()
        L.check(self.lib.fcpp_batch_stage_times(self.handle, 16, ms, C.byref(ns), C.byref(nr)))
        runs = max(nr.value, 1)
        return {self.lib.fcpp_batch_stage_name(self._last_mode, k).decode(): ms[k] / runs for k in range(ns.value)}, nr.value
# ... 657 lines not shown
```

### include/fcpp.h

```cpp
#ifndef FCPP_H
#define FCPP_H
#include <stdint.h>

#ifdef __cplusplus
extern "C" {
#endif

#define FCPP_ABI_VERSION 5

enum {
    FCPP_OK = 0,
    FCPP_EINVAL = -1,
    FCPP_EHEADLAND = -2,
    FCPP_EUNSUPPORTED = -3,
    FCPP_EHIP = -4,
    FCPP_ENOMEM = -5,
    FCPP_ESIZE = -6
};

typedef struct fcpp_vehicle {
    double working_width;
    double min_turn_radius;
    double max_work_speed_kmh;
    double max_headland_speed_kmh;
    double headland_turn_speed_kmh;
    double max_lateral_accel;
    double max_longitudinal_accel;
    double safety_factor;
} fcpp_vehicle;

enum { FCPP_TURN_ARC = 0, FCPP_TURN_CLOTHOID = 1 };
typedef struct fcpp_options {
    int32_t turn_model;
    int32_t clothoid_fit;
    double sample_spacing;
    double clothoid_frac;
    double geofence_tol;
    int32_t obstacle_mode;
    int32_t ring_order;
} fcpp_options;
enum { FCPP_RING_AS_VERTICES = 0, FCPP_RING_REVERSED = 1 };

enum { FCPP_OBSTACLES_FLAG = 0, FCPP_OBSTACLES_AVOID = 1 };

typedef struct fcpp_field {
    double vx[4], vy[4];
    int32_t from_vertices;
    int32_t has_start, has_end;
    double start_x, start_y, end_x, end_y;
    int32_t n_obstacles;
    int32_t _pad;
    int64_t obstacle_first;
} fcpp_field;

typedef struct fcpp_polys {
    int64_t n_polys;
    const int64_t *offsets;
    const double *x, *y;
} fcpp_polys;

typedef struct fcpp_field_info {
    int64_t point_offset;
    int64_t n_main, n_head;
    int32_t n_swaths;
    int32_t n_loops;
    int32_t start_corner;
    int32_t reverse_order, start_from_right;
    int32_t rotated;
    int32_t start_kept, end_kept;
    int32_t shape;
    int32_t n_reverse[4];
    int32_t status;
    double corner_angles[4];
    double field_length, field_width, headland_width, rotation_angle;
    double approach_from[2], approach_to[2];
    double departure_from[2], departure_to[2];
} fcpp_field_info;

typedef struct fcpp_field_stats {
    double main_len_m, main_time_pre_s, main_time_s;
    double head_len_m, head_time_pre_s, head_time_s;
    double max_kappa, max_alat, max_jump;
    int64_t n_viol;
    int64_t n_outside;
    int64_t n_in_obstacle;
    int64_t n_adjusted;
} fcpp_field_stats;

enum {
    FCPP_KIND_SWATH = 0, FCPP_KIND_UTURN = 1, FCPP_KIND_HEAD_START = 2, FCPP_KIND_HEAD_STRAIGHT = 3,
    FCPP_KIND_CORNER = 4, FCPP_KIND_REVERSE = 5, FCPP_KIND_DETOUR = 6
};
#define FCPP_KIND_MASK 7u
#define FCPP_FLAG_HEADLAND 8u
#define FCPP_FLAG_ALAT 16u
#define FCPP_FLAG_OUTSIDE 32u
#define FCPP_FLAG_OBSTACLE 64u
#define FCPP_INDEX_SHIFT 8

typedef struct fcpp_ctx fcpp_ctx;
typedef struct fcpp_batch fcpp_batch;

const char *fcpp_last_error(void);
int fcpp_abi_version(void);
void fcpp_vehicle_default(fcpp_vehicle *v);
void fcpp_options_default(fcpp_options *o);
int fcpp_ctx_create(int device_id, fcpp_ctx **ctx);
int fcpp_ctx_destroy(fcpp_ctx *ctx);
int fcpp_ctx_set_stream(fcpp_ctx *ctx, void *hip_stream);
int fcpp_ctx_synchronize(fcpp_ctx *ctx);
enum { FCPP_SETUP_AUTO = 0, FCPP_SETUP_HOST = 1, FCPP_SETUP_DEVICE = 2 };
int fcpp_ctx_set_setup(fcpp_ctx *ctx, int mode);
int fcpp_malloc(fcpp_ctx *ctx, int64_t bytes, void **dev_ptr);
int fcpp_free(fcpp_ctx *ctx, void *dev_ptr);
#define FCPP_OUTPUT_PITCH ((int64_t)24 << 30)
int fcpp_ctx_reserve_outputs(fcpp_ctx *ctx, int64_t lane_bytes, int64_t pitch_bytes);
int fcpp_ctx_outputs_info(const fcpp_ctx *ctx, int64_t *lane_bytes, int64_t *pitch_bytes, int64_t *live_bytes);
int fcpp_outputs_alloc(fcpp_ctx *ctx, int64_t n_points, int64_t pitch_bytes, double **x_dev, double **y_dev, double **kappa_dev,
                       double **v_dev, uint32_t **flagseg_dev);
int fcpp_outputs_free(fcpp_ctx *ctx, double *x_dev);
int fcpp_memcpy_h2d(fcpp_ctx *ctx, void *dst_dev, const void *src, int64_t bytes);
int fcpp_memcpy_d2h(fcpp_ctx *ctx, void *dst, const void *src_dev, int64_t bytes);

int fcpp_plan_count(const fcpp_vehicle *veh, const fcpp_options *opt, int64_t n_fields,
                    const fcpp_field *fields, const fcpp_polys *obstacles ,
                    fcpp_field_info *info_out);
int fcpp_plan_points(fcpp_ctx *ctx, const fcpp_vehicle *veh, const fcpp_options *opt, int64_t n_fields, const fcpp_field *fields,
                     const fcpp_polys *obstacles, int64_t *points_out);
int fcpp_batch_create(fcpp_ctx *ctx, const fcpp_vehicle *veh, const fcpp_options *opt, int64_t n_fields,
                      const fcpp_field *fields, const fcpp_polys *obstacles, fcpp_batch **batch);
int fcpp_batch_info(const fcpp_batch *batch, fcpp_field_info *info_out ,
                    int64_t *total_points);
typedef struct fcpp_setup_times {
    double host_plan_ms;
    double templates_ms;
    double tiler_ms;
    double image_ms;
    double h2d_ms;
    double total_ms;
    int64_t image_bytes;
    int32_t threads;
    int32_t device_setup;
} fcpp_setup_times;
int fcpp_batch_setup_times(const fcpp_batch *batch, fcpp_setup_times *out);
int fcpp_batch_run(fcpp_batch *batch, double *x_dev, double *y_dev, double *kappa_dev, double *v_dev,
                   uint32_t *flagseg_dev, fcpp_field_stats *stats_dev, int mode);
int fcpp_batch_plan(fcpp_ctx *ctx, const fcpp_vehicle *veh, const fcpp_options *opt, int64_t n_fields, const fcpp_field *fields,
                    const fcpp_polys *obstacles, fcpp_field_stats *stats_dev, fcpp_batch **batch, double **x_dev, double **y_dev,
                    double **kappa_dev, double **v_dev, uint32_t **flagseg_dev, int64_t *total_points);
int fcpp_batch_own_stats(const fcpp_batch *batch, fcpp_field_stats **stats_dev);
int fcpp_batch_connectors(fcpp_batch *batch, double *approach_xy_dev, double *departure_xy_dev);
int fcpp_batch_trajectory(fcpp_batch *batch, const double *x_dev, const double *y_dev, const double *v_dev, const uint32_t *flagseg_dev,
                          double *s_dev, double *t_dev, double *heading_dev, double *totals_dev);
int fcpp_batch_destroy(fcpp_batch *batch);
int fcpp_batch_set_profiling(fcpp_batch *batch, int enable);
int fcpp_batch_stage_times(fcpp_batch *batch, int max_stages, double *ms_sum_out, int *n_stages_out, int *n_runs_out);
const char *fcpp_batch_stage_name(int mode, int stage);
int fcpp_batch_stage_points(const fcpp_batch *batch, int mode, int stage, int64_t *points);
int fcpp_batch_point_split(const fcpp_batch *batch, int64_t *quiet_points, int64_t *general_points);
int fcpp_batch_reduce_classes(const fcpp_batch *batch, int64_t *classes_out);

int fcpp_curvature(fcpp_ctx *ctx, int64_t n_paths, const int64_t *offsets_dev, int64_t total_points,
                   const double *x_dev, const double *y_dev, double *kappa_dev, const int64_t *offsets_host);
int fcpp_speed_plan(fcpp_ctx *ctx, const fcpp_vehicle *veh, int clamp, int64_t n_paths,
                    const int64_t *offsets_dev, int64_t total_points, const double *x_dev,
                    const double *y_dev, const double *v_in_dev, double *v_out_dev, double *kappa_dev,
                    int64_t *n_adjusted_dev, const int64_t *offsets_host);
int fcpp_verify(fcpp_ctx *ctx, const fcpp_vehicle *veh, int64_t n_paths, const int64_t *offsets_dev,
                int64_t total_points, const double *x_dev, const double *y_dev, const double *v_dev,
                fcpp_field_stats *stats_dev, const int64_t *offsets_host);
int fcpp_validate(fcpp_ctx *ctx, const fcpp_vehicle *veh, const fcpp_options *opt, int64_t n_paths, const int64_t *offsets_dev,
                  int64_t total_points, const double *x_dev, const double *y_dev, const double *v_dev, const fcpp_polys *field_polys,
                  const fcpp_polys *obstacles, const int64_t *obstacle_offsets, uint32_t *flags_dev, fcpp_field_stats *stats_dev,
                  const int64_t *offsets_host);
int fcpp_trajectory(fcpp_ctx *ctx, int64_t n_paths, const int64_t *offsets_dev, int64_t total_points, const double *x_dev, const double *y_dev,
                    const double *v_dev, const uint32_t *flagseg_dev , double *s_dev, double *t_dev, double *heading_dev,
                    double *totals_dev, const int64_t *offsets_host);
int fcpp_trajectory_counts(fcpp_ctx *ctx, int64_t n_paths, const double *totals_dev, double dt, int include_end, int64_t *out_offsets_dev,
                           int64_t *out_offsets_host);
int fcpp_trajectory_sample(fcpp_ctx *ctx, int64_t n_paths, const int64_t *offsets_dev, int64_t total_points, const double *x_dev,
                           const double *y_dev, const double *v_dev, const double *s_dev, const double *t_dev, const double *heading_dev,
                           const uint32_t *flagseg_dev , double dt, int include_end, const int64_t *out_offsets_dev,
                           int64_t total_samples, double *xs_dev, double *ys_dev, double *vs_dev, double *ss_dev, double *hs_dev,
                           uint32_t *flagseg_s_dev, int64_t *src_index_dev, const int64_t *offsets_host, const int64_t *out_offsets_host);
int fcpp_straight_segments(fcpp_ctx *ctx, int64_t n_seg, const double *seg_dev, int32_t n_points,
                           double *out_xy_dev);
int fcpp_corner_turns(fcpp_ctx *ctx, const fcpp_vehicle *veh, int64_t n, const double *corners_dev,
                      const int32_t *corner_index_dev, const int32_t *with_reverse_dev, double field_length,
                      double field_width, int32_t stride, double *out_xy_dev, int32_t *counts_dev);
int fcpp_fresnel(fcpp_ctx *ctx, int64_t n, const double *t_dev, double *c_dev, double *s_dev);

int fcpp_ga_fitness(fcpp_ctx *ctx, int32_t n_nodes, int64_t pop, const double *D_dev,
                    const int32_t *routes_dev, double *dist_dev, double *fit_dev, int order_mode);

typedef struct fcpp_ga_config {
    int32_t population_size, max_generations;
    double crossover_rate, mutation_rate;
    int32_t elite_size, tournament_size, convergence_threshold, _pad;
    uint64_t seed;
} fcpp_ga_config;
typedef struct fcpp_ga_result {
    int32_t generations;
    int32_t convergence_gen;
    double best_distance, best_fitness;
} fcpp_ga_result;
int fcpp_ga_evolve(fcpp_ctx *ctx, int32_t n_nodes, const fcpp_ga_config *cfg, const double *D_dev, int32_t *routes_dev,
                   int32_t *best_route_dev, double *hist_dev, fcpp_ga_result *result);

int fcpp_distance_matrix(fcpp_ctx *ctx, int32_t n, const double *x_dev, const double *y_dev, double *D_dev);
int fcpp_best_connections(fcpp_ctx *ctx, int64_t n_pairs, const int64_t *from_off_dev, const int64_t *to_off_dev,
                          const double *fx_dev, const double *fy_dev, const double *tx_dev, const double *ty_dev,
                          int32_t *best_from_dev, int32_t *best_to_dev, double *best_dist_dev);

int fcpp_dubins_solve(fcpp_ctx *ctx, int64_t n, const double *from_x_dev, const double *from_y_dev, const double *from_h_dev,
                      const double *to_x_dev, const double *to_y_dev, const double *to_h_dev, double radius, int32_t *word_dev,
                      double *seg_dev, double *len_dev);
int fcpp_dubins_matrix(fcpp_ctx *ctx, int64_t n_from, const double *from_x_dev, const double *from_y_dev, const double *from_h_dev,
                       int64_t n_to, const double *to_x_dev, const double *to_y_dev, const double *to_h_dev, double radius, double *D_dev,
                       int8_t *word_dev);
int fcpp_dubins_counts(fcpp_ctx *ctx, int64_t n, const double *len_dev, double spacing, int64_t *out_offsets_dev, int64_t *out_offsets_host);
int fcpp_dubins_sample(fcpp_ctx *ctx, int64_t n, const double *from_x_dev, const double *from_y_dev, const double *from_h_dev, double radius,
                       const int32_t *word_dev, const double *seg_dev, double spacing, const int64_t *out_offsets_dev, int64_t total_samples,
                       double *xs_dev, double *ys_dev, double *hs_dev, double *kappas_dev, const int64_t *out_offsets_host);

int fcpp_rs_solve(fcpp_ctx *ctx, int64_t n, const double *from_x_dev, const double *from_y_dev, const double *from_h_dev,
                  const double *to_x_dev, const double *to_y_dev, const double *to_h_dev, double radius, int32_t *word_dev,
                  double *seg_dev, double *len_dev);
int fcpp_rs_matrix(fcpp_ctx *ctx, int64_t n_from, const double *from_x_dev, const double *from_y_dev, const double *from_h_dev,
                   int64_t n_to, const double *to_x_dev, const double *to_y_dev, const double *to_h_dev, double radius, double *D_dev,
                   int8_t *word_dev);
int fcpp_rs_counts(fcpp_ctx *ctx, int64_t n, const int32_t *word_dev, const double *seg_dev, double spacing, int64_t *out_offsets_dev,
                   int64_t *out_offsets_host);
int fcpp_rs_sample(fcpp_ctx *ctx, int64_t n, const double *from_x_dev, const double *from_y_dev, const double *from_h_dev, double radius,
                   const int32_t *word_dev, const double *seg_dev, double spacing, const int64_t *out_offsets_dev, int64_t total_samples,
                   double *xs_dev, double *ys_dev, double *hs_dev, double *kappas_dev, int8_t *gears_dev, const int64_t *out_offsets_host);

#define FCPP_SWATH_MAX_CROSSINGS 64
int fcpp_swath_scores(fcpp_ctx *ctx, int64_t n, const int64_t *ring_offsets_dev, int64_t n_rings, const int64_t *vert_offsets_dev,
                      int64_t n_verts, const double *x_dev, const double *y_dev, int64_t A, const double *angles_dev, double W, double first,
                      double min_length, int32_t *n_swaths_dev, int32_t *n_lines_dev, double *length_dev, int32_t *status_dev);
int fcpp_swath_counts(fcpp_ctx *ctx, int64_t n, const int64_t *ring_offsets_dev, int64_t n_rings, const int64_t *vert_offsets_dev,
                      int64_t n_verts, const double *x_dev, const double *y_dev, const double *angle_dev, double W, double first,
                      double min_length, int64_t *out_offsets_dev, int64_t *out_offsets_host, int32_t *n_lines_dev, int32_t *status_dev);
int fcpp_swath_fill(fcpp_ctx *ctx, int64_t n, const int64_t *ring_offsets_dev, int64_t n_rings, const int64_t *vert_offsets_dev, int64_t n_verts,
                    const double *x_dev, const double *y_dev, const double *angle_dev, double W, double first, double min_length,
                    const int64_t *offsets_dev, int64_t n_total, double *ax_dev, double *ay_dev, double *bx_dev, double *by_dev, int32_t *line_dev,
                    double *length_dev);

typedef struct fcpp_cover_job {
    double ox, oy;
    double res, shift;
    double radius;
    int32_t nx, ny;
    int32_t n_a, n_b;
    int64_t pts_first;
    int64_t grid_first;
    int32_t strict;
    int32_t region;
    double outer[12];
    double inner[12];
} fcpp_cover_job;

int fcpp_cover_grid(fcpp_ctx *ctx, int64_t n_jobs, const fcpp_cover_job *jobs, int64_t n_pts, const double *px_dev,
                    const double *py_dev, uint8_t *grid_dev, int64_t *counts_dev);

int fcpp_gather(fcpp_ctx *ctx, void *nccl_comm, int rank, int world, int root, int n_arrays, const void *const *send_dev, const int32_t *elem_bytes,
                const int64_t *counts_per_rank, void *const *recv_dev, int flags);

int fcpp_debug_math(int fn, int64_t n, const double *a, const double *b, double *out0, double *out1);
int fcpp_debug_math_dev(fcpp_ctx *ctx, int fn, int64_t n, const double *a_dev, const double *b_dev, double *out0_dev, double *out1_dev);
int fcpp_debug_dubins(int64_t n, const double *from_x, const double *from_y, const double *from_h, const double *to_x, const double *to_y,
                      const double *to_h, double radius, int32_t *word, double *seg, double *len);
int fcpp_debug_rs(int64_t n, const double *from_x, const double *from_y, const double *from_h, const double *to_x, const double *to_y,
                  const double *to_h, double radius, int32_t *word, double *seg, double *len);
int fcpp_debug_swaths(int64_t n, const int64_t *ring_offsets, int64_t n_rings, const int64_t *vert_offsets, int64_t n_verts, const double *x,
                      const double *y, int64_t A, const double *angles, int per_field, double W, double first, double min_length,
                      int32_t *n_swaths, int32_t *n_lines, double *length, int32_t *status, int64_t *out_offsets, int64_t cap, double *ax,
                      double *ay, double *bx, double *by, int32_t *line, double *seg_length);
int fcpp_batch_debug_table(const fcpp_batch *batch, int table, void *dst, int64_t cap_bytes, int64_t *bytes_out);

#ifdef __cplusplus
}
#endif
#endif
```

Measured before the change: 50.32 billion points/s.

## Run fused work-span chunks on side stream concurrently with sparse field kernel

In the fused device-setup plan path, the long per-field work spans are split out into a new kernel launched on the side stream. It runs concurrently with the sparse, fused and per-field kernels on the main stream. The two kernels hand off per-field stats through a generation-tagged atomic exchange in a zeroed scratch area, so whichever finishes second adds the outside/obstacle counts. This aims to overlap span generation with the remaining plan stages, at the cost of extra cross-stream synchronisation and an unconditional __syncthreads_or in the scan kernel.

Result: slower. 46.69 billion points/s (-7.2%).

```diff
diff --git a/field_coverage_path_planning_amd/_lib.py b/field_coverage_path_planning_amd/_lib.py
--- a/field_coverage_path_planning_amd/_lib.py
+++ b/field_coverage_path_planning_amd/_lib.py
@@ -121,6 +121,7 @@
     ('fcpp_batch_own_stats', C.c_int, [_VP, C.POINTER(_VP)]),
     ('fcpp_batch_info', C.c_int, [_VP, C.POINTER(FieldInfo), c_i64_p]),
     ('fcpp_batch_setup_times', C.c_int, [_VP, C.POINTER(SetupTimes)]),
+    ('fcpp_batch_span_stream', C.c_int, [_VP, C.POINTER(C.c_int)]),
     ('fcpp_batch_run', C.c_int, [_VP, _VP, _VP, _VP, _VP, _VP, _VP, C.c_int]),
     ('fcpp_batch_connectors', C.c_int, [_VP, _VP, _VP]),
     ('fcpp_batch_trajectory', C.c_int, [_VP] * 9),
diff --git a/field_coverage_path_planning_amd/csrc/fcpp_api.cpp b/field_coverage_path_planning_amd/csrc/fcpp_api.cpp
--- a/field_coverage_path_planning_amd/csrc/fcpp_api.cpp
+++ b/field_coverage_path_planning_amd/csrc/fcpp_api.cpp
@@ -95,6 +95,12 @@
     const fcpp_field_info *info_dev = nullptr;
     std::vector<hipStream_t> used_streams;
     void note_stream(hipStream_t s) { if (std::find(used_streams.begin(), used_streams.end(), s) == used_streams.end()) used_streams.push_back(s); }
+    struct SpanSplit {
+        bool ready = false;
+        const DevField *ftmp = nullptr; const int64_t *span_pts = nullptr, *pt_offs = nullptr;
+        unsigned long long *sync = nullptr; int64_t gen = 0;
+    } span_split;
+    int span_stream_used = 0;
     hipStream_t setup_stream = nullptr;
     bool setup_pending = false;
     hipEvent_t ev_setup = nullptr;
@@ -225,10 +231,12 @@
     if (e == hipSuccess) e = hipStreamCreateWithFlags(&c->side, hipStreamNonBlocking);
     if (e == hipSuccess) e = hipEventCreateWithFlags(&c->ev_fork, hipEventDisableTiming);
     if (e == hipSuccess) e = hipEventCreateWithFlags(&c->ev_join, hipEventDisableTiming);
+    if (e == hipSuccess) e = hipEventCreateWithFlags(&c->ev_span, hipEventDisableTiming);
     if (e != hipSuccess) {
         if (c->own) (void)hipStreamDestroy(c->own);
         if (c->side) (void)hipStreamDestroy(c->side);
         if (c->ev_fork) (void)hipEventDestroy(c->ev_fork);
+        if (c->ev_join) (void)hipEventDestroy(c->ev_join);
         delete c;
         return fail(FCPP_EHIP, std::string("hipStreamCreate: ") + hipGetErrorString(e));
     }
@@ -253,6 +261,7 @@
     if (c->side) { (void)hipStreamSynchronize(c->side); (void)hipStreamDestroy(c->side); }
     if (c->ev_fork) (void)hipEventDestroy(c->ev_fork);
     if (c->ev_join) (void)hipEventDestroy(c->ev_join);
+    if (c->ev_span) (void)hipEventDestroy(c->ev_span);
     free_paths_cache(c);
     (void)c->stage_wait();
     if (c->stage) (void)hipHostFree(c->stage);
@@ -595,7 +604,7 @@
         const size_t want = need + need / 4;
         if (hipMalloc(&sl.p, want) != hipSuccess) { (void)hipGetLastError(); sl.p = nullptr; err = "out of device memory for the planner's scratch"; return FCPP_ENOMEM; }
         sl.cap = want;
-        DEVCHK(hipMemsetAsync(sl.p, 0, PLAN_TOTALS * sizeof(int64_t), st));
+        DEVCHK(hipMemsetAsync(sl.p, 0, devplan_scratch_zeroed_bytes(), st));
     }
     if (!c->plan_totals_host)
         { DEVCHK(hipHostMalloc((void **)&c->plan_totals_host, PLAN_TOTALS * sizeof(int64_t), hipHostMallocMapped | hipHostMallocCoherent)); memset(c->plan_totals_host, 0, PLAN_TOTALS * sizeof(int64_t)); }
@@ -779,6 +788,11 @@
     if (spec && tot[PC_COLS + PF_OVER_CAPACITY] != tc.gen) {
         counts_from_totals(lay, tot, fuse);
         tm.image_ms = ms_since(t0);
+        if (fuse && n_fields <= SPAN_SYNC_FIELDS) {
+            fcpp_batch::SpanSplit &sp = b->span_split;
+            sp.ready = true; sp.ftmp = s.fields_tmp; sp.span_pts = s.counts + (int64_t)PC_WORK_SPAN_PTS * n_fields; sp.pt_offs = s.bases + (int64_t)PC_POINTS * n_fields;
+            sp.sync = s.span_sync; sp.gen = tc.gen;
+        }
     } else {
         ImageLayout ex;
         device_layout(ex, n_fields, obstacles);
@@ -957,10 +971,12 @@
     return FCPP_OK;
 }
 
-int fcpp_batch_run(fcpp_batch *b, double *x, double *y, double *kappa, double *v, uint32_t *fs,
-                   fcpp_field_stats *stats, int mode)
+static int batch_run(fcpp_batch *b, double *x, double *y, double *kappa, double *v, uint32_t *fs,
+                     fcpp_field_stats *stats, int mode, bool split)
 {
     if (!b) return fail(FCPP_EINVAL, "batch is NULL");
+    split = split && b->span_split.ready;
+    b->span_split.ready = false;
     if (mode != 0 && mode != 1) return fail(FCPP_EINVAL, "unknown pipeline mode");
     if (mode != b->last_mode) { b->prof_runs = 0; b->last_mode = mode; }
     if (b->n_fields == 0) return FCPP_OK;
@@ -1011,6 +1027,15 @@
             HIPCHK(hipStreamWaitEvent(sd, b->ctx->ev_fork, 0));
         }
         const bool fw = lay.n_field_work > 0;
+        split = split && fw && !two && lay.work_span_points > 0 && lay.n_work[0] == lay.n_field_work && !ev;
+        if (split) {
+            const fcpp_batch::SpanSplit &sp = b->span_split;
+            hipStream_t ss = b->ctx->side;
+            b->note_stream(ss);
+            LAUNCHCHK(launch_plan_field_spans(ss, b->n_fields, sp.ftmp, sp.span_pts, sp.pt_offs, b->cst, obs, x, y, kappa, v, fs, stats, sp.sync, sp.gen));
+            b->span_stream_used = 1;
+            HIPCHK(hipEventRecord(b->ctx->ev_span, ss));
+        }
         if (!fw) STAGE(2, launch_plan_sparse(sd, lay.n_wave, t.wtiles, t.fields, t.prims, b->cst, obs, x, y, kappa, v, fs, t.partial));
         else STAGE(2, launch_plan_sparse(sd, lay.n_open_wave, t.wtiles, t.fields, t.prims, b->cst, obs, x, y, kappa, v, fs, t.partial, t.open_wave_ids));
         STAGE(3, launch_plan_fused(sd, lay.n_general, t.general_ids, t.tiles, t.fields, t.prims, b->cst, obs, x,
@@ -1023,7 +1048,9 @@
             bool first = true;
             for (int c = 0; c < 4; ++c) {
                 if (lay.n_work[c] == 0) continue;
-                if (first) STAGE(5, launch_plan_sparse_fields(st, lay.n_work[c], t.field_packs + off, b->cst, obs, x, y, kappa, v, fs, t.partial,
+                if (split) LAUNCHCHK(launch_plan_sparse_fields_join(st, lay.n_work[c], t.field_packs + off, b->cst, obs, x, y, kappa, v, fs, t.partial,
+                                                                    t.work_totals + off, stats, b->span_split.sync, b->span_split.gen));
+                else if (first) STAGE(5, launch_plan_sparse_fields(st, lay.n_work[c], t.field_packs + off, b->cst, obs, x, y, kappa, v, fs, t.partial,
                                                               FIELD_WORK_WAVES[c], t.work_totals + off, stats, lay.work_span_points > 0));
                 else LAUNCHCHK(launch_plan_sparse_fields(st, lay.n_work[c], t.field_packs + off, b->cst, obs, x, y, kappa, v, fs, t.partial,
                                                          FIELD_WORK_WAVES[c], t.work_totals + off, stats, lay.work_span_points > 0));
@@ -1049,6 +1076,7 @@
                 pl += lay.n_red[c];
             }
         }
+        if (split) HIPCHK(hipStreamWaitEvent(st, b->ctx->ev_span, 0));
         if (ev) ++b->prof_runs;
         return FCPP_OK;
     }
@@ -1063,6 +1091,19 @@
     STAGE(6, launch_reduce_stats(st, t.n_paths, t.partial.p, t.tile_first.p, t.n_adj.p, stats));
 #undef STAGE
     if (ev) ++b->prof_runs;
+    return FCPP_OK;
+}
+
+int fcpp_batch_run(fcpp_batch *b, double *x, double *y, double *kappa, double *v, uint32_t *fs,
+                   fcpp_field_stats *stats, int mode)
+{
+    return batch_run(b, x, y, kappa, v, fs, stats, mode, false);
+}
+
+int fcpp_batch_span_stream(const fcpp_batch *b, int *used)
+{
+    if (!b || !used) return fail(FCPP_EINVAL, "bad arguments");
+    *used = b->span_stream_used;
     return FCPP_OK;
 }
 
@@ -1083,11 +1124,12 @@
     const double t_alloc = trace ? ms_since(t_begin) : 0.0;
     if (rc == FCPP_OK) {
         if (!stats) stats = b->t.own_stats;
-        rc = fcpp_batch_run(b, *x, *y, *kappa, *v, *fs, stats, 1);
+        const char *e_ss = getenv("FCPP_SPAN_STREAM");
+        rc = batch_run(b, *x, *y, *kappa, *v, *fs, stats, 1, !(e_ss && atoi(e_ss) == 0));
         if (trace) fprintf(stderr, "[fcpp] plan call: entered at %.1f us (CLOCK_MONOTONIC mod 1 s), totals seen %.1f us, create returns %.1f, arrays %.1f, step enqueued %.1f\n",
                            (double)(std::chrono::duration_cast<std::chrono::nanoseconds>(t_begin.time_since_epoch()).count() % 1000000000ll) / 1e3,
                            g_trace_totals_ms * 1e3, t_create * 1e3, t_alloc * 1e3, ms_since(t_begin) * 1e3);
-        if (rc != FCPP_OK) { const std::string keep = g_err; (void)hipStreamSynchronize(c->stream); (void)fcpp_outputs_free(c, *x); g_err = keep; }
+        if (rc != FCPP_OK) { const std::string keep = g_err; (void)hipStreamSynchronize(c->stream); (void)hipStreamSynchronize(c->side); (void)fcpp_outputs_free(c, *x); g_err = keep; }
     }
     if (rc != FCPP_OK) {
         const std::string keep = g_err;
diff --git a/field_coverage_path_planning_amd/csrc/fcpp_api_internal.h b/field_coverage_path_planning_amd/csrc/fcpp_api_internal.h
--- a/field_coverage_path_planning_amd/csrc/fcpp_api_internal.h
+++ b/field_coverage_path_planning_amd/csrc/fcpp_api_internal.h
@@ -114,6 +114,7 @@
     hipStream_t own = nullptr, stream = nullptr;
     hipStream_t side = nullptr;
     hipEvent_t ev_fork = nullptr, ev_join = nullptr;
+    hipEvent_t ev_span = nullptr;
     void *stage = nullptr; size_t stage_cap = 0;
     hipStream_t stage_stream = nullptr; bool stage_busy = false;
     hipError_t stage_wait()
diff --git a/field_coverage_path_planning_amd/csrc/fcpp_device.h b/field_coverage_path_planning_amd/csrc/fcpp_device.h
--- a/field_coverage_path_planning_amd/csrc/fcpp_device.h
+++ b/field_coverage_path_planning_amd/csrc/fcpp_device.h
@@ -77,6 +77,12 @@
 int launch_plan_sparse_fields(hipStream_t st, int64_t n_work, const DevFieldPack *packs, const DevConst &cst, const DevObstacles &obs, double *x,
                               double *y, double *kappa, double *v, uint32_t *fs, TilePartial *partial, int waves, const TilePartial *totals,
                               fcpp_field_stats *stats, bool spans);
+int launch_plan_sparse_fields_join(hipStream_t st, int64_t n_work, const DevFieldPack *packs, const DevConst &cst, const DevObstacles &obs, double *x,
+                                   double *y, double *kappa, double *v, uint32_t *fs, TilePartial *partial, const TilePartial *totals,
+                                   fcpp_field_stats *stats, unsigned long long *span_sync, int64_t gen);
+int launch_plan_field_spans(hipStream_t st, int64_t n_fields, const DevField *ftmp, const int64_t *span_pts, const int64_t *pt_offs, const DevConst &cst,
+                            const DevObstacles &obs, double *x, double *y, double *kappa, double *v, uint32_t *fs, fcpp_field_stats *stats,
+                            unsigned long long *span_sync, int64_t gen);
 int launch_work_totals(hipStream_t st, int64_t n_work, const DevFieldWork *work, const int64_t *stat_run, const TilePartial *partial, TilePartial *totals);
 int launch_distance_matrix(hipStream_t st, int n, const double *x, const double *y, double *D);
 int launch_best_connections(hipStream_t st, int64_t n_pairs, const int64_t *fo, const int64_t *to, const double *fx, const double *fy,
diff --git a/field_coverage_path_planning_amd/csrc/fcpp_devplan.h b/field_coverage_path_planning_amd/csrc/fcpp_devplan.h
--- a/field_coverage_path_planning_amd/csrc/fcpp_devplan.h
+++ b/field_coverage_path_planning_amd/csrc/fcpp_devplan.h
@@ -46,8 +46,11 @@
     int64_t *totals;
     DevTile *keep_tiles;
     DevWaveTile *keep_wtiles;
+    unsigned long long *span_sync;
 };
+constexpr int64_t SPAN_SYNC_FIELDS = 8192;
 int64_t devplan_small_blocks();
+size_t devplan_scratch_zeroed_bytes();
 size_t devplan_scratch_layout(int64_t n, int max_prims, void *base, DevPlanScratch &s);
 
 constexpr int DEVPLAN_WINDOW = 576;
diff --git a/field_coverage_path_planning_amd/csrc/fcpp_devplan.hip b/field_coverage_path_planning_amd/csrc/fcpp_devplan.hip
--- a/field_coverage_path_planning_amd/csrc/fcpp_devplan.hip
+++ b/field_coverage_path_planning_amd/csrc/fcpp_devplan.hip
@@ -14,10 +14,18 @@
     auto take = [&](auto *&p, size_t count) { p = base ? reinterpret_cast<decltype(p + 0)>(static_cast<unsigned char *>(base) + off) : nullptr; off = (off + count * sizeof(*p) + 255) & ~(size_t)255; };
     const size_t nn = (size_t)(n > 0 ? n : 1), nblk = (nn + 1023) / 1024;
     take(s.totals, PLAN_TOTALS);
+    take(s.span_sync, (size_t)(2 * SPAN_SYNC_FIELDS));
     take(s.fields_in, nn); take(s.info, nn); take(s.fields_tmp, nn); take(s.prims_tmp, nn * (size_t)max_prims);
     take(s.counts, nn * PC_COLS); take(s.bases, nn * PC_COLS); take(s.blk_sums, nblk * PC_COLS);
     take(s.keep_tiles, nn * DEVPLAN_KEEP_ROWS); take(s.keep_wtiles, nn * DEVPLAN_KEEP_WROWS);
     return off;
+}
+
+size_t devplan_scratch_zeroed_bytes()
+{
+    DevPlanScratch s;
+    devplan_scratch_layout(1, 1, reinterpret_cast<void *>((uintptr_t)256), s);
+    return (size_t)(reinterpret_cast<unsigned char *>(s.fields_in) - reinterpret_cast<unsigned char *>(s.totals));
 }
 
 #define FCPP_FILL_TABLES(X)                                                                                                          \
@@ -605,7 +613,7 @@
         carry += tot;
     }
     const bool spec_span = derive && spec_gen > 0 && col == PC_SPAN;
-    if (spec_span) over = __syncthreads_or(over);
+    over = __syncthreads_or(over);
     if (threadIdx.x == 0) {
         totals[col] = carry;
         publish_total(totals, mirror, col, carry, with_flags && blockIdx.x == 0, derive && spec_gen > 0);
diff --git a/field_coverage_path_planning_amd/csrc/fcpp_sparse.hip b/field_coverage_path_planning_amd/csrc/fcpp_sparse.hip
--- a/field_coverage_path_planning_amd/csrc/fcpp_sparse.hip
+++ b/field_coverage_path_planning_amd/csrc/fcpp_sparse.hip
@@ -40,13 +40,11 @@
 }
 
 template <int W, bool OBS>
-__device__ __forceinline__ void field_span_chunk(const DevFieldPack &pk, int wave, const DevConst &cst, const DevObstacles &obs, double *obs_lds,
-                                                 double *tlds, double *__restrict__ xo, double *__restrict__ yo, double *__restrict__ ko,
-                                                 double *__restrict__ vo, uint32_t *__restrict__ fso, unsigned long long *cnt)
+__device__ __forceinline__ void span_chunk(const DevField &f, const int64_t S, const int32_t junc, int wave, const DevConst &cst, const DevObstacles &obs,
+                                           double *obs_lds, double *tlds, double *__restrict__ xo, double *__restrict__ yo, double *__restrict__ ko,
+                                           double *__restrict__ vo, uint32_t *__restrict__ fso, unsigned long long *cnt)
 {
     static_assert(W == FUSED_SPAN_CHUNKS, "one chunk per wavefront");
-    const int64_t S = pk.span_points;
-    const DevField &f = pk.field;
     const unsigned per = (unsigned)(f.n_line + f.n_turn);
     const int r0 = (int)(f.pt_off & (TILE_POINTS - 1));
     const int c_first = (int)(S < TILE_POINTS - r0 ? S : TILE_POINTS - r0);
@@ -56,20 +54,41 @@
     stage_turn_template(cst, tlds);
     DevTile tl;
     const unsigned start = wave == 0 ? 0u : (unsigned)(c_first + (wave - 1) * TILE_POINTS);
-    tl.field = pk.work.field; tl.start = start; tl.quiet = 4; tl.stat_tile = 0;
+    tl.field = junc; tl.start = start; tl.quiet = 4; tl.stat_tile = 0;
     tl.count = wave == 0 ? c_first : (int)((S - start < TILE_POINTS) ? S - start : TILE_POINTS);
     tl.idx0 = __builtin_amdgcn_readfirstlane((int)(start / per)); tl.off0 = __builtin_amdgcn_readfirstlane((int)(start - (unsigned)tl.idx0 * per));
     tl.count = __builtin_amdgcn_readfirstlane(tl.count);
     quiet_tile<16, true, OBS>(tl, &f, nullptr, cst, obs, obs_lds, tlds, xo, yo, ko, vo, fso, cnt, cnt + 1);
 }
-
-template <int W, bool OBS, bool SPANS>
+template <int W, bool OBS>
+__device__ __forceinline__ void field_span_chunk(const DevFieldPack &pk, int wave, const DevConst &cst, const DevObstacles &obs, double *obs_lds,
+                                                 double *tlds, double *__restrict__ xo, double *__restrict__ yo, double *__restrict__ ko,
+                                                 double *__restrict__ vo, uint32_t *__restrict__ fso, unsigned long long *cnt)
+{
+    span_chunk<W, OBS>(pk.field, pk.span_points, pk.work.field, wave, cst, obs, obs_lds, tlds, xo, yo, ko, vo, fso, cnt);
+}
+
+__device__ __forceinline__ void span_sync_store(unsigned long long *p, unsigned long long v) { __hip_atomic_store(p, v, __ATOMIC_RELAXED, __HIP_MEMORY_SCOPE_AGENT); }
+__device__ __forceinline__ unsigned long long span_sync_load(unsigned long long *p) { return __hip_atomic_load(p, __ATOMIC_RELAXED, __HIP_MEMORY_SCOPE_AGENT); }
+__device__ __forceinline__ bool span_sync_arrive(unsigned long long *tag, int64_t gen)
+{
+    asm volatile("s_waitcnt vmcnt(0)" ::: "memory");
+    unsigned long long old = 0;
+    if ((threadIdx.x & 63) == 0) old = __hip_atomic_exchange(tag, (unsigned long long)gen, __ATOMIC_RELAXED, __HIP_MEMORY_SCOPE_AGENT);
+    old = __shfl(old, 0);
+    asm volatile("" ::: "memory");
+    return old == (unsigned long long)gen;
+}
+
+template <int W, bool OBS, bool SPANS, bool JOIN = false>
 __device__ __forceinline__ void plan_sparse_fields_body(const DevFieldPack *__restrict__ packs,
                                                               DevConst cst, double *__restrict__ xo, double *__restrict__ yo,
                                                               double *__restrict__ ko, double *__restrict__ vo, uint32_t *__restrict__ fso,
                                                               DevObstacles obs, TilePartial *__restrict__ partial,
-                                                              const TilePartial *__restrict__ totals, fcpp_field_stats *__restrict__ stats)
-{
+                                                              const TilePartial *__restrict__ totals, fcpp_field_stats *__restrict__ stats,
+                                                              unsigned long long *__restrict__ span_sync = nullptr, int64_t gen = 0)
+{
+    static_assert(!(JOIN && SPANS), "a span is written by one of the two kernels");
     __shared__ double obs_lds[W][OBS ? 2 * OBS_LDS_VERTS : 1];
     __shared__ TilePartial red[FIELD_WORK_TILES];
     __shared__ double atab[ATAN_TAB_DOUBLES];
@@ -138,7 +157,17 @@
         if (lane == 10) bits += c_out;
         if (lane == 11) bits += c_obs;
     }
-    reinterpret_cast<unsigned long long *>(&stats[w.field])[lane] = bits;
+    unsigned long long *sw = reinterpret_cast<unsigned long long *>(&stats[w.field]);
+    if (!JOIN || w.fused_span <= 0) { sw[lane] = bits; return; }
+    const bool flag_word = lane == 10 || lane == 11;
+    if (flag_word) span_sync_store(sw + lane, bits);
+    else sw[lane] = bits;
+    unsigned long long *sy = span_sync + 2 * (int64_t)w.field;
+    if (!span_sync_arrive(sy, gen)) return;
+    if (flag_word) {
+        const unsigned long long c = span_sync_load(sy + 1);
+        span_sync_store(sw + lane, bits + (lane == 10 ? c >> 32 : (c & 0xffffffffull)));
+    }
 }
 
 template <int W, bool OBS, bool SPANS>
@@ -148,6 +177,55 @@
                                                               const TilePartial *__restrict__ totals, fcpp_field_stats *__restrict__ stats)
 {
     plan_sparse_fields_body<W, OBS, SPANS>(packs, cst, xo, yo, ko, vo, fso, obs, partial, totals, stats);
+}
+
+template <int W, bool OBS>
+__global__ __launch_bounds__(64 * W) void k_plan_sparse_fields_join(const DevFieldPack *__restrict__ packs, DevConst cst, double *__restrict__ xo, double *__restrict__ yo,
+                                                                   double *__restrict__ ko, double *__restrict__ vo, uint32_t *__restrict__ fso,
+                                                                   DevObstacles obs, TilePartial *__restrict__ partial,
+                                                                   const TilePartial *__restrict__ totals, fcpp_field_stats *__restrict__ stats,
+                                                                   unsigned long long *__restrict__ span_sync, int64_t gen)
+{
+    plan_sparse_fields_body<W, OBS, false, true>(packs, cst, xo, yo, ko, vo, fso, obs, partial, totals, stats, span_sync, gen);
+}
+
+template <int W, bool OBS>
+__global__ __launch_bounds__(64 * W) void k_plan_field_spans(int64_t n, const DevField *__restrict__ ftmp, const int64_t *__restrict__ span_pts,
+                                                            const int64_t *__restrict__ pt_offs, DevConst cst, DevObstacles obs,
+                                                            double *__restrict__ xo, double *__restrict__ yo, double *__restrict__ ko,
+                                                            double *__restrict__ vo, uint32_t *__restrict__ fso, fcpp_field_stats *__restrict__ stats,
+                                                            unsigned long long *__restrict__ span_sync, int64_t gen)
+{
+    __shared__ double obs_lds[W][OBS ? 2 * OBS_LDS_VERTS : 1];
+    __shared__ double wlds[W][3 * TMPL_LDS];
+    __shared__ unsigned long long span_cnt[W][2];
+    __shared__ double2 junc_lds[W];
+    const int wave = __builtin_amdgcn_readfirstlane((int)(threadIdx.x >> 6)), lane = threadIdx.x & 63;
+    const int64_t field = blockIdx.x;
+    if (field >= n) return;
+    const int64_t S = span_pts[field];
+    if (S <= 0) return;
+    DevField f = ftmp[field];
+    f.pt_off = pt_offs[field];
+    if (lane < 2) span_cnt[wave][lane] = 0;
+    double jump = 0.0, k_start = 0.0;
+    if (f.P >= 2 && f.n_line >= 2 && f.n_turn >= 1) k_start = line_start_curvature(f, cst, 1, jump);
+    if (lane == 0) junc_lds[wave] = make_double2(k_start, jump);
+    DevConst cw = cst;
+    cw.field_junc = &junc_lds[wave];
+    span_chunk<W, OBS>(f, S, 0, wave, cw, obs, obs_lds[wave], wlds[wave], xo, yo, ko, vo, fso, &span_cnt[wave][0]);
+    __syncthreads();
+    if (wave != 0) return;
+    unsigned long long c = 0;
+    if (lane < 2) for (int v = 0; v < W; ++v) c += span_cnt[v][lane];
+    const unsigned long long c_out = __shfl(c, 0), c_obs = __shfl(c, 1);
+    unsigned long long *sy = span_sync + 2 * field;
+    if (lane == 0) span_sync_store(sy + 1, (c_out << 32) | c_obs);
+    if (!span_sync_arrive(sy, gen)) return;
+    if (lane < 2 && c != 0) {
+        unsigned long long *sw = reinterpret_cast<unsigned long long *>(&stats[field]) + 10 + lane;
+        span_sync_store(sw, span_sync_load(sw) + c);
+    }
 }
 
 __global__ void k_work_totals(int64_t n_work, const DevFieldWork *__restrict__ work, const int64_t *__restrict__ stat_run,
@@ -194,6 +272,28 @@
     return e == hipSuccess ? 0 : (int)e;
 }
 
+int launch_plan_sparse_fields_join(hipStream_t st, int64_t n_work, const DevFieldPack *packs, const DevConst &cst, const DevObstacles &obs, double *x,
+                                   double *y, double *kappa, double *v, uint32_t *fs, TilePartial *partial, const TilePartial *totals,
+                                   fcpp_field_stats *stats, unsigned long long *span_sync, int64_t gen)
+{
+    if (n_work <= 0) return 0;
+    if (obs.offsets != nullptr) FCPP_LAUNCH((k_plan_sparse_fields_join<4, true>), dim3((unsigned)n_work), dim3(256), 0, st, packs, cst, x, y, kappa, v, fs, obs, partial, totals, stats, span_sync, gen);
+    else FCPP_LAUNCH((k_plan_sparse_fields_join<4, false>), dim3((unsigned)n_work), dim3(256), 0, st, packs, cst, x, y, kappa, v, fs, obs, partial, totals, stats, span_sync, gen);
+    hipError_t e = hipGetLastError();
+    return e == hipSuccess ? 0 : (int)e;
+}
+
+int launch_plan_field_spans(hipStream_t st, int64_t n_fields, const DevField *ftmp, const int64_t *span_pts, const int64_t *pt_offs, const DevConst &cst,
+                            const DevObstacles &obs, double *x, double *y, double *kappa, double *v, uint32_t *fs, fcpp_field_stats *stats,
+                            unsigned long long *span_sync, int64_t gen)
+{
+    if (n_fields <= 0) return 0;
+    if (obs.offsets != nullptr) hipLaunchKernelGGL((k_plan_field_spans<4, true>), dim3((unsigned)n_fields), dim3(256), 0, st, n_fields, ftmp, span_pts, pt_offs, cst, obs, x, y, kappa, v, fs, stats, span_sync, gen);
+    else hipLaunchKernelGGL((k_plan_field_spans<4, false>), dim3((unsigned)n_fields), dim3(256), 0, st, n_fields, ftmp, span_pts, pt_offs, cst, obs, x, y, kappa, v, fs, stats, span_sync, gen);
+    hipError_t e = hipGetLastError();
+    return e == hipSuccess ? 0 : (int)e;
+}
+
 int launch_plan_sparse(hipStream_t st, int64_t n_wtiles, const DevWaveTile *wtiles, const DevField *fields, const DevPrim *prims,
                        const DevConst &cst, const DevObstacles &obs, double *x, double *y, double *kappa, double *v, uint32_t *fs,
                        TilePartial *partial, const int32_t *ids)
diff --git a/field_coverage_path_planning_amd/engine.py b/field_coverage_path_planning_amd/engine.py
--- a/field_coverage_path_planning_amd/engine.py
+++ b/field_coverage_path_planning_amd/engine.py
@@ -535,6 +535,11 @@
         t = L.SetupTimes()
         L.check(self.lib.fcpp_batch_setup_times(self.handle, C.byref(t)))
         return 'device' if t.device_setup else 'host'
+
+    def span_stream(self):
+        u = C.c_int()
+        L.check(self.lib.fcpp_batch_span_stream(self.handle, C.byref(u)))
+        return bool(u.value)
 
     def debug_table(self, table):
         nb = C.c_int64()
diff --git a/include/fcpp.h b/include/fcpp.h
--- a/include/fcpp.h
+++ b/include/fcpp.h
@@ -148,6 +148,7 @@
 int fcpp_batch_plan(fcpp_ctx *ctx, const fcpp_vehicle *veh, const fcpp_options *opt, int64_t n_fields, const fcpp_field *fields,
                     const fcpp_polys *obstacles, fcpp_field_stats *stats_dev, fcpp_batch **batch, double **x_dev, double **y_dev,
                     double **kappa_dev, double **v_dev, uint32_t **flagseg_dev, int64_t *total_points);
+int fcpp_batch_span_stream(const fcpp_batch *batch, int *used);
 int fcpp_batch_own_stats(const fcpp_batch *batch, fcpp_field_stats **stats_dev);
 int fcpp_batch_connectors(fcpp_batch *batch, double *approach_xy_dev, double *departure_xy_dev);
 int fcpp_batch_trajectory(fcpp_batch *batch, const double *x_dev, const double *y_dev, const double *v_dev, const uint32_t *flagseg_dev,
```
